# endiqq/Multi-Feature-ViT

Measured on AMD Instinct MI355X. Metric: images/sec (two-stream 224^2 vit_small MF-CA train step), higher is better.
Workload: dtype bf16x3 (split bf16 hi+lo operands, 3 MFMAs per product, f32 accumulate)

## Files before the change

### include/mfvit.h

```cpp
#ifndef MFVIT_H
#define MFVIT_H
#include <stddef.h>
#include <stdint.h>

#ifdef __cplusplus
extern "C" {
#endif

typedef void* mfvit_stream_t;

#define MFVIT_OK 0
#define MFVIT_EINVAL (-22)
#define MFVIT_ENOSYS (-38)
#define MFVIT_ELAUNCH (-5)

#define MFVIT_F32 0
#define MFVIT_BF16 1
#define MFVIT_BF16X3 2
#define MFVIT_F16 3
#define MFVIT_X3F16 4

int mfvit_abi_version(void);
const char* mfvit_build_info(void);

typedef struct mfvit_vit_cfg {
    int dtype;
    int batch;
    int img_h, img_w;
    int dim;
    int depth;
    int heads;
    int mlp_dim;
    int save_for_backward;
    int stop_grad_conv1;
    float ln_eps;
    int token_input;
    int tokens;
    int use_pos;
    int act;
    float p_embd, p_attn, p_resid;
    uint32_t seed_lo, seed_hi;
    int stream_share;
} mfvit_vit_cfg;

size_t mfvit_vit_param_count(const mfvit_vit_cfg* cfg);
int mfvit_vit_param_layout(const mfvit_vit_cfg* cfg, int64_t out[9]);

size_t mfvit_vit_shadow_bytes(const mfvit_vit_cfg* cfg);
int mfvit_vit_prepare_shadow(const mfvit_vit_cfg* cfg, const float* params, void* shadow, mfvit_stream_t stream);

size_t mfvit_vit_workspace_bytes(const mfvit_vit_cfg* cfg);

int mfvit_vit_forward(const mfvit_vit_cfg* cfg, const float* params, const void* shadow, const float* img, void* workspace,
                      float* features, mfvit_stream_t stream);

int mfvit_vit_backward(const mfvit_vit_cfg* cfg, const float* params, const void* shadow, void* workspace, const float* dfeatures,
                       float* dparams, int stage_hi, int stage_lo, mfvit_stream_t stream);

typedef struct mfvit_vit_drop {
    float drop;
    float attn_drop;
    const float* drop_path;
    uint64_t seed;
} mfvit_vit_drop;
size_t mfvit_vit_workspace_bytes_drop(const mfvit_vit_cfg* cfg, const mfvit_vit_drop* drop);
int mfvit_vit_forward_drop(const mfvit_vit_cfg* cfg, const mfvit_vit_drop* drop, const float* params, const void* shadow, const float* img,
                           void* workspace, float* features, mfvit_stream_t stream);
int mfvit_vit_backward_drop(const mfvit_vit_cfg* cfg, const mfvit_vit_drop* drop, const float* params, const void* shadow, void* workspace,
                            const float* dfeatures, float* dparams, int stage_hi, int stage_lo, mfvit_stream_t stream);

size_t mfvit_vit_workspace_bytes_ex(const mfvit_vit_cfg* cfg, const mfvit_vit_drop* drop, int want_dimg);
int mfvit_vit_backward_ex(const mfvit_vit_cfg* cfg, const mfvit_vit_drop* drop, const float* params, const void* shadow, void* workspace,
                          const float* dfeatures, float* dparams, float* dimg, int stage_hi, int stage_lo, mfvit_stream_t stream);

typedef struct mfvit_vit_attn_req {
    uint64_t blocks;
    int fuse;
    int cls_only;
    float* maps;
    float* rollout;
    void* scratch;
} mfvit_vit_attn_req;
size_t mfvit_vit_attn_scratch_bytes(const mfvit_vit_cfg* cfg, const mfvit_vit_attn_req* req);
int mfvit_vit_forward_attn(const mfvit_vit_cfg* cfg, const mfvit_vit_attn_req* req, const float* params, const void* shadow,
                           const float* img, void* workspace, float* features, mfvit_stream_t stream);

typedef struct mfvit_vit_rel_req {
    uint64_t blocks;
    float* maps;
    float* relevance;
    void* scratch;
} mfvit_vit_rel_req;
size_t mfvit_vit_rel_scratch_bytes(const mfvit_vit_cfg* cfg, const mfvit_vit_rel_req* req);
int mfvit_vit_backward_rel(const mfvit_vit_cfg* cfg, const mfvit_vit_rel_req* req, const float* params, const void* shadow, void* workspace,
                           const float* dfeatures, mfvit_stream_t stream);

int mfvit_gpt_forward(const mfvit_vit_cfg* cfg, const float* params, const void* shadow, const float* tokens, void* workspace, float* out,
                      mfvit_stream_t stream);
int mfvit_gpt_backward(const mfvit_vit_cfg* cfg, const float* params, const void* shadow, void* workspace, const float* dout, float* dparams,
                       float* dtokens, mfvit_stream_t stream);

int mfvit_linear_fwd(int dtype, int epilogue, const void* x, int64_t ldx, const void* w, int64_t ldw, const float* bias, void* y,
                     int64_t ldy, void* y2, int64_t ldy2, int M, int N, int K, mfvit_stream_t stream);
int mfvit_linear_dgrad_act(int dtype, const void* dy, int64_t lddy, const void* wt, int64_t ldwt, const void* act_grad, int64_t ldg,
                           void* dx, int64_t lddx, int M, int N, int K, mfvit_stream_t stream);
int mfvit_linear_wgrad(int dtype, const void* dy, int64_t lddy, const void* x, int64_t ldx, float* dw, int64_t lddw, int M, int N, int K,
                       mfvit_stream_t stream);
#define MFVIT_WGRAD_SCRATCH_FLOATS (384 * 128 * 128)
int mfvit_linear_wgrad_ws(int dtype, const void* dy, int64_t lddy, const void* x, int64_t ldx, float* dw, int64_t lddw, int M, int N,
                          int K, float* scratch, mfvit_stream_t stream);
int mfvit_linear_wgrad_pair(int dtype, const void* dy_a, int64_t lddy_a, const void* x_a, int64_t ldx_a, float* dw_a, int64_t lddw_a, float* dbias_a,
                            int Na, const void* dy_b, int64_t lddy_b, const void* x_b, int64_t ldx_b, float* dw_b, int64_t lddw_b, int Nb, int M, int K,
                            mfvit_stream_t stream);
int mfvit_linear_res_ln_fwd(int dtype, const void* a, int64_t lda, const void* w, int64_t ldw, const float* bias, const float* res,
                            int64_t ldres, float* x_out, void* y, int y_f32, const float* gamma, const float* beta, float eps,
                            float* mean, float* rstd, int M, int K, mfvit_stream_t stream);
int mfvit_linear_dgrad_ln_bwd(int dtype, const void* dy, int64_t lddy, const void* wt, int64_t ldwt, const float* x, const float* mean,
                              const float* rstd, const float* gamma, const float* dres, float* dx, void* dx_t, float* dgamma,
                              float* dbeta, float* dcol, int M, int K, mfvit_stream_t stream);
#define MFVIT_ROWP_SCRATCH_FLOATS (264 * 7 * 12 * 512)
int mfvit_linear_res_ln_fwd_ws(int dtype, const void* a, int64_t lda, const void* w, int64_t ldw, const float* bias, const float* res,
                               int64_t ldres, float* x_out, void* y, int y_f32, const float* gamma, const float* beta, float eps,
                               float* mean, float* rstd, int M, int K, float* scratch, mfvit_stream_t stream);
int mfvit_linear_dgrad_ln_bwd_ws(int dtype, const void* dy, int64_t lddy, const void* wt, int64_t ldwt, const float* x, const float* mean,
                                 const float* rstd, const float* gamma, const float* dres, float* dx, void* dx_t, float* dgamma,
                                 float* dbeta, float* dcol, int M, int K, float* scratch, mfvit_stream_t stream);
int mfvit_attention_qkv_dtype(int dtype, int T, int head_dim);
int mfvit_attention_fwd(int dtype, const void* qkv, void* out, float* lse, int B, int T, int H, int head_dim, mfvit_stream_t stream);
int mfvit_attention_bwd(int dtype, const void* qkv, const void* out, const void* dout, const float* lse, void* dqkv, float* dbias_qkv,
                        int B, int T, int H, int head_dim, mfvit_stream_t stream);
int mfvit_attention_drop_fwd(int dtype, const void* qkv, void* out, float* lse, int B, int T, int H, int head_dim, float p, uint64_t seed,
                             uint32_t site, mfvit_stream_t stream);
int mfvit_attention_drop_bwd(int dtype, const void* qkv, const void* out, const void* dout, const float* lse, void* dqkv, int B, int T, int H,
                             int head_dim, float p, uint64_t seed, uint32_t site, mfvit_stream_t stream);
int mfvit_dropout_mask(float p, uint64_t seed, uint32_t site, int64_t n, uint8_t* keep, mfvit_stream_t stream);
int mfvit_layernorm_fwd(int dtype, const float* x, void* y, int y_f32, const float* gamma, const float* beta, float eps, float* mean,
                        float* rstd, int rows, int N, mfvit_stream_t stream);
int mfvit_layernorm_bwd(int dtype, const float* dy, const float* x, const float* mean, const float* rstd, const float* gamma,
                        const float* dres, float* dx, void* dx_t, float* dgamma, float* dbeta, float* dcol, int rows, int N,
                        mfvit_stream_t stream);
int mfvit_cast_transpose(int dtype, const float* src, void* dst, void* dst_t, int R, int C, mfvit_stream_t stream);
int mfvit_head_fwd(const float* x, int64_t ldx, const float* w, const float* b, float* y, int64_t ldy, int M, int N, int K, int accumulate,
                   mfvit_stream_t stream);
int mfvit_head_bwd(const float* dy, int64_t lddy, const float* x, int64_t ldx, const float* w, float* dx, int64_t lddx, int dx_accumulate,
                   float* dw, float* db, int M, int N, int K, mfvit_stream_t stream);
int mfvit_cross_entropy(const float* logits, const int64_t* target, float* loss_mean, float* dlogits, int64_t* preds, int B, int C,
                        mfvit_stream_t stream);
int mfvit_cross_entropy_soft(const float* logits, const int64_t* target, const int32_t* partner, const float* lam, float smoothing,
                             float* loss_mean, float* dlogits, int64_t* preds, int B, int C, mfvit_stream_t stream);

int mfvit_batch_mix(const float* a, const float* b, float* out_a, float* out_b, const int32_t* desc, const float* lam, int n, int C, int H,
                    int W, mfvit_stream_t stream);

int mfvit_input_transform(const uint8_t* src, const int64_t* desc, const int32_t* tables, int n, int S, int crop, const float* mean3,
                          const float* std3, float* out, mfvit_stream_t stream);
int mfvit_input_transform_rect(const uint8_t* src, const int64_t* desc, const int32_t* tables, int n, int S, int out_h, int out_w,
                               const float* mean3, const float* std3, float* out, mfvit_stream_t stream);

size_t mfvit_input_photometric_workspace_bytes(int n, int S);
int mfvit_input_photometric(const uint8_t* src, const int64_t* desc, const int32_t* tables, const int32_t* photo, int n, int S, int max_radius,
                            void* workspace, const float* mean3, const float* std3, float* out, mfvit_stream_t stream);

int mfvit_eval_counts(const float* scores, int64_t ld, const int64_t* labels, int n, int C, uint64_t* confusion, int64_t* preds,
                      uint64_t* u2, uint64_t* npos, mfvit_stream_t stream);

int mfvit_patch_rank(const float* rel, int64_t ld, int32_t* rank, int B, int P, mfvit_stream_t stream);
int mfvit_patch_perturb(const float* img, const int32_t* rank, const int32_t* steps, const float* fill, float* out, int B, int C, int H,
                        int W, int S, mfvit_stream_t stream);
int mfvit_perturb_score(const float* logits, int64_t ld, const int64_t* target, int S, int B, int C, uint64_t* correct, double* sums,
                        uint64_t* nonfinite, mfvit_stream_t stream);

int mfvit_attr_inputs(const float* x, const float* base, int base_full, const float* alpha, const float* sigma, const uint64_t* seed, int s0,
                      float* out, int S, int B, int C, int64_t hw, mfvit_stream_t stream);
int mfvit_attr_accumulate(const float* g, const float* w, float* acc, int k, int B, int64_t n, int power, mfvit_stream_t stream);
int mfvit_attr_finish(const float* acc, const float* x, const float* base, int base_full, int times_input, int absval, float* pixels,
                      float* patches, double* total, int B, int C, int H, int W, mfvit_stream_t stream);

typedef struct mfvit_fusion_cfg {
    int batch;
    int tokens;
    int dim;
    int heads;
    int num_classes;
    float eps_pre;
    float eps_post;
} mfvit_fusion_cfg;

size_t mfvit_fusion_param_count(const mfvit_fusion_cfg* cfg);
size_t mfvit_fusion_workspace_bytes(const mfvit_fusion_cfg* cfg);
int mfvit_fusion_forward(const mfvit_fusion_cfg* cfg, const float* params, const float* f_cxr, const float* f_enh, const float* hw_cxr,
                         const float* hb_cxr, const float* hw_enh, const float* hb_enh, void* workspace, float* fused, float* x_cxr,
                         float* x_enh, mfvit_stream_t stream);
int mfvit_fusion_backward(const mfvit_fusion_cfg* cfg, const float* params, const float* f_cxr, const float* f_enh, const float* hw_cxr,
                          const float* hw_enh, void* workspace, const float* dfused, const float* dx_cxr, const float* dx_enh,
                          float* dparams, float* df_cxr, float* df_enh, float* dhw_cxr, float* dhb_cxr, float* dhw_enh, float* dhb_enh,
                          mfvit_stream_t stream);

size_t mfvit_fusion_ex_param_count(const mfvit_fusion_cfg* cfg, int cross_attn_depth, int pool_mean);
size_t mfvit_fusion_ex_workspace_bytes(const mfvit_fusion_cfg* cfg, int cross_attn_depth, int pool_mean);
int mfvit_fusion_ex_forward(const mfvit_fusion_cfg* cfg, int cross_attn_depth, int pool_mean, const float* params, const float* f_cxr,
                            const float* f_enh, const float* hw_cxr, const float* hb_cxr, const float* hw_enh, const float* hb_enh,
                            void* workspace, float* fused, float* x_cxr, float* x_enh, mfvit_stream_t stream);
int mfvit_fusion_ex_backward(const mfvit_fusion_cfg* cfg, int cross_attn_depth, int pool_mean, const float* params, const float* f_cxr,
                             const float* f_enh, const float* hw_cxr, const float* hw_enh, void* workspace, const float* dfused,
                             const float* dx_cxr, const float* dx_enh, float* dparams, float* df_cxr, float* df_enh, float* dhw_cxr,
                             float* dhb_cxr, float* dhw_enh, float* dhb_enh, mfvit_stream_t stream);

int mfvit_fusion_ex_attention(const mfvit_fusion_cfg* cfg, int cross_attn_depth, int pool_mean, const void* workspace, int layer, int fuse,
                              float* out, mfvit_stream_t stream);
int mfvit_fusion_ex_grad_attention(const mfvit_fusion_cfg* cfg, int cross_attn_depth, int pool_mean, const float* params, const float* f_cxr,
                                   const float* f_enh, const void* workspace, int layer, float* abar, mfvit_stream_t stream);

size_t mfvit_bimodal_relevance_scratch_bytes(int B, int T);
int mfvit_bimodal_relevance(int B, int T, int depth_c, int depth_e, const float* maps_c, const float* maps_e, const float* abar, float* out4,
                            void* scratch, mfvit_stream_t stream);

int mfvit_prenorm_xattn_forward(const mfvit_fusion_cfg* cfg, const float* params, const float* x_own, const float* x_oth,
                                void* workspace, float* out, mfvit_stream_t stream);
int mfvit_prenorm_xattn_backward(const mfvit_fusion_cfg* cfg, const float* params, const float* x_own, const float* x_oth,
                                 void* workspace, const float* dout, float* dparams, float* dx_own, float* dx_oth,
                                 mfvit_stream_t stream);

int mfvit_xattn_forward(const mfvit_fusion_cfg* cfg, const float* params, const float* x, void* workspace, float* out,
                        mfvit_stream_t stream);
int mfvit_xattn_backward(const mfvit_fusion_cfg* cfg, const float* params, const float* x, void* workspace, const float* dout,
                         float* dparams, float* dx, mfvit_stream_t stream);

int mfvit_prof_enable(int class_mask);
int mfvit_set_wgrad_stream(int enabled);
int mfvit_set_stream_share(int n);
int mfvit_prof_collect(double* out, int ncls);
int mfvit_prof_collect_tags(double* out, int ntags);
const char* mfvit_prof_class_name(int cls);

int mfvit_bn_stats(int dtype, const void* x, int n, int C, float* mean, float* m2, mfvit_stream_t stream);
int mfvit_bn_combine(const float* means, const float* m2s, const float* counts, int W, int C, float eps, float momentum, float* mean,
                     float* invstd, float* running_mean, float* running_var, mfvit_stream_t stream);
int mfvit_bn_apply(int dtype, const void* x, const float* mean, const float* invstd, const float* gamma, const float* beta, int relu,
                   void* y, int n, int C, mfvit_stream_t stream);
int mfvit_bn_bwd_sums(int dtype, const void* dy, const void* x, const void* y, const float* mean, const float* invstd, int relu, int n,
                      int C, float* s1, float* s2, mfvit_stream_t stream);
int mfvit_bn_bwd_apply(int dtype, const void* dy, const void* x, const void* y, const float* mean, const float* invstd, const float* gamma,
                       int relu, const float* S1, const float* S2, float inv_count, void* dx, int n, int C, mfvit_stream_t stream);
int mfvit_l2norm_fwd(const float* x, float* y, float* inv_norm, int n, int C, float eps, mfvit_stream_t stream);
int mfvit_l2norm_bwd(const float* dy, const float* y, const float* inv_norm, float* dx, int n, int C, mfvit_stream_t stream);
int mfvit_rowdot(const float* a, const float* b, float* out, int64_t ldo, float scale, int n, int C, mfvit_stream_t stream);
int mfvit_cross_entropy_rows(const float* logits, int64_t ld, const int64_t* target, float* loss_mean, float* lse, float* dlogits,
                             int64_t ldd, int n, int C, mfvit_stream_t stream);
int mfvit_ema_update(float* dst, const float* src, float m, int64_t n, mfvit_stream_t stream);

int mfvit_lars_step(const int64_t* table, int nchunks, int ntensors, float* norms, float lr, float weight_decay, float momentum,
                    float trust_coefficient, mfvit_stream_t stream);
int mfvit_adam_step(const int64_t* table, int nchunks, float lr, float beta1, float beta2, float eps, float weight_decay, int step,
                    mfvit_stream_t stream);
int mfvit_sgd_step(const int64_t* table, int nchunks, float lr, float momentum, float weight_decay, int first_step,
                   mfvit_stream_t stream);
int mfvit_amp_unscale(const int64_t* table, int nchunks, float inv_scale, float* found_inf, mfvit_stream_t stream);

int mfvit_grad_norm_partials(const int64_t* table, int nchunks, int norm_kind, float* partials, mfvit_stream_t stream);
int mfvit_grad_clip_coef(const float* partials, const int32_t* row_tensor, int nrows, int ntensors, int norm_kind, double max_norm,
                         float* per_tensor, float* out2, mfvit_stream_t stream);
int mfvit_grad_scale(const int64_t* table, int nchunks, const float* coef, mfvit_stream_t stream);

#ifdef __cplusplus
}
#endif
#endif
```

### multi-feature-vit_amd/csrc/abi_ops.hip

```cpp
#include "../../include/mfvit.h"
#include "kernels.h"

using namespace mfvit;

extern "C" {

int mfvit_input_transform(const uint8_t* src, const int64_t* desc, const int32_t* tables, int n, int S, int crop, const float* mean3,
                          const float* std3, float* out, mfvit_stream_t stream) {
    if (!src || !desc || !tables || !mean3 || !std3 || !out) return MFVIT_EINVAL;
    if (crop > S) return MFVIT_EINVAL;
    return input_transform(src, (const long long*)desc, tables, n, S, crop, crop, mean3, std3, out, (hipStream_t)stream);
}
int mfvit_input_transform_rect(const uint8_t* src, const int64_t* desc, const int32_t* tables, int n, int S, int out_h, int out_w,
                               const float* mean3, const float* std3, float* out, mfvit_stream_t stream) {
    if (!src || !desc || !tables || !mean3 || !std3 || !out) return MFVIT_EINVAL;
    return input_transform(src, (const long long*)desc, tables, n, S, out_h, out_w, mean3, std3, out, (hipStream_t)stream);
}
size_t mfvit_input_photometric_workspace_bytes(int n, int S) { return input_photometric_workspace_bytes(n, S); }
int mfvit_input_photometric(const uint8_t* src, const int64_t* desc, const int32_t* tables, const int32_t* photo, int n, int S, int max_radius,
                            void* workspace, const float* mean3, const float* std3, float* out, mfvit_stream_t stream) {
    if (!src || !desc || !tables || !photo || !workspace || !mean3 || !std3 || !out) return MFVIT_EINVAL;
    return input_photometric(src, (const long long*)desc, tables, photo, n, S, max_radius, workspace, mean3, std3, out, (hipStream_t)stream);
}
int mfvit_eval_counts(const float* scores, int64_t ld, const int64_t* labels, int n, int C, uint64_t* confusion, int64_t* preds,
                      uint64_t* u2, uint64_t* npos, mfvit_stream_t stream) {
    if (!scores || !labels || (!confusion && !(u2 && npos))) return MFVIT_EINVAL;
    return eval_counts(scores, ld, labels, n, C, (unsigned long long*)confusion, (unsigned long long*)u2, (unsigned long long*)npos, preds,
                       (hipStream_t)stream);
}
int mfvit_linear_fwd(int dtype, int epilogue, const void* x, int64_t ldx, const void* w, int64_t ldw, const float* bias, void* y,
                     int64_t ldy, void* y2, int64_t ldy2, int M, int N, int K, mfvit_stream_t stream) {
    if (!x || !w || (!y && epilogue != EPI_BIAS_GELU)) return MFVIT_EINVAL;
    if (epilogue != EPI_BIAS && epilogue != EPI_BIAS_GELU && epilogue != EPI_NONE && epilogue != EPI_BIAS_X3F16) return MFVIT_EINVAL;
    if (epilogue == EPI_BIAS_GELU && !y2) return MFVIT_EINVAL;
    GemmP p = nt(x, ldx, w, ldw, M, N, K);
    p.bias = bias; p.out0 = y; p.ldo0 = ldy; p.out1 = y2; p.ldo1 = ldy2;
    return gemm_nt_tile(dtype, epilogue, p, (hipStream_t)stream);
}
int mfvit_linear_dgrad_act(int dtype, const void* dy, int64_t lddy, const void* wt, int64_t ldwt, const void* act_grad, int64_t ldg,
                           void* dx, int64_t lddx, int M, int N, int K, mfvit_stream_t stream) {
    if (!dy || !wt || !act_grad || !dx) return MFVIT_EINVAL;
    GemmP p = nt(dy, lddy, wt, ldwt, M, N, K);
    p.aux = act_grad; p.ldaux = ldg; p.out0 = dx; p.ldo0 = lddx;
    return gemm_nt_tile(dtype, EPI_GELU_BWD, p, (hipStream_t)stream);
}
int mfvit_linear_wgrad(int dtype, const void* dy, int64_t lddy, const void* x, int64_t ldx, float* dw, int64_t lddw, int M, int N, int K,
                       mfvit_stream_t stream) {
    if (!dy || !x || !dw) return MFVIT_EINVAL;
    GemmP p = nt(dy, lddy, x, ldx, M, N, K);
    p.out0 = dw; p.ldo0 = lddw;
    return gemm_tn(dtype, p, (hipStream_t)stream);
}
int mfvit_linear_wgrad_ws(int dtype, const void* dy, int64_t lddy, const void* x, int64_t ldx, float* dw, int64_t lddw, int M, int N,
                          int K, float* scratch, mfvit_stream_t stream) {
    if (!dy || !x || !dw) return MFVIT_EINVAL;
    GemmP p = nt(dy, lddy, x, ldx, M, N, K);
    p.out0 = dw; p.ldo0 = lddw;
    p.cpart = scratch;
    return gemm_tn(dtype, p, (hipStream_t)stream);
}
int mfvit_linear_wgrad_pair(int dtype, const void* dy_a, int64_t lddy_a, const void* x_a, int64_t ldx_a, float* dw_a, int64_t lddw_a, float* dbias_a,
                            int Na, const void* dy_b, int64_t lddy_b, const void* x_b, int64_t ldx_b, float* dw_b, int64_t lddw_b, int Nb, int M, int K,
                            mfvit_stream_t stream) {
    if (!dy_a || !x_a || !dw_a || !dy_b || !x_b || !dw_b) return MFVIT_EINVAL;
    GemmP a = nt(dy_a, lddy_a, x_a, ldx_a, M, Na, K), b = nt(dy_b, lddy_b, x_b, ldx_b, M, Nb, K);
    a.out0 = dw_a; a.ldo0 = lddw_a; a.cs0 = dbias_a;
    b.out0 = dw_b; b.ldo0 = lddw_b;
    if (!gemm_tn_pair_supported(dtype, a, b)) return MFVIT_ENOSYS;
    return gemm_tn_glds_pair(dtype, a, b, (hipStream_t)stream);
}
int mfvit_linear_res_ln_fwd(int dtype, const void* a, int64_t lda, const void* w, int64_t ldw, const float* bias, const float* res,
                            int64_t ldres, float* x_out, void* y, int y_f32, const float* gamma, const float* beta, float eps,
                            float* mean, float* rstd, int M, int K, mfvit_stream_t stream) {
    return mfvit_linear_res_ln_fwd_ws(dtype, a, lda, w, ldw, bias, res, ldres, x_out, y, y_f32, gamma, beta, eps, mean, rstd, M, K, nullptr, stream);
}
int mfvit_linear_res_ln_fwd_ws(int dtype, const void* a, int64_t lda, const void* w, int64_t ldw, const float* bias, const float* res,
                               int64_t ldres, float* x_out, void* y, int y_f32, const float* gamma, const float* beta, float eps,
                               float* mean, float* rstd, int M, int K, float* scratch, mfvit_stream_t stream) {
    if (!a || !w || !y || !gamma || !beta || ((size_t)scratch & 15)) return MFVIT_EINVAL;
    GemmP p = nt(a, lda, w, ldw, M, 384, K);
    p.kpart = scratch;
    p.bias = bias; p.res = res; p.ldres = ldres;
    p.out0 = x_out; p.ldo0 = 384; p.out1 = y; p.ldo1 = (dtype == MFVIT_BF16X3 && !y_f32) ? 768 : 384; p.y_f32 = y_f32;
    p.gamma = gamma; p.beta = beta; p.eps = eps; p.mean = mean; p.rstd = rstd;
    return gemm_nt_row(dtype, REPI_RES_LN, p, (hipStream_t)stream);
}
int mfvit_linear_dgrad_ln_bwd(int dtype, const void* dy, int64_t lddy, const void* wt, int64_t ldwt, const float* x, const float* mean,
                              const float* rstd, const float* gamma, const float* dres, float* dx, void* dx_t, float* dgamma,
                              float* dbeta, float* dcol, int M, int K, mfvit_stream_t stream) {
    return mfvit_linear_dgrad_ln_bwd_ws(dtype, dy, lddy, wt, ldwt, x, mean, rstd, gamma, dres, dx, dx_t, dgamma, dbeta, dcol, M, K, nullptr, stream);
}
int mfvit_linear_dgrad_ln_bwd_ws(int dtype, const void* dy, int64_t lddy, const void* wt, int64_t ldwt, const float* x, const float* mean,
                                 const float* rstd, const float* gamma, const float* dres, float* dx, void* dx_t, float* dgamma,
                                 float* dbeta, float* dcol, int M, int K, float* scratch, mfvit_stream_t stream) {
    if (!dy || !wt || !x || !mean || !rstd || !gamma || !dx || ((size_t)scratch & 15)) return MFVIT_EINVAL;
    GemmP p = nt(dy, lddy, wt, ldwt, M, 384, K);
    p.kpart = scratch;
    p.aux = x; p.ldaux = 384; p.mean = (float*)mean; p.rstd = (float*)rstd; p.gamma = gamma;
    p.res = dres; p.ldres = 384;
    p.out0 = dx; p.ldo0 = 384; p.out1 = dx_t; p.ldo1 = dtype == MFVIT_BF16X3 ? 768 : 384;
    p.cs0 = dgamma; p.cs1 = dbeta; p.cs2 = dcol;
    return gemm_nt_row(dtype, REPI_LNBWD_RES, p, (hipStream_t)stream);
}
int mfvit_attention_fwd(int dtype, const void* qkv, void* out, float* lse, int B, int T, int H, int head_dim, mfvit_stream_t stream) {
    if (!qkv || !out || !lse || B <= 0 || T <= 0 || H <= 0) return MFVIT_EINVAL;
    return attn_fwd(dtype, qkv, out, lse, B, T, H, head_dim, (hipStream_t)stream);
}
int mfvit_attention_qkv_dtype(int dtype, int T, int head_dim) { return attn_qkv_dtype(dtype, T, head_dim); }
int mfvit_attention_bwd(int dtype, const void* qkv, const void* out, const void* dout, const float* lse, void* dqkv, float* dbias_qkv,
                        int B, int T, int H, int head_dim, mfvit_stream_t stream) {
    if (!qkv || !out || !dout || !lse || !dqkv || B <= 0 || T <= 0 || H <= 0) return MFVIT_EINVAL;
    return attn_bwd(dtype, qkv, out, dout, lse, dqkv, dbias_qkv, B, T, H, head_dim, (hipStream_t)stream);
}
int mfvit_attention_drop_fwd(int dtype, const void* qkv, void* out, float* lse, int B, int T, int H, int head_dim, float p, uint64_t seed,
                             uint32_t site, mfvit_stream_t stream) {
    if (!qkv || !out || !lse || B <= 0 || T <= 0 || H <= 0 || !(p >= 0.f && p < 1.f)) return MFVIT_EINVAL;
    if (!attn_tiled_supported(dtype, T, head_dim)) return MFVIT_ENOSYS;
    return attn_fwd_tiled_drop(dtype, qkv, out, lse, B, T, H, head_dim, make_drop(p, seed, site), (hipStream_t)stream);
}
int mfvit_attention_drop_bwd(int dtype, const void* qkv, const void* out, const void* dout, const float* lse, void* dqkv, int B, int T, int H,
                             int head_dim, float p, uint64_t seed, uint32_t site, mfvit_stream_t stream) {
    if (!qkv || !out || !dout || !lse || !dqkv || B <= 0 || T <= 0 || H <= 0 || !(p >= 0.f && p < 1.f)) return MFVIT_EINVAL;
    if (!attn_tiled_supported(dtype, T, head_dim)) return MFVIT_ENOSYS;
    return attn_bwd_tiled_drop(dtype, qkv, out, dout, lse, dqkv, B, T, H, head_dim, make_drop(p, seed, site), (hipStream_t)stream);
}
int mfvit_dropout_mask(float p, uint64_t seed, uint32_t site, int64_t n, uint8_t* keep, mfvit_stream_t stream) {
    if (!keep || !(p >= 0.f && p < 1.f)) return MFVIT_EINVAL;
    return dropout_mask(make_drop(p, seed, site), n, keep, (hipStream_t)stream);
}
int mfvit_layernorm_fwd(int dtype, const float* x, void* y, int y_f32, const float* gamma, const float* beta, float eps, float* mean,
                        float* rstd, int rows, int N, mfvit_stream_t stream) {
    if (!x || !y || !gamma || !beta) return MFVIT_EINVAL;
    return ln_rows(dtype, N, x, N, nullptr, 0, 0, nullptr, 0, y, (dtype == MFVIT_BF16X3 && !y_f32) ? 2 * N : N, y_f32, gamma, beta, eps, mean, rstd, rows, 1, 0,
                   0, (hipStream_t)stream);
}
int mfvit_layernorm_bwd(int dtype, const float* dy, const float* x, const float* mean, const float* rstd, const float* gamma,
                        const float* dres, float* dx, void* dx_t, float* dgamma, float* dbeta, float* dcol, int rows, int N,
                        mfvit_stream_t stream) {
    if (!dy || !x || !mean || !rstd || !gamma) return MFVIT_EINVAL;
    return ln_bwd_rows(dtype, N, dy, N, x, N, mean, rstd, gamma, dres, N, dx, N, dx_t, dtype == MFVIT_BF16X3 ? 2 * N : N, dgamma, dbeta, dcol, nullptr, rows, 1, 0,
                       (hipStream_t)stream);
}
int mfvit_cast_transpose(int dtype, const float* src, void* dst, void* dst_t, int R, int C, mfvit_stream_t stream) {
    if (!src || R <= 0 || C <= 0) return MFVIT_EINVAL;
    return cast_transpose(dtype, src, dst, dst_t, R, C, (hipStream_t)stream);
}
int mfvit_head_fwd(const float* x, int64_t ldx, const float* w, const float* b, float* y, int64_t ldy, int M, int N, int K, int accumulate,
                   mfvit_stream_t stream) {
    if (!x || !w || !y) return MFVIT_EINVAL;
    return linear_small_fwd(x, ldx, w, b, y, ldy, M, N, K, accumulate, (hipStream_t)stream);
}
int mfvit_head_bwd(const float* dy, int64_t lddy, const float* x, int64_t ldx, const float* w, float* dx, int64_t lddx, int dx_accumulate,
                   float* dw, float* db, int M, int N, int K, mfvit_stream_t stream) {
    if (!dy || !x || !w) return MFVIT_EINVAL;
    return linear_small_bwd(dy, lddy, x, ldx, w, dx, lddx, dx_accumulate, dw, db, M, N, K, (hipStream_t)stream);
}
int mfvit_cross_entropy(const float* logits, const int64_t* target, float* loss_mean, float* dlogits, int64_t* preds, int B, int C,
                        mfvit_stream_t stream) {
    if (!logits || !target || !loss_mean) return MFVIT_EINVAL;
    return ce_small(logits, (const long*)target, loss_mean, dlogits, (long*)preds, B, C, (hipStream_t)stream);
}

}
```

### multi-feature-vit_amd/csrc/elementwise.hip

```cpp
#include "kernels.h"

namespace mfvit {

template <typename T>
__global__ void im2col16_kernel(const float* __restrict__ img, T* __restrict__ P, int B, int Hh, int Ww) {
    const int gh = Hh / 16, gw = Ww / 16;
    const long total = (long)B * gh * gw * 3 * 16 * 2;
    for (long q = blockIdx.x * (long)blockDim.x + threadIdx.x; q < total; q += (long)gridDim.x * blockDim.x) {
        const int half = q & 1;
        long r = q >> 1;
        const int py = r % 16; r /= 16;
        const int c = r % 3; r /= 3;
        const int pw = r % gw; r /= gw;
        const int ph = r % gh; r /= gh;
        const int b = (int)r;
        const float* s = img + (((long)b * 3 + c) * Hh + ph * 16 + py) * Ww + pw * 16 + half * 8;
        const float4 v0 = *(const float4*)s, v1 = *(const float4*)(s + 4);
        const int k = c * 256 + py * 16 + half * 8;
        T* d = P + ((long)(b * gh + ph) * gw + pw) * 768 * elems_per<T>::value + (is_split<T>::value ? split_col(k) : k);
        if constexpr (sizeof(T) == 2) {
            typedef typename Vec4<T>::elem E;
            const float f[8] = {v0.x, v0.y, v0.z, v0.w, v1.x, v1.y, v1.z, v1.w};
            typename Vec8<T>::type o, l;
#pragma unroll
// ... 99 lines not shown
template <typename T, int NPL>
__global__ __launch_bounds__(256) void add_ln_rows_kernel(const T* __restrict__ tin, long ldt, const float* __restrict__ pos, long ldp, int pmod,
                                                          const float* __restrict__ res, long ldres, int rin, int rout, int roff,
                                                          float* __restrict__ xout, long ldx, void* __restrict__ y, long ldy, int y_f32,
                                                          const float* __restrict__ gamma, const float* __restrict__ beta, float eps,
                                                          float* __restrict__ mean, float* __restrict__ rstd, int rows) {
    constexpr int N = NPL * 64;
    const int lane = threadIdx.x & 63;
    const int g = blockIdx.x * 4 + (threadIdx.x >> 6);
    if (g >= rows) return;
    const long go = rin ? (long)(g / rin) * rout + roff + g % rin : g;
    float v[NPL];
#pragma unroll
    for (int i = 0; i < NPL; ++i) {
        const int n = lane + 64 * i;
        float t = load_elem<T>(tin + (long)g * ldt, n);
        if (pos) t += pos[(pmod ? go % pmod : go) * ldp + n];
        v[i] = res ? res[go * ldres + n] + t : t;
    }
    float s = 0.f;
#pragma unroll
    for (int i = 0; i < NPL; ++i) s += v[i];
    const float mu = wave_sum(s) * (1.0f / N);
    float q = 0.f;
#pragma unroll
    for (int i = 0; i < NPL; ++i) { const float dd = v[i] - mu; q += dd * dd; }
    const float rs = rsqrtf(wave_sum(q) * (1.0f / N) + eps);
    if (lane == 0) {
        if (mean) mean[go] = mu;
        if (rstd) rstd[go] = rs;
    }
#pragma unroll
    for (int i = 0; i < NPL; ++i) {
        const int n = lane + 64 * i;
        if (xout) xout[go * ldx + n] = v[i];
        const float o = (v[i] - mu) * rs * gamma[n] + beta[n];
        if (y_f32) ((float*)y)[go * ldy + n] = o;
        else store_elem<T>((T*)y + go * ldy, n, o);
    }
}
int add_ln_rows(int dtype, int N, const void* tin, long ldt, const float* pos, long ldp, int pmod, const float* res, long ldres, int rin, int rout,
                int roff, float* xout, long ldx, void* y, long ldy, int y_f32, const float* gamma, const float* beta, float eps, float* mean,
                float* rstd, int rows, hipStream_t st) {
    if (rows <= 0) return MFVIT_OK;
    if (!tin || !y || !gamma || !beta || (rin && (rout < rin || roff < 0))) return MFVIT_EINVAL;
    const dim3 grid((rows + 3) / 4), blk(256);
#define MFVIT_ALN(TT, NPL)                                                                                                                 \
    MFVIT_LAUNCH((add_ln_rows_kernel<TT, NPL>), grid, blk, 0, st, (const TT*)tin, ldt, pos, ldp, pmod, res, ldres, rin, rout, roff, xout, ldx, y, \
                 ldy, y_f32, gamma, beta, eps, mean, rstd, rows)
#define MFVIT_ALN_N(NPL)                                  \
    switch (dtype) {                                      \
        case MFVIT_BF16: MFVIT_ALN(bf16, NPL); break;     \
        case MFVIT_BF16X3: MFVIT_ALN(sbf16, NPL); break;  \
        case MFVIT_F16: MFVIT_ALN(f16, NPL); break;       \
        case MFVIT_F32: MFVIT_ALN(float, NPL); break;     \
        default: return MFVIT_EINVAL;                     \
    }
    if (N == 384) { MFVIT_ALN_N(6) }
    else if (N == 768) { MFVIT_ALN_N(12) }
    else return MFVIT_EINVAL;
#undef MFVIT_ALN_N
#undef MFVIT_ALN
    MFVIT_CHECK_LAUNCH();
    return MFVIT_OK;
}

template <typename T, int NPL>
__global__ __launch_bounds__(256) void drop_add_ln_rows_kernel(const T* __restrict__ tin, long ldt, const float* a0, long lda0,
                                                               const float* __restrict__ a1, long lda1, int mod1, const float* __restrict__ res,
                                                               long ldres, DropP drop, DropP dpath, int tpr, float* xout, long ldx, void* __restrict__ y,
                                                               long ldy, int y_f32, const float* __restrict__ gamma,
                                                               const float* __restrict__ beta, float eps, float* __restrict__ mean,
                                                               float* __restrict__ rstd, int rows) {
    constexpr int N = NPL * 64;
    const int lane = threadIdx.x & 63;
    const int g = blockIdx.x * 4 + (threadIdx.x >> 6);
    if (g >= rows) return;
    float v[NPL];
    const float sk = drop_mul(dpath, (unsigned)(g / tpr));
#pragma unroll
    for (int i = 0; i < NPL; ++i) {
        const int n = lane + 64 * i;
        float t = tin ? load_elem<T>(tin + (long)g * ldt, n) : a0[(long)g * lda0 + n];
        if (!tin && a1) t += a1[(long)(mod1 ? g % mod1 : g) * lda1 + n];
        t *= drop_mul(drop, (unsigned)g * (unsigned)N + (unsigned)n) * sk;
        v[i] = res ? res[(long)g * ldres + n] + t : t;
    }
    float s = 0.f;
#pragma unroll
    for (int i = 0; i < NPL; ++i) s += v[i];
    const float mu = wave_sum(s) * (1.0f / N);
    float q = 0.f;
#pragma unroll
    for (int i = 0; i < NPL; ++i) { const float dd = v[i] - mu; q += dd * dd; }
    const float rs = rsqrtf(wave_sum(q) * (1.0f / N) + eps);
    if (lane == 0) {
        if (mean) mean[g] = mu;
        if (rstd) rstd[g] = rs;
    }
#pragma unroll
    for (int i = 0; i < NPL; ++i) {
        const int n = lane + 64 * i;
        if (xout) xout[(long)g * ldx + n] = v[i];
        const float o = (v[i] - mu) * rs * gamma[n] + beta[n];
        if (y_f32) ((float*)y)[(long)g * ldy + n] = o;
        else store_elem<T>((T*)y + (long)g * ldy, n, o);
    }
}
int drop_add_ln_rows(int dtype, int N, const void* tin, long ldt, const float* a0, long lda0, const float* a1, long lda1, int mod1,
                     const float* res, long ldres, DropP drop, DropP dpath, int tpr, float* xout, long ldx, void* y, long ldy, int y_f32,
                     const float* gamma, const float* beta, float eps, float* mean, float* rstd, int rows, hipStream_t st) {
    if (rows <= 0) return MFVIT_OK;
    if ((N != 384 && N != 768) || tpr <= 0 || (!tin && !a0) || !y || (double)rows * N >= 4294967296.0) return MFVIT_EINVAL;
    const dim3 grid((rows + 3) / 4), blk(256);
#define MFVIT_DAL(TT)                                                                                                                      \
    if (N == 384) MFVIT_LAUNCH((drop_add_ln_rows_kernel<TT, 6>), grid, blk, 0, st, (const TT*)tin, ldt, a0, lda0, a1, lda1, mod1, res, ldres, drop, \
                               dpath, tpr, xout, ldx, y, ldy, y_f32, gamma, beta, eps, mean, rstd, rows);                                          \
    else MFVIT_LAUNCH((drop_add_ln_rows_kernel<TT, 12>), grid, blk, 0, st, (const TT*)tin, ldt, a0, lda0, a1, lda1, mod1, res, ldres, drop,       \
                      dpath, tpr, xout, ldx, y, ldy, y_f32, gamma, beta, eps, mean, rstd, rows)
    switch (dtype) {
        case MFVIT_BF16: MFVIT_DAL(bf16); break;
        case MFVIT_BF16X3: MFVIT_DAL(sbf16); break;
        case MFVIT_F16: MFVIT_DAL(f16); break;
        default: return MFVIT_EINVAL;
    }
#undef MFVIT_DAL
    MFVIT_CHECK_LAUNCH();
    return MFVIT_OK;
}
template <typename T, bool F32>
__global__ __launch_bounds__(256) void mask_scale_rows_kernel(const void* src, long lds_, void* dst, long ldd, DropP drop, DropP dpath, int tpr,
                                                              int rows, int N) {
    const long i = (long)blockIdx.x * 256 + threadIdx.x;
    if (i >= (long)rows * N) return;
    const int g = (int)(i / N), n = (int)(i % N);
    const float mk = drop_mul(drop, (unsigned)i) * drop_mul(dpath, (unsigned)(g / tpr));
    if constexpr (F32) ((float*)dst)[(long)g * ldd + n] = ((const float*)src)[(long)g * lds_ + n] * mk;
    else store_elem<T>((T*)dst + (long)g * ldd, n, load_elem<T>((const T*)src + (long)g * lds_, n) * mk);
}
int mask_scale_rows(int dtype, bool f32, const void* src, long lds_, void* dst, long ldd, DropP drop, DropP dpath, int tpr, int rows, int N,
                    hipStream_t st) {
    if (rows <= 0) return MFVIT_OK;
    if (tpr <= 0 || (double)rows * N >= 4294967296.0) return MFVIT_EINVAL;
    const dim3 grid((unsigned)(((long)rows * N + 255) / 256)), blk(256);
    if (f32) MFVIT_LAUNCH((mask_scale_rows_kernel<float, true>), grid, blk, 0, st, src, lds_, dst, ldd, drop, dpath, tpr, rows, N);
    else if (dtype == MFVIT_BF16) MFVIT_LAUNCH((mask_scale_rows_kernel<bf16, false>), grid, blk, 0, st, src, lds_, dst, ldd, drop, dpath, tpr, rows, N);
    else if (dtype == MFVIT_BF16X3) MFVIT_LAUNCH((mask_scale_rows_kernel<sbf16, false>), grid, blk, 0, st, src, lds_, dst, ldd, drop, dpath, tpr, rows, N);
    else if (dtype == MFVIT_F16) MFVIT_LAUNCH((mask_scale_rows_kernel<f16, false>), grid, blk, 0, st, src, lds_, dst, ldd, drop, dpath, tpr, rows, N);
    else return MFVIT_EINVAL;
    MFVIT_CHECK_LAUNCH();
    return MFVIT_OK;
}

template <typename T, int NPL>
__global__ __launch_bounds__(256) void ln_bwd_rows_kernel(const float* __restrict__ dy, long lddy, const float* __restrict__ x, long ldx,
                                                          const float* __restrict__ mean, const float* __restrict__ rstd,
                                                          const float* __restrict__ gamma, const float* __restrict__ dres, long ldres,
                                                          float* __restrict__ dx, long lddx, T* __restrict__ dxT, long lddxT,
                                                          float* __restrict__ dgamma, float* __restrict__ dbeta, float* __restrict__ dcol,
                                                          float* __restrict__ cpart, int rows, int row_stride, int row_off,
                                                          const T* __restrict__ dyT, long lddyT) {
    constexpr int N = NPL * 64;
    __shared__ float red[3][4][N];
    const int lane = threadIdx.x & 63, w = threadIdx.x >> 6;
    float gm[NPL], ag[NPL], ab[NPL], ax[NPL];
#pragma unroll
    for (int i = 0; i < NPL; ++i) { gm[i] = gamma[lane + 64 * i]; ag[i] = ab[i] = ax[i] = 0.f; }
    for (int r = blockIdx.x * 4 + w; r < rows; r += gridDim.x * 4) {
        const long g = (long)r * row_stride + row_off;
        const float mu = mean[g], rs = rstd[g];
        float d[NPL], h[NPL];
        float s1 = 0.f, s2 = 0.f;
#pragma unroll
        for (int i = 0; i < NPL; ++i) {
            const int n = lane + 64 * i;
            d[i] = dyT ? load_elem<T>(dyT + g * lddyT, n) : dy[g * lddy + n];
            h[i] = (x[g * ldx + n] - mu) * rs;
            const float t = d[i] * gm[i];
            s1 += t;
            s2 += t * h[i];
            ag[i] += d[i] * h[i];
            ab[i] += d[i];
        }
        const float c1 = wave_sum(s1) * (1.0f / N), c2 = wave_sum(s2) * (1.0f / N);
#pragma unroll
        for (int i = 0; i < NPL; ++i) {
            const int n = lane + 64 * i;
            float o = rs * (d[i] * gm[i] - c1 - h[i] * c2);
            if (dres) o += dres[g * ldres + n];
            if (dx) dx[g * lddx + n] = o;
            if (dxT) store_elem<T>(dxT + g * lddxT, n, o);
            ax[i] += o;
        }
    }
#pragma unroll
    for (int i = 0; i < NPL; ++i) {
        red[0][w][lane + 64 * i] = ag[i];
        red[1][w][lane + 64 * i] = ab[i];
        red[2][w][lane + 64 * i] = ax[i];
    }
    __syncthreads();
    for (int n = threadIdx.x; n < N; n += 256) {
        const float a = red[0][0][n] + red[0][1][n] + red[0][2][n] + red[0][3][n];
        const float b = red[1][0][n] + red[1][1][n] + red[1][2][n] + red[1][3][n];
        const float c = red[2][0][n] + red[2][1][n] + red[2][2][n] + red[2][3][n];
        if (cpart) {
            cpart[((long)blockIdx.x * 3 + 0) * N + n] = a;
            cpart[((long)blockIdx.x * 3 + 1) * N + n] = b;
            cpart[((long)blockIdx.x * 3 + 2) * N + n] = c;
        } else {
            if (dgamma) atomicAdd(dgamma + n, a);
            if (dbeta) atomicAdd(dbeta + n, b);
            if (dcol) atomicAdd(dcol + n, c);
        }
    }
}
int ln_bwd_rows(int dtype, int N, const float* dy, long lddy, const float* x, long ldx, const float* mean, const float* rstd,
                const float* gamma, const float* dres, long ldres, float* dx, long lddx, void* dxT, long lddxT, float* dgamma, float* dbeta,
                float* dcol, float* cpart, int rows, int row_stride, int row_off, hipStream_t st, const void* dyT, long lddyT) {
    if (rows <= 0) return MFVIT_OK;
    if (!dy && !dyT) return MFVIT_EINVAL;
    int blocks = (rows + 3) / 4;
    const int cap = cpart ? 256 : 1024;
    if (blocks > cap) blocks = cap;
#define MFVIT_LNB(TT, NPL)                                                                                                         \
    MFVIT_LAUNCH((ln_bwd_rows_kernel<TT, NPL>), dim3(blocks), dim3(256), 0, st, dy, lddy, x, ldx, mean, rstd, gamma, dres, ldres, dx, \
                       lddx, (TT*)dxT, lddxT, dgamma, dbeta, dcol, cpart, rows, row_stride, row_off, (const TT*)dyT, lddyT)
#define MFVIT_LNB_N(NPL)                                  \
    switch (dtype) {                                      \
        case MFVIT_BF16: MFVIT_LNB(bf16, NPL); break;     \
        case MFVIT_BF16X3: MFVIT_LNB(sbf16, NPL); break;  \
        case MFVIT_F16: MFVIT_LNB(f16, NPL); break;       \
        case MFVIT_F32: MFVIT_LNB(float, NPL); break;     \
        default: return MFVIT_EINVAL;                     \
    }
    if (N == 384) { MFVIT_LNB_N(6) }
    else if (N == 768) { MFVIT_LNB_N(12) }
    else return MFVIT_EINVAL;
#undef MFVIT_LNB_N
#undef MFVIT_LNB
    MFVIT_CHECK_LAUNCH();
    if (cpart) return colpart_reduce(cpart, blocks, N, 3, dgamma, dbeta, dcol, st);
    return MFVIT_OK;
}

template <typename T>
__global__ __launch_bounds__(256) void cast_transpose_kernel(const float* __restrict__ src, T* __restrict__ dst, T* __restrict__ dstT, int R,
                                                             int C, long s_src, long s_dst, long s_dstT) {
    __shared__ float tile[64][65];
    src += blockIdx.z * s_src;
    if (dst) dst = (T*)((char*)dst + blockIdx.z * s_dst);
    if (dstT) dstT = (T*)((char*)dstT + blockIdx.z * s_dstT);
    const int r0 = blockIdx.y * 64, c0 = blockIdx.x * 64;
    for (int q = threadIdx.x; q < 64 * 64; q += 256) {
        const int r = q >> 6, c = q & 63;
        float v = 0.f;
        if (r0 + r < R && c0 + c < C) {
            v = src[(long)(r0 + r) * C + c0 + c];
            if (dst) store_elem<T>(dst + (long)(r0 + r) * C * elems_per<T>::value, c0 + c, v);
        }
        tile[r][c] = v;
    }
    __syncthreads();
    if (dstT) {
        for (int q = threadIdx.x; q < 64 * 64; q += 256) {
            const int c = q >> 6, r = q & 63;
            if (r0 + r < R && c0 + c < C) store_elem<T>(dstT + (long)(c0 + c) * R * elems_per<T>::value, r0 + r, tile[r][c]);
        }
    }
}
template <typename T> __device__ __forceinline__ void store_elem4(T* row, int n, float v0, float v1, float v2, float v3) {
    if constexpr (std::is_same<T, float>::value) {
        *(float4*)(row + n) = make_float4(v0, v1, v2, v3);
    } else if constexpr (is_split<T>::value) {
        bf16 h[4], l[4];
        cvt_pair<bf16, true>(v0, v1, h[0], h[1], l[0], l[1]);
        cvt_pair<bf16, true>(v2, v3, h[2], h[3], l[2], l[3]);
        bf16* r = (bf16*)row + split_col(n);
        *(bf16x4*)r = bf16x4{h[0], h[1], h[2], h[3]};
        *(bf16x4*)(r + 32) = bf16x4{l[0], l[1], l[2], l[3]};
    } else {
        T h[4], l[4];
        cvt_pair<T, false>(v0, v1, h[0], h[1], l[0], l[1]);
        cvt_pair<T, false>(v2, v3, h[2], h[3], l[2], l[3]);
        typedef typename Vec4<T>::type V;
        *(V*)(row + n) = V{h[0], h[1], h[2], h[3]};
    }
}
template <typename T>
__global__ __launch_bounds__(256) void cast_transpose4_kernel(const float* __restrict__ src, T* __restrict__ dst, T* __restrict__ dstT, int R,
                                                              int C, long s_src, long s_dst, long s_dstT) {
    __shared__ float tile[64][65];
    src += blockIdx.z * s_src;
    if (dst) dst = (T*)((char*)dst + blockIdx.z * s_dst);
    if (dstT) dstT = (T*)((char*)dstT + blockIdx.z * s_dstT);
    const int r0 = blockIdx.y * 64, c0 = blockIdx.x * 64;
#pragma unroll
    for (int k = 0; k < 4; ++k) {
        const int q = threadIdx.x + 256 * k, r = q >> 4, c = (q & 15) * 4;
        float4 v = make_float4(0.f, 0.f, 0.f, 0.f);
        if (r0 + r < R && c0 + c < C) {
            v = *(const float4*)(src + (long)(r0 + r) * C + c0 + c);
            if (dst) store_elem4<T>(dst + (long)(r0 + r) * C * elems_per<T>::value, c0 + c, v.x, v.y, v.z, v.w);
        }
        tile[r][c] = v.x;
        tile[r][c + 1] = v.y;
        tile[r][c + 2] = v.z;
        tile[r][c + 3] = v.w;
    }
    __syncthreads();
    if (dstT) {
#pragma unroll
        for (int k = 0; k < 4; ++k) {
            const int q = threadIdx.x + 256 * k, c = q >> 4, r = (q & 15) * 4;
            if (r0 + r < R && c0 + c < C)
                store_elem4<T>(dstT + (long)(c0 + c) * R * elems_per<T>::value, r0 + r, tile[r][c], tile[r + 1][c], tile[r + 2][c], tile[r + 3][c]);
        }
    }
}
int cast_transpose_batched(int dtype, const float* src, void* dst, void* dstT, int R, int C, int nb, long s_src, long s_dst, long s_dstT,
                           hipStream_t st) {
    const dim3 grid((C + 63) / 64, (R + 63) / 64, nb);
    if (R % 4 == 0 && C % 4 == 0 && s_src % 4 == 0 && s_dst % 16 == 0 && s_dstT % 16 == 0 &&
        (((uintptr_t)src | (uintptr_t)dst | (uintptr_t)dstT) & 15) == 0 && !(dtype == MFVIT_BF16X3 && ((dst && C % 32) || (dstT && R % 32)))) {
        switch (dtype) {
            case MFVIT_BF16: MFVIT_LAUNCH(cast_transpose4_kernel<bf16>, grid, dim3(256), 0, st, src, (bf16*)dst, (bf16*)dstT, R, C, s_src, s_dst, s_dstT); break;
            case MFVIT_BF16X3: MFVIT_LAUNCH(cast_transpose4_kernel<sbf16>, grid, dim3(256), 0, st, src, (sbf16*)dst, (sbf16*)dstT, R, C, s_src, s_dst, s_dstT); break;
            case MFVIT_F16: MFVIT_LAUNCH(cast_transpose4_kernel<f16>, grid, dim3(256), 0, st, src, (f16*)dst, (f16*)dstT, R, C, s_src, s_dst, s_dstT); break;
            case MFVIT_F32: MFVIT_LAUNCH(cast_transpose4_kernel<float>, grid, dim3(256), 0, st, src, (float*)dst, (float*)dstT, R, C, s_src, s_dst, s_dstT); break;
            default: return MFVIT_EINVAL;
        }
        MFVIT_CHECK_LAUNCH();
        return MFVIT_OK;
    }
    if (dtype == MFVIT_BF16)
        MFVIT_LAUNCH(cast_transpose_kernel<bf16>, grid, dim3(256), 0, st, src, (bf16*)dst, (bf16*)dstT, R, C, s_src, s_dst, s_dstT);
    else if (dtype == MFVIT_BF16X3) {
        if ((dst && C % 32) || (dstT && R % 32)) return MFVIT_EINVAL;
        MFVIT_LAUNCH(cast_transpose_kernel<sbf16>, grid, dim3(256), 0, st, src, (sbf16*)dst, (sbf16*)dstT, R, C, s_src, s_dst, s_dstT);
    } else if (dtype == MFVIT_F16)
        MFVIT_LAUNCH(cast_transpose_kernel<f16>, grid, dim3(256), 0, st, src, (f16*)dst, (f16*)dstT, R, C, s_src, s_dst, s_dstT);
    else if (dtype == MFVIT_F32)
        MFVIT_LAUNCH(cast_transpose_kernel<float>, grid, dim3(256), 0, st, src, (float*)dst, (float*)dstT, R, C, s_src, s_dst, s_dstT);
    else
        return MFVIT_EINVAL;
    MFVIT_CHECK_LAUNCH();
    return MFVIT_OK;
}
int cast_transpose(int dtype, const float* src, void* dst, void* dstT, int R, int C, hipStream_t st) {
    return cast_transpose_batched(dtype, src, dst, dstT, R, C, 1, 0, 0, 0, st);
}

__global__ __launch_bounds__(256) void linear_small_fwd_kernel(const float* __restrict__ x, long ldx, const float* __restrict__ W,
                                                               const float* __restrict__ b, float* __restrict__ y, long ldy, int M, int N,
                                                               int K, int accumulate) {
    const int o = blockIdx.x * 4 + (threadIdx.x >> 6), lane = threadIdx.x & 63;
    if (o >= M * N) return;
    const int m = o / N, n = o % N;
    float s = 0.f;
    for (int k = lane; k < K; k += 64) s = fmaf(x[(long)m * ldx + k], W[(long)n * K + k], s);
    s = wave_sum(s);
    if (lane == 0) {
        s += b ? b[n] : 0.f;
        if (accumulate) y[(long)m * ldy + n] += s; else y[(long)m * ldy + n] = s;
    }
}
__global__ __launch_bounds__(256) void linear_small_bwd_kernel(const float* __restrict__ dy, long lddy, const float* __restrict__ x, long ldx,
                                                               const float* __restrict__ W, float* __restrict__ dx, long lddx,
                                                               int dx_accumulate, float* __restrict__ dW, float* __restrict__ db, int M,
                                                               int N, int K) {
    const long id = blockIdx.x * (long)blockDim.x + threadIdx.x;
    if (dx && id < (long)M * K) {
        const int m = id / K, k = id % K;
        float s = 0.f;
        for (int n = 0; n < N; ++n) s = fmaf(dy[(long)m * lddy + n], W[(long)n * K + k], s);
        if (dx_accumulate) dx[(long)m * lddx + k] += s; else dx[(long)m * lddx + k] = s;
    }
    if (dW && id < (long)N * K) {
        const int n = id / K, k = id % K;
        float s = 0.f;
        for (int m = 0; m < M; ++m) s = fmaf(dy[(long)m * lddy + n], x[(long)m * ldx + k], s);
        dW[(long)n * K + k] += s;
    }
    if (db && id < N) {
        float s = 0.f;
        for (int m = 0; m < M; ++m) s += dy[(long)m * lddy + id];
        db[id] += s;
    }
}
int linear_small_fwd(const float* x, long ldx, const float* W, const float* b, float* y, long ldy, int M, int N, int K, int accumulate,
                     hipStream_t st) {
    MFVIT_LAUNCH(linear_small_fwd_kernel, dim3((M * N + 3) / 4), dim3(256), 0, st, x, ldx, W, b, y, ldy, M, N, K, accumulate);
    MFVIT_CHECK_LAUNCH();
    return MFVIT_OK;
}
int linear_small_bwd(const float* dy, long lddy, const float* x, long ldx, const float* W, float* dx, long lddx, int dx_accumulate, float* dW,
                     float* db, int M, int N, int K, hipStream_t st) {
    long work = (long)M * K;
    if ((long)N * K > work) work = (long)N * K;
    MFVIT_LAUNCH(linear_small_bwd_kernel, dim3((unsigned)((work + 255) / 256)), dim3(256), 0, st, dy, lddy, x, ldx, W, dx, lddx,
                       dx_accumulate, dW, db, M, N, K);
    MFVIT_CHECK_LAUNCH();
    return MFVIT_OK;
}

__global__ __launch_bounds__(1024) void ce_small_kernel(const float* __restrict__ logits, const long* __restrict__ target, float* __restrict__ loss_mean,
                                                        float* __restrict__ dlogits, long* __restrict__ preds, int B, int C) {
    __shared__ float red[16];
    float li = 0.f;
    for (int b = threadIdx.x; b < B; b += 1024) {
        const float* z = logits + (long)b * C;
        float m = z[0];
        int am = 0;
        for (int c = 1; c < C; ++c) if (first_max_takes(z[c], m)) { m = z[c]; am = c; }
        float s = 0.f;
        for (int c = 0; c < C; ++c) s += __expf(z[c] - m);
        const float lse = m + __logf(s);
        const int t = (int)target[b];
        li += (lse - z[t]) / (float)B;
        if (dlogits)
            for (int c = 0; c < C; ++c) dlogits[(long)b * C + c] = (__expf(z[c] - lse) - (c == t ? 1.f : 0.f)) / (float)B;
        if (preds) preds[b] = am;
    }
    li = wave_sum(li);
    if ((threadIdx.x & 63) == 0) red[threadIdx.x >> 6] = li;
    __syncthreads();
    if (threadIdx.x == 0) {
        float t = 0.f;
#pragma unroll
        for (int i = 0; i < 16; ++i) t += red[i];
        *loss_mean = t;
    }
}
int ce_small(const float* logits, const long* target, float* loss_mean, float* dlogits, long* preds, int B, int C, hipStream_t st) {
    if (C > 64 || C < 1) return MFVIT_EINVAL;
    MFVIT_LAUNCH(ce_small_kernel, dim3(1), dim3(1024), 0, st, logits, target, loss_mean, dlogits, preds, B, C);
    MFVIT_CHECK_LAUNCH();
    return MFVIT_OK;
}

__global__ void add_rows_kernel(float* __restrict__ dst, long ldd, const float* __restrict__ src, long lds_, int rows, int N) {
    const long id = blockIdx.x * (long)blockDim.x + threadIdx.x;
    if (id < (long)rows * N) dst[(id / N) * ldd + id % N] += src[(id / N) * lds_ + id % N];
}
int add_rows(float* dst, long ldd, const float* src, long lds_, int rows, int N, hipStream_t st) {
    MFVIT_LAUNCH(add_rows_kernel, dim3((unsigned)(((long)rows * N + 255) / 256)), dim3(256), 0, st, dst, ldd, src, lds_, rows, N);
    MFVIT_CHECK_LAUNCH();
    return MFVIT_OK;
}
__global__ void axpy_kernel(float* __restrict__ y, const float* __restrict__ x, float a, long n) {
    const long i = blockIdx.x * (long)blockDim.x + threadIdx.x;
    if (i < n) y[i] = fmaf(a, x[i], y[i]);
}
int axpy(float* y, const float* x, float a, long n, hipStream_t st) {
    MFVIT_LAUNCH(axpy_kernel, dim3((unsigned)((n + 255) / 256)), dim3(256), 0, st, y, x, a, n);
    MFVIT_CHECK_LAUNCH();
    return MFVIT_OK;
}
__global__ __launch_bounds__(1024) void colsum_rows_kernel(const float* __restrict__ x, long ld, float* __restrict__ out, int rows,
                                                           int row_stride, int row_off, int N) {
    const int n = blockIdx.x * 64 + (threadIdx.x & 63), sub = threadIdx.x >> 6;
    __shared__ float sm[16][64];
    float s = 0.f;
    if (n < N) {
#pragma unroll 4
        for (int r = sub; r < rows; r += 16) s += x[((long)r * row_stride + row_off) * ld + n];
    }
    sm[sub][threadIdx.x & 63] = s;
    __syncthreads();
    if (sub == 0 && n < N) {
        s = 0.f;
#pragma unroll
        for (int i = 0; i < 16; ++i) s += sm[i][threadIdx.x];
        out[n] += s;
    }
}
int colsum_rows(const float* x, long ld, float* out, int rows, int row_stride, int row_off, int N, hipStream_t st) {
    MFVIT_LAUNCH(colsum_rows_kernel, dim3((N + 63) / 64), dim3(1024), 0, st, x, ld, out, rows, row_stride, row_off, N);
    MFVIT_CHECK_LAUNCH();
    return MFVIT_OK;
}

__global__ __launch_bounds__(256) void batch_sum_kernel(const float* __restrict__ x, float* __restrict__ out, int B, long n) {
    const long i = blockIdx.x * 256L + threadIdx.x;
    if (i >= n) return;
    float s = 0.f;
    for (int b = 0; b < B; ++b) s += x[(long)b * n + i];
    out[i] += s;
}
int batch_sum(const float* x, float* out, int B, long n, hipStream_t st) {
    MFVIT_LAUNCH(batch_sum_kernel, dim3((unsigned)((n + 255) / 256)), dim3(256), 0, st, x, out, B, n);
    MFVIT_CHECK_LAUNCH();
    return MFVIT_OK;
}

__global__ __launch_bounds__(256) void dropout_mask_kernel(DropP drop, long n, unsigned char* __restrict__ out) {
    const long i = (long)blockIdx.x * 256 + threadIdx.x;
    if (i < n) out[i] = drop_mul(drop, (unsigned)i) != 0.f;
}
int dropout_mask(DropP drop, long n, unsigned char* out, hipStream_t st) {
    if (n <= 0 || n >= (1L << 32)) return MFVIT_EINVAL;
    MFVIT_LAUNCH(dropout_mask_kernel, dim3((unsigned)((n + 255) / 256)), dim3(256), 0, st, drop, n, out);
    MFVIT_CHECK_LAUNCH();
    return MFVIT_OK;
}

}
```

### multi-feature-vit_amd/csrc/fusion.hip

```cpp
#include "kernels.h"
#include "prof.h"

#include <string.h>

using namespace mfvit;

namespace {

constexpr int NH = 3;

struct FusLayout {
    long ca[2], post[2], head[2];
    long n_w, n_b, wq, wk, wv, wp, bp;
    long ca_stride;
    long total;
    int no_norm;
};
FusLayout fus_layout(int D, int C) {
    FusLayout L;
    const long blk = 4L * D * D + 3L * D;
    L.n_w = 0; L.n_b = D; L.wq = 2L * D; L.wk = L.wq + (long)D * D; L.wv = L.wk + (long)D * D; L.wp = L.wv + (long)D * D;
    L.bp = L.wp + (long)D * D;
    const long o0 = 0, o1 = blk, o2 = o1 + 2 * D, o3 = o2 + blk, oh = o3 + 2 * D;
    L.ca[0] = o0; L.ca[1] = o2;
// ... 720 lines not shown
        if (dx) {
            const float c1 = wave_sum(s1) * (1.f / D), c2 = wave_sum(s2) * (1.f / D);
#pragma unroll
            for (int i = 0; i < NPL; ++i) {
                float* o = dx + ((long)b * T + t) * D + lane + 64 * i;
                *o = *o + rs * (dy[i] * g[i] - c1 - xh[i] * c2) + (add_ev ? e[i] : 0.f);
            }
        }
    }
#pragma unroll
    for (int i = 0; i < NPL; ++i) { red[(w * 2) * D + lane + 64 * i] = ag[i]; red[(w * 2 + 1) * D + lane + 64 * i] = ab[i]; }
    __syncthreads();
    for (int q = threadIdx.x; q < 2 * D; q += XW * 64) {
        float v = 0.f;
        for (int w2 = 0; w2 < XW; ++w2) v += red[w2 * 2 * D + q];
        pr_r[q] = v;
    }
}

__global__ __launch_bounds__(256) void x_attn_map_kernel(const float* __restrict__ a, int nh, int T, long n, int fuse, float* __restrict__ out) {
    const long i = blockIdx.x * 256L + threadIdx.x;
    if (i >= n) return;
    if (fuse == 0) { out[i] = a[i]; return; }
    const long sb = i / T;
    const int t = (int)(i - sb * T);
    const float* p = a + sb * nh * T + t;
    float f = p[0];
    for (int h = 1; h < nh; ++h) {
        const float v = p[(long)h * T];
        f = fuse == 1 ? f + v : fuse == 2 ? fmaxf(f, v) : fminf(f, v);
    }
    out[i] = fuse == 1 ? f / (float)nh : f;
}

template <int XW, int D>
__global__ __launch_bounds__(XW * 64) void x_grad_map_kernel(const float* __restrict__ fc, const float* __restrict__ fe,
                                                         const float* __restrict__ params, FusLayout L, int B, int T, int nh,
                                                         const float* __restrict__ a_in, const float* __restrict__ st_in,
                                                         const float* __restrict__ du, float* __restrict__ abar) {
    constexpr int NPL = D / 64;
    extern __shared__ __attribute__((aligned(16))) float xs[];
    float* st = xs;
    float* acc = st + 2 * T;
    const int b = blockIdx.x, dir = blockIdx.y, lane = threadIdx.x & 63, w = threadIdx.x >> 6;
    const long sb = (long)dir * B + b;
    const float* own = (dir == 0 ? fc : fe) + (long)b * T * D;
    const float* oth = (dir == 0 ? fe : fc) + (long)b * T * D;
    float g[NPL], be[NPL];
#pragma unroll
    for (int i = 0; i < NPL; ++i) {
        g[i] = L.no_norm ? 1.f : params[L.ca[dir] + L.n_w + lane + 64 * i];
        be[i] = L.no_norm ? 0.f : params[L.ca[dir] + L.n_b + lane + 64 * i];
    }
    for (int q = threadIdx.x; q < 2 * T; q += XW * 64) st[q] = st_in[sb * 2 * T + q];
    __syncthreads();
    for (int h0 = 0; h0 < nh; h0 += NH) {
        float duv[NH][NPL];
#pragma unroll
        for (int h = 0; h < NH; ++h)
#pragma unroll
            for (int i = 0; i < NPL; ++i) duv[h][i] = du[(sb * nh + h0 + h) * D + lane + 64 * i];
        for (int t = w; t < T; t += XW) {
            const float* row = t == 0 ? own : oth + (long)t * D;
            const float mu = st[t], rs = st[T + t];
            float d0 = 0.f, d1 = 0.f, d2 = 0.f;
#pragma unroll
            for (int i = 0; i < NPL; ++i) {
                const float z = (row[lane + 64 * i] - mu) * rs * g[i] + be[i];
                d0 = fmaf(z, duv[0][i], d0); d1 = fmaf(z, duv[1][i], d1); d2 = fmaf(z, duv[2][i], d2);
            }
            d0 = wave_sum(d0); d1 = wave_sum(d1); d2 = wave_sum(d2);
            if (lane == 0) {
                const float* ap = a_in + (sb * nh + h0) * T + t;
                float s = h0 == 0 ? 0.f : acc[t];
                s += fmaxf(0.f, ap[0] * d0);
                s += fmaxf(0.f, ap[T] * d1);
                s += fmaxf(0.f, ap[2 * T] * d2);
                acc[t] = s;
            }
        }
    }
    __syncthreads();
    for (int t = threadIdx.x; t < T; t += XW * 64) abar[sb * T + t] = acc[t] / (float)nh;
}

GemmP zg() { GemmP p; memset(&p, 0, sizeof(p)); return p; }

template <int D> constexpr int xw_fwd() { return D == 384 ? 16 : 8; }
constexpr int XW_BWD = 8, XW_DZ = 8, XW_ROWS = 8;
constexpr int MAX_XDEPTH = 16;
#define FUS_TRY(expr) do { int rc__ = (expr); if (rc__ != MFVIT_OK) return rc__; } while (0)
#define FUS_BY_DIM(dim, CALL) ((dim) == 384 ? CALL<384> : CALL<768>)

constexpr size_t FUS_MAX_LDS = 160 * 1024;
size_t lds_stream_fwd(int D, int T) { return (size_t)(5L * T + (long)(D == 384 ? xw_fwd<384>() : xw_fwd<768>()) * NH * D) * 4; }
size_t lds_stream_bwd(int D, int T) { return (size_t)(8L * T + (long)XW_BWD * 5 * D) * 4; }
size_t lds_stream_dz(int D, int T, int nh) {
    const long big = 2L * nh * D + 2L * nh * T, redn = (long)XW_DZ * 2 * D;
    return (size_t)((big > redn ? big : redn) + 2L * T) * 4;
}
bool fus_lds_ok(int D, int T, int nh) {
    return lds_stream_fwd(D, T) <= FUS_MAX_LDS && lds_stream_bwd(D, T) <= FUS_MAX_LDS && (nh == NH || lds_stream_dz(D, T, nh) <= FUS_MAX_LDS);
}

bool fus_ok(const mfvit_fusion_cfg* c) {
    return c && c->batch > 0 && c->tokens > 1 && (c->dim == 384 || c->dim == 768) && (c->heads == 3 || c->heads == 6 || c->heads == 12) &&
           c->num_classes > 0 && c->num_classes <= 64 && fus_lds_ok(c->dim, c->tokens, c->heads);
}
bool fus_ex_ok(const mfvit_fusion_cfg* c, int depth, int pool_mean) {
    return fus_ok(c) && depth >= 1 && depth <= MAX_XDEPTH && (pool_mean == 0 || pool_mean == 1);
}
bool fus_full(int depth, int pool_mean) { return depth > 1 || pool_mean; }

FusLayout fus_layer_layout(int D, int C, int depth, int l) {
    FusLayout L = fus_layout(D, C);
    const long lay = 8L * D * D + 10L * D;
    for (int dir = 0; dir < 2; ++dir) { L.ca[dir] += l * lay; L.post[dir] += l * lay; }
    L.head[0] = depth * lay;
    L.head[1] = L.head[0] + (long)C * D + C;
    L.total = depth * lay + 2 * ((long)C * D + C);
    return L;
}

struct FusExWs {
    long Y, yst, pr, pbp, slab;
    long dx, ev, bb, fusv;
    long total;
};
FusExWs fus_ex_ws(int B, int T, int C, int D, int NH, int depth) {
    FusExWs E;
    long o = 0;
    auto take = [&](long n) { long r = o; o += (n + 63) & ~63L; return r; };
    take(fus_ws(B, T, C, D, NH).total);
    E.Y = take(2L * B * T * D); E.yst = take(2L * B * T * 2); E.pr = take(2L * 2 * B * 2 * D); E.pbp = take(2L * B * D);
    E.slab = o;
    o = depth * E.slab;
    E.dx = take(depth > 1 ? 2 * 2L * B * T * D : 0);
    E.ev = take(2L * B * D); E.bb = take(2L * B * D); E.fusv = take(2L * B * D);
    E.total = o;
    return E;
}

template <typename K> void max_lds(K* kern, PerDeviceOnce& once) {
    if (once.first()) (void)hipFuncSetAttribute((const void*)kern, hipFuncAttributeMaxDynamicSharedMemorySize, (int)FUS_MAX_LDS);
}

}

template <int D>
static int xattn_core_forward(int ndir, int nh, const FusLayout& L, const FusWs& W, const float* params, const float* f_cxr,
                              const float* f_enh, float* ws, int B, int T, float eps_pre, hipStream_t st) {
    const int DH = D / nh;
    const float scale = 1.0f / sqrtf((float)DH);
    for (int dir = 0; dir < ndir; ++dir) {
        const long offs[4] = {L.wq, L.wk, L.wv, L.wp};
        for (int k = 0; k < 4; ++k)
            FUS_TRY(cast_transpose(MFVIT_F32, params + L.ca[dir] + offs[k], nullptr, ws + W.wT + ((long)dir * 4 + k) * D * D, D, D, st));
    }
    MFVIT_LAUNCH(x_cls_ln_kernel<D>, dim3(B, ndir), dim3(64), 0, st, f_cxr, f_enh, params, L, eps_pre, B, T, ws + W.z0, ws + W.st0);
    MFVIT_CHECK_LAUNCH();
    {
        GemmP p = zg();
        p.A = ws + W.z0; p.lda = D; p.W = params + L.ca[0] + L.wq; p.ldw = D; p.M = B; p.N = D; p.K = D;
        p.out0 = ws + W.qv; p.ldo0 = D;
        p.nb = ndir; p.nbi = 1; p.sAo = (long)B * D; p.sWo = L.ca_stride; p.sOo = (long)B * D;
        FUS_TRY(gemm_nt_tile(MFVIT_F32, EPI_NONE, p, st));
    }
    {
        GemmP p = zg();
        p.A = ws + W.qv; p.lda = D; p.W = ws + W.wT + 1L * D * D; p.ldw = D; p.M = B; p.N = D; p.K = DH;
        p.out0 = ws + W.kq; p.ldo0 = nh * D;
        p.nb = ndir * nh; p.nbi = nh; p.sAo = (long)B * D; p.sAi = DH; p.sWo = 4L * D * D; p.sWi = DH; p.sOo = (long)B * nh * D; p.sOi = D;
        FUS_TRY(gemm_nt_tile(MFVIT_F32, EPI_NONE, p, st));
    }
    {
        constexpr int XW = xw_fwd<D>();
        const size_t lds = lds_stream_fwd(D, T);
        static PerDeviceOnce attr1, attrc;
        ProfScope ps(PROF_XATTN_FWD, 0, 2.0 * B * T * D * 4 * 2 * (nh / NH), st);
        if (nh == NH) {
            max_lds((x_stream_fwd_kernel<XW, D, false>), attr1);
            MFVIT_LAUNCH((x_stream_fwd_kernel<XW, D, false>), dim3(B, ndir), dim3(XW * 64), lds, st, f_cxr, f_enh, params, L, eps_pre, scale, B, T,
                               ws + W.kq, ws + W.u, ws + W.a, ws + W.st);
        } else {
            max_lds((x_stream_fwd_kernel<XW, D, true>), attrc);
            MFVIT_LAUNCH((x_stream_fwd_kernel<XW, D, true>), dim3(B, ndir, nh / NH), dim3(XW * 64), lds, st, f_cxr, f_enh, params, L, eps_pre, scale,
                               B, T, ws + W.kq, ws + W.u, ws + W.a, ws + W.st);
        }
        MFVIT_CHECK_LAUNCH();
    }
    {
        GemmP p = zg();
        p.A = ws + W.u; p.lda = nh * D; p.W = params + L.ca[0] + L.wv; p.ldw = D; p.M = B; p.N = DH; p.K = D;
        p.out0 = ws + W.o; p.ldo0 = D;
        p.nb = ndir * nh; p.nbi = nh; p.sAo = (long)B * nh * D; p.sAi = D; p.sWo = L.ca_stride; p.sWi = (long)DH * D; p.sOo = (long)B * D; p.sOi = DH;
        FUS_TRY(gemm_nt_tile(MFVIT_F32, EPI_NONE, p, st));
    }
    {
        GemmP p = zg();
        p.A = ws + W.o; p.lda = D; p.W = params + L.ca[0] + L.wp; p.ldw = D; p.M = B; p.N = D; p.K = D;
        p.bias = params + L.ca[0] + L.bp;
        p.out0 = ws + W.outp; p.ldo0 = D;
        p.nb = ndir; p.nbi = 1; p.sAo = (long)B * D; p.sWo = L.ca_stride; p.sOo = (long)B * D; p.sBo = L.ca_stride;
        FUS_TRY(gemm_nt_tile(MFVIT_F32, EPI_BIAS, p, st));
    }
    return MFVIT_OK;
}

static int fus_prenorm_job(int D, int dir, const FusLayout& L, const FusWs& W, float* ws, int B, float* dparams, hipStream_t st) {
    if (L.no_norm) return MFVIT_OK;
    return colpart_reduce(ws + W.pd + (long)dir * 2 * B * 2 * D, 2 * B, D, 2, dparams + L.ca[dir] + L.n_w, dparams + L.ca[dir] + L.n_b, nullptr, st);
}

static int fus_wgrad(const GemmP& p, hipStream_t st) { return gemm_tn_small(p, st); }

template <int D>
static int xattn_core_backward(int ndir, int nh, const FusLayout& L, const FusWs& W, const float* params, const float* f_cxr,
                               const float* f_enh, float* ws, int B, int T, float* dparams, float* df_cxr, float* df_enh, hipStream_t st) {
    const int DH = D / nh;
    const float scale = 1.0f / sqrtf((float)DH);
    const float* wT = ws + W.wT;
    {
        GemmP p = zg();
        p.A = ws + W.dout; p.lda = D; p.W = ws + W.o; p.ldw = D; p.M = B; p.N = D; p.K = D;
        p.out0 = dparams + L.ca[0] + L.wp; p.ldo0 = D;
        p.nb = ndir; p.nbi = 1; p.sAo = (long)B * D; p.sWo = (long)B * D; p.sOo = L.ca_stride;
        FUS_TRY(fus_wgrad(p, st));
    }
    {
        GemmP p = zg();
        p.A = ws + W.dout; p.lda = D; p.W = wT + 3L * D * D; p.ldw = D; p.M = B; p.N = D; p.K = D;
        p.out0 = ws + W.dob; p.ldo0 = D;
        p.nb = ndir; p.nbi = 1; p.sAo = (long)B * D; p.sWo = 4L * D * D; p.sOo = (long)B * D;
        FUS_TRY(gemm_nt_tile(MFVIT_F32, EPI_NONE, p, st));
    }
    {
        GemmP p = zg();
        p.A = ws + W.dob; p.lda = D; p.W = ws + W.u; p.ldw = nh * D; p.M = B; p.N = DH; p.K = D;
        p.out0 = dparams + L.ca[0] + L.wv; p.ldo0 = D;
        p.nb = ndir * nh; p.nbi = nh; p.sAo = (long)B * D; p.sAi = DH; p.sWo = (long)B * nh * D; p.sWi = D; p.sOo = L.ca_stride; p.sOi = (long)DH * D;
        FUS_TRY(fus_wgrad(p, st));
    }
    {
        GemmP p = zg();
        p.A = ws + W.dob; p.lda = D; p.W = wT + 2L * D * D; p.ldw = D; p.M = B; p.N = D; p.K = DH;
        p.out0 = ws + W.du; p.ldo0 = nh * D;
        p.nb = ndir * nh; p.nbi = nh; p.sAo = (long)B * D; p.sAi = DH; p.sWo = 4L * D * D; p.sWi = DH; p.sOo = (long)B * nh * D; p.sOi = D;
        FUS_TRY(gemm_nt_tile(MFVIT_F32, EPI_NONE, p, st));
    }
    {
        const size_t lds = lds_stream_bwd(D, T);
        static PerDeviceOnce attr1, attrc, attrz;
        ProfScope ps(PROF_XATTN_BWD, 0, 2.0 * B * T * D * 4 * 3 * (nh == NH ? 1 : nh / NH + 1), st);
        if (nh == NH) {
            max_lds((x_stream_bwd_kernel<XW_BWD, D, false>), attr1);
            MFVIT_LAUNCH((x_stream_bwd_kernel<XW_BWD, D, false>), dim3(B, ndir), dim3(XW_BWD * 64), lds, st, f_cxr, f_enh, params, L, scale, B, T,
                               ws + W.kq, ws + W.a, ws + W.st, ws + W.du, ws + W.dkq, ws + W.dz0p, ws + W.pd, df_cxr, df_enh, nullptr);
            MFVIT_CHECK_LAUNCH();
        } else {
            max_lds((x_stream_bwd_kernel<XW_BWD, D, true>), attrc);
            MFVIT_LAUNCH((x_stream_bwd_kernel<XW_BWD, D, true>), dim3(B, ndir, nh / NH), dim3(XW_BWD * 64), lds, st, f_cxr, f_enh, params, L, scale,
                               B, T, ws + W.kq, ws + W.a, ws + W.st, ws + W.du, ws + W.dkq, ws + W.dz0p, ws + W.pd, df_cxr, df_enh, ws + W.ds);
            MFVIT_CHECK_LAUNCH();
            const size_t ldz = lds_stream_dz(D, T, nh);
            max_lds((x_stream_dz_kernel<XW_DZ, D>), attrz);
            MFVIT_LAUNCH((x_stream_dz_kernel<XW_DZ, D>), dim3(B, ndir), dim3(XW_DZ * 64), ldz, st, f_cxr, f_enh, params, L, scale, B, T, nh,
                               ws + W.kq, ws + W.a, ws + W.st, ws + W.du, ws + W.ds, ws + W.dz0p, ws + W.pd, df_cxr, df_enh);
            MFVIT_CHECK_LAUNCH();
        }
    }
    {
        GemmP p = zg();
        p.A = ws + W.qv; p.lda = D; p.W = ws + W.dkq; p.ldw = nh * D; p.M = B; p.N = DH; p.K = D;
        p.out0 = dparams + L.ca[0] + L.wk; p.ldo0 = D;
        p.nb = ndir * nh; p.nbi = nh; p.sAo = (long)B * D; p.sAi = DH; p.sWo = (long)B * nh * D; p.sWi = D; p.sOo = L.ca_stride; p.sOi = (long)DH * D;
        FUS_TRY(fus_wgrad(p, st));
    }
    {
        GemmP p = zg();
        p.A = ws + W.dkq; p.lda = nh * D; p.W = params + L.ca[0] + L.wk; p.ldw = D; p.M = B; p.N = DH; p.K = D;
        p.out0 = ws + W.dqv; p.ldo0 = D;
        p.nb = ndir * nh; p.nbi = nh; p.sAo = (long)B * nh * D; p.sAi = D; p.sWo = L.ca_stride; p.sWi = (long)DH * D; p.sOo = (long)B * D; p.sOi = DH;
        FUS_TRY(gemm_nt_tile(MFVIT_F32, EPI_NONE, p, st));
    }
    {
        GemmP p = zg();
        p.A = ws + W.dqv; p.lda = D; p.W = ws + W.z0; p.ldw = D; p.M = B; p.N = D; p.K = D;
        p.out0 = dparams + L.ca[0] + L.wq; p.ldo0 = D;
        p.nb = ndir; p.nbi = 1; p.sAo = (long)B * D; p.sWo = (long)B * D; p.sOo = L.ca_stride;
        FUS_TRY(fus_wgrad(p, st));
    }
    {
        GemmP p = zg();
        p.A = ws + W.dqv; p.lda = D; p.W = wT; p.ldw = D; p.M = B; p.N = D; p.K = D;
        p.out0 = ws + W.dz0q; p.ldo0 = D;
        p.nb = ndir; p.nbi = 1; p.sAo = (long)B * D; p.sWo = 4L * D * D; p.sOo = (long)B * D;
        FUS_TRY(gemm_nt_tile(MFVIT_F32, EPI_NONE, p, st));
    }
    MFVIT_LAUNCH(x_row0_bwd_kernel<D>, dim3(B), dim3(64 * ndir), 0, st, f_cxr, f_enh, params, L, B, T, ws + W.st0, ws + W.dz0p, ws + W.dz0q,
                       ws + W.dqp, ws + W.pd, df_cxr, df_enh);
    MFVIT_CHECK_LAUNCH();
    return MFVIT_OK;
}

template <int D>
static int fusion_forward(const mfvit_fusion_cfg* cfg, const float* params, const float* f_cxr, const float* f_enh, const float* hw_cxr,
                          const float* hb_cxr, const float* hw_enh, const float* hb_enh, float* ws, float* fused, float* x_cxr, float* x_enh,
                          hipStream_t st) {
    const int B = cfg->batch, T = cfg->tokens, C = cfg->num_classes;
    const FusLayout L = fus_layout(D, C);
// ... 298 lines not shown
```

### multi-feature-vit_amd/csrc/kernels.h

```cpp
#pragma once
#include "gemm.cuh"

#include <string.h>

namespace mfvit {

enum { EPI_BIAS = 0, EPI_BIAS_GELU = 1, EPI_GELU_BWD = 2, EPI_NONE = 3, EPI_BIAS_RELU = 4,
       EPI_BIAS_X3F16 = 5,
       EPI_BIAS_GELU_DROP = 6,
       EPI_COL2IM16 = 7 };
enum { REPI_RES_LN = 0, REPI_LNBWD_RES = 1,
       REPI_RES_LN_DP = 2 };

int gemm_nt_tile(int dtype, int epi, const GemmP& p, hipStream_t st);
bool gemm_nt_pp_supported(int dtype, int epi, const GemmP& p);
int gemm_nt_pp(int dtype, int epi, const GemmP& p, hipStream_t st);
int gemm_nt_row(int dtype, int repi, const GemmP& p, hipStream_t st);
bool gemm_nt_rowp_supported(int dtype, int repi, const GemmP& p);
int gemm_nt_rowp(int dtype, int repi, const GemmP& p, hipStream_t st);
int input_transform(const unsigned char* src, const long long* desc, const int* tables, int n, int S, int out_h, int out_w,
                    const float* mean, const float* stdv, float* out, hipStream_t st);
int input_transform_u8(const unsigned char* src, const long long* desc, const int* tables, int n, int S, unsigned* frames,
                       hipStream_t st);
size_t input_photometric_workspace_bytes(int n, int S);
int input_photometric(const unsigned char* src, const long long* desc, const int* tables, const int* photo, int n, int S, int max_radius,
                      void* workspace, const float* mean, const float* stdv, float* out, hipStream_t st);
int eval_counts(const float* scores, long ld, const int64_t* labels, int n, int C, unsigned long long* conf, unsigned long long* u2,
                unsigned long long* npos, int64_t* preds, hipStream_t st);
int gemm_tn(int dtype, const GemmP& p, hipStream_t st);
bool gemm_nt_small_supported(int dtype, int epi, const GemmP& p);
int gemm_nt_small(int epi, GemmP p, hipStream_t st);
bool gemm_tn_small_supported(int dtype, const GemmP& p);
int gemm_tn_small(GemmP p, hipStream_t st);
bool gemm_tn_glds_supported(int dtype, const GemmP& p);
int gemm_tn_glds(int dtype, GemmP p, hipStream_t st);
int colpart_reduce(const float* part, int G, int ncols, int nq, float* d0, float* d1, float* d2, hipStream_t st);
struct ColpartJob { const float* part; float* d[3]; int G, ncols, nq; };
struct ColpartBatch { static constexpr int MAXJ = 48; int n; ColpartJob job[MAXJ]; };
ColpartBatch* colpart_batch_begin(ColpartBatch* b);
int colpart_batch_flush(hipStream_t st);
bool gemm_tn_pair_supported(int dtype, const GemmP& a, const GemmP& b);
int gemm_tn_glds_pair(int dtype, GemmP a, const GemmP& b, hipStream_t st);
int tn_partial_reduce(const float* part, int splits, long stride, int N, int K, float* out, long ldo, hipStream_t st);
struct TnPartJob { const float* part; float* out; long stride, ldo; int splits, N, K; long first4; };
struct TnPartBatch { static constexpr int MAXJ = 56; int n; long total4; TnPartJob job[MAXJ]; };
TnPartBatch* tnpart_batch_begin(TnPartBatch* b);
int tnpart_batch_flush(hipStream_t st);

int attn_fwd_exact(int dtype, const void* qkv, void* out, float* lse, int B, int Tn, int H, int HD, hipStream_t st);
int attn_bwd_exact(int dtype, const void* qkv, const void* out, const void* dout, const float* lse, void* dqkv, float* dbias, int B, int Tn,
                   int H, int HD, hipStream_t st);

int attn_qkv_dtype(int dtype, int Tn, int HD);
int attn_fwd(int dtype, const void* qkv, void* out, float* lse, int B, int Tn, int H, int HD, hipStream_t st);
int attn_bwd(int dtype, const void* qkv, const void* out, const void* dout, const float* lse, void* dqkv, float* dbias, int B, int Tn,
             int H, int HD, hipStream_t st, const unsigned* domax = nullptr);

int im2col16(int dtype, const float* img, void* P, int B, int H, int W, hipStream_t st);
int ln_rows(int dtype, int N, const float* in0, long ld0, const float* in1, long ld1, int mod1, float* xout, long ldx, void* y, long ldy,
            int y_f32, const float* gamma, const float* beta, float eps, float* mean, float* rstd, int rows, int row_stride, int row_off,
            int in0_bcast, hipStream_t st);
int ln_bwd_rows(int dtype, int N, const float* dy, long lddy, const float* x, long ldx, const float* mean, const float* rstd,
                const float* gamma, const float* dres, long ldres, float* dx, long lddx, void* dxT, long lddxT, float* dgamma, float* dbeta,
                float* dcol, float* cpart, int rows, int row_stride, int row_off, hipStream_t st, const void* dyT = nullptr, long lddyT = 0);
int add_ln_rows(int dtype, int N, const void* tin, long ldt, const float* pos, long ldp, int pmod, const float* res, long ldres, int rin, int rout,
                int roff, float* xout, long ldx, void* y, long ldy, int y_f32, const float* gamma, const float* beta, float eps, float* mean,
                float* rstd, int rows, hipStream_t st);
int cast_transpose(int dtype, const float* src, void* dst, void* dstT, int R, int C, hipStream_t st);
int cast_transpose_batched(int dtype, const float* src, void* dst, void* dstT, int R, int C, int nb, long s_src, long s_dst, long s_dstT,
                           hipStream_t st);
int linear_small_fwd(const float* x, long ldx, const float* W, const float* b, float* y, long ldy, int M, int N, int K, int accumulate,
                     hipStream_t st);
int linear_small_bwd(const float* dy, long lddy, const float* x, long ldx, const float* W, float* dx, long lddx, int dx_accumulate, float* dW,
                     float* db, int M, int N, int K, hipStream_t st);
int ce_small(const float* logits, const long* target, float* loss_mean, float* dlogits, long* preds, int B, int C, hipStream_t st);
int add_rows(float* dst, long ldd, const float* src, long lds_, int rows, int N, hipStream_t st);
int axpy(float* y, const float* x, float a, long n, hipStream_t st);
int colsum_rows(const float* x, long ld, float* out, int rows, int row_stride, int row_off, int N, hipStream_t st);
int batch_sum(const float* x, float* out, int B, long n, hipStream_t st);

int attn_fwd_tiled_drop(int dtype, const void* qkv, void* out, float* lse, int B, int Tn, int H, int HDim, DropP drop, hipStream_t st);
int attn_bwd_tiled_drop(int dtype, const void* qkv, const void* out, const void* dout, const float* lse, void* dqkv, int B, int Tn, int H, int HDim,
                        DropP drop, hipStream_t st);
bool attn_tiled_supported(int dtype, int Tn, int HDim);
int dropout_mask(DropP drop, long n, unsigned char* out, hipStream_t st);
int drop_add_ln_rows(int dtype, int N, const void* tin, long ldt, const float* a0, long lda0, const float* a1, long lda1, int mod1,
                     const float* res, long ldres, DropP drop, DropP dpath, int tpr, float* xout, long ldx, void* y, long ldy, int y_f32,
                     const float* gamma, const float* beta, float eps, float* mean, float* rstd, int rows, hipStream_t st);
int mask_scale_rows(int dtype, bool f32, const void* src, long lds_, void* dst, long ldd, DropP drop, DropP dpath, int tpr, int rows, int N,
                    hipStream_t st);
int attn_probs(int qdt, const void* qkv, const float* lse, int B, int Tn, int H, int HD, int fuse, int cls_only, float* out, float* sums,
               hipStream_t st);
int attn_rollout(const float* maps, const float* sums, int depth, int B, int Tn, float* out, hipStream_t st);
int attn_rel_map(int qdt, int ddt, const void* qkv, const float* lse, const void* dout, int B, int Tn, int H, int HD, float* map, const float* v,
                 float* part, int first, hipStream_t st);
int attn_rel_update(float* v, const float* part, int B, int Tn, int first, float* out, hipStream_t st);

inline GemmP nt(const void* A, long lda, const void* W, long ldw, int M, int N, int K) {
    GemmP p;
    memset(&p, 0, sizeof(p));
    p.A = A; p.lda = lda; p.W = W; p.ldw = ldw;
    p.M = M; p.N = N; p.K = K;
    return p;
}
}

#define MFVIT_TRY(expr)            \
    do {                           \
        int rc__ = (expr);         \
        if (rc__ != MFVIT_OK) return rc__; \
    } while (0)
```

### multi-feature-vit_amd/csrc/vit.hip

```cpp
#include "../../include/mfvit.h"
#include "kernels.h"
#include "prof.h"

#include <atomic>
#include <stdlib.h>

using namespace mfvit;

namespace mfvit {
static std::atomic<int> g_stream_share{1};
static thread_local int t_stream_share = 0;
int stream_share() { return t_stream_share > 0 ? t_stream_share : g_stream_share.load(std::memory_order_relaxed); }
namespace {
struct ShareScope {
    int prev;
    explicit ShareScope(const mfvit_vit_cfg* cfg) : prev(t_stream_share) { if (cfg && cfg->stream_share > 0) t_stream_share = cfg->stream_share > 8 ? 8 : cfg->stream_share; }
    ~ShareScope() { t_stream_share = prev; }
};
}
}

namespace {

inline size_t align256(size_t x) { return (x + 255) & ~(size_t)255; }
// ... 236 lines not shown
    float* xbuf(int l) const { return (float*)(ws + W.x0 + slot(l) * W.x_stride); }
    float* stat(int l) const { return (float*)(ws + W.st0 + slot(l) * W.st_stride); }
    char* blk(int l) const { return ws + W.blk0 + slot(l) * W.blk_stride; }
    const float* pblk(int l) const { return params + L.blk0 + (long)l * L.blk_stride; }
    const char* sblk(int l) const { return sh + S.blk0 + (size_t)l * S.blk_stride; }
    float* kpart() const { return (float*)(ws + W.kpart); }
    const void* weight(const char* shadow_w, const float* arena_w) const { return hw ? (const void*)shadow_w : (const void*)arena_w; }
    static unsigned site(int l, int which) { return 16u * (unsigned)l + (unsigned)which; }
    DropP dpath(int l, int which) const { return make_drop(d.dpr ? d.dpr[l] : 0.f, d.seed, site(l, which)); }
};

struct BranchDrop { DropP drop, dpath; };

GemmP operands_of(const GemmP& p) {
    GemmP q = nt(p.A, p.lda, p.W, p.ldw, p.M, p.N, p.K);
    q.bias = p.bias;
    return q;
}

int linear_res_ln(const EncCtx& c, const GemmP& p, const BranchDrop* mask, int tag) {
    const Dims& d = c.d;
    const long De = c.D * c.e;
    const bool masked = mask && d.rdrop;
    if (masked && !(d.p_resid > 0.f) && !d.unfused) {
        GemmP r = p;
        r.aux = p.res; r.ldaux = p.ldres; r.res = nullptr; r.ldres = 0;
        r.drop = mask->dpath; r.drop_tpr = d.T;
        ProfTag scope(tag);
        if (gemm_nt_rowp_supported(d.dtype, REPI_RES_LN_DP, r)) return gemm_nt_rowp(d.dtype, REPI_RES_LN_DP, r, c.st);
    }
    if (masked || d.unfused) {
        GemmP q = operands_of(p);
        q.out0 = c.ws + (masked ? c.W.dtmp : c.W.utmp); q.ldo0 = De;
        MFVIT_TRY(gemm_nt_tile(d.dtype, EPI_BIAS, q, c.st));
        if (masked)
            return drop_add_ln_rows(d.dtype, d.D, q.out0, De, nullptr, 0, nullptr, 0, 0, p.res, p.ldres, mask->drop, mask->dpath, d.T, (float*)p.out0,
                                    p.ldo0, p.out1, p.ldo1, p.y_f32, p.gamma, p.beta, p.eps, p.mean, p.rstd, p.M, c.st);
        const bool table = p.res_mod != 0;
        return add_ln_rows(d.dtype, d.D, q.out0, De, table ? p.res : nullptr, table ? p.ldres : 0, table ? p.orow_out : 0, table ? nullptr : p.res,
                           table ? 0 : p.ldres, p.orow_in, p.orow_out, p.orow_off, (float*)p.out0, p.ldo0, p.out1, p.ldo1, p.y_f32, p.gamma, p.beta,
                           p.eps, p.mean, p.rstd, p.M, c.st);
    }
    ProfTag scope(tag);
    return gemm_nt_row(d.dtype, REPI_RES_LN, p, c.st);
}

int dgrad_ln_bwd(const EncCtx& c, GemmP p, const float* res, const void* res_t, float* dx, void* dx_t) {
    const Dims& d = c.d;
    const long D = c.D, De = c.D * c.e;
    if (d.unfused) {
        GemmP q = operands_of(p);
        q.out0 = c.ws + c.W.utmp; q.ldo0 = De;
        MFVIT_TRY(gemm_nt_tile(d.dtype, EPI_NONE, q, c.st));
        return ln_bwd_rows(d.dtype, d.D, nullptr, 0, (const float*)p.aux, p.ldaux, p.mean, p.rstd, p.gamma, res, D, dx, D, dx_t, De, p.cs0, p.cs1,
                           p.cs2, p.cpart, p.M, 1, 0, c.st, q.out0, De);
    }
    if (c.lean_grad) { p.res_t = res_t; p.ldres_t = De; }
    else { p.res = res; p.ldres = D; }
    p.out0 = dx; p.ldo0 = D; p.out1 = dx_t; p.ldo1 = De;
    return gemm_nt_row(d.dtype, REPI_LNBWD_RES, p, c.st);
}

struct SideStream {
    hipStream_t owner = nullptr;
    hipStream_t s = nullptr;
    hipEvent_t in = nullptr, end = nullptr;
    hipEvent_t done[64] = {};
    bool ok = false;
};
std::atomic<int> g_wgrad_stream{1};
SideStream& side_stream(hipStream_t caller) {
    static thread_local SideStream ss[8];
    static thread_local int used = 0;
    SideStream* px = nullptr;
    for (int i = 0; i < used; ++i)
        if (ss[i].owner == caller) px = &ss[i];
    if (!px) {
        px = &ss[used < 8 ? used++ : 7];
        if (px->owner != caller && px->s) return *px;
        px->owner = caller;
    }
    SideStream& x = *px;
    if (!x.s) {
        if (hipStreamCreateWithFlags(&x.s, hipStreamNonBlocking) == hipSuccess &&
            hipEventCreateWithFlags(&x.in, hipEventDisableTiming) == hipSuccess &&
            hipEventCreateWithFlags(&x.end, hipEventDisableTiming) == hipSuccess) {
            x.ok = true;
            for (auto& e : x.done) x.ok = x.ok && hipEventCreateWithFlags(&e, hipEventDisableTiming) == hipSuccess;
        }
        if (!x.ok && !x.s) x.s = (hipStream_t)-1;
    }
    return x;
}

}

extern "C" {

int mfvit_abi_version(void) { return 5; }
int mfvit_set_stream_share(int n) {
    mfvit::g_stream_share.store(n < 1 ? 1 : (n > 8 ? 8 : n), std::memory_order_relaxed);
    return MFVIT_OK;
}
int mfvit_set_wgrad_stream(int enabled) {
    g_wgrad_stream.store(enabled ? 1 : 0, std::memory_order_relaxed);
    return MFVIT_OK;
}
const char* mfvit_build_info(void) { return "libmfvit_hip gfx950 (MFMA bf16 | split-bf16 x3 | f16 32x32x16, f32 32x32x2), wave64, abi 5"; }

size_t mfvit_vit_param_count(const mfvit_vit_cfg* cfg) {
    Dims d;
    if (!get_dims(cfg, d)) return 0;
    return (size_t)param_layout(d).total;
}
int mfvit_vit_param_layout(const mfvit_vit_cfg* cfg, int64_t out[9]) {
    Dims d;
    if (!get_dims(cfg, d) || !out) return MFVIT_EINVAL;
    const ParamLayout L = param_layout(d);
    out[0] = L.cls; out[1] = L.pos; out[2] = L.pe_w; out[3] = L.pe_b; out[4] = L.blk0; out[5] = L.blk_stride;
    out[6] = L.norm_w; out[7] = L.norm_b; out[8] = L.total;
    return MFVIT_OK;
}
size_t mfvit_vit_shadow_bytes(const mfvit_vit_cfg* cfg) {
    Dims d;
    if (!get_dims(cfg, d)) return 0;
    return shadow_layout(d).total;
}
size_t mfvit_vit_workspace_bytes(const mfvit_vit_cfg* cfg) {
    Dims d;
    if (!get_dims(cfg, d)) return 0;
    return ws_layout(d).total;
}
size_t mfvit_vit_workspace_bytes_drop(const mfvit_vit_cfg* cfg, const mfvit_vit_drop* drop) {
    Dims d;
    if (!get_dims(cfg, drop, d)) return 0;
    return ws_layout(d).total;
}
size_t mfvit_vit_workspace_bytes_ex(const mfvit_vit_cfg* cfg, const mfvit_vit_drop* drop, int want_dimg) {
    Dims d;
    if (!get_dims(cfg, drop, d)) return 0;
    if (!want_dimg) return ws_layout(d).total;
    if (d.tok || !d.save) return 0;
    return ws_layout(d).total_dimg;
}

int mfvit_vit_prepare_shadow(const mfvit_vit_cfg* cfg, const float* params, void* shadow, mfvit_stream_t stream) {
    Dims d;
    if (!get_dims(cfg, d) || !params || !shadow) return MFVIT_EINVAL;
    hipStream_t st = (hipStream_t)stream;
    const ParamLayout L = param_layout(d);
    const ShadowLayout S = shadow_layout(d);
    char* sh = (char*)shadow;
    const bool hw = d.dtype != MFVIT_F32;
    if (hw && !d.tok) MFVIT_TRY(cast_transpose(d.dtype, params + L.pe_w, sh + S.pe_w, nullptr, d.D, 768, st));
    const float* pb = params + L.blk0;
    char* sb = sh + S.blk0;
    const long ss = L.blk_stride, sd = (long)S.blk_stride;
    MFVIT_TRY(cast_transpose_batched(d.dtype, pb + L.qkv_w, hw ? sb + S.qkv_w : nullptr, sb + S.qkv_t, 3 * d.D, d.D, d.depth, ss, sd, sd, st));
    MFVIT_TRY(cast_transpose_batched(d.dtype, pb + L.proj_w, hw ? sb + S.proj_w : nullptr, sb + S.proj_t, d.D, d.D, d.depth, ss, sd, sd, st));
    MFVIT_TRY(cast_transpose_batched(d.dtype, pb + L.fc1_w, hw ? sb + S.fc1_w : nullptr, sb + S.fc1_t, d.F, d.D, d.depth, ss, sd, sd, st));
    MFVIT_TRY(cast_transpose_batched(d.dtype, pb + L.fc2_w, hw ? sb + S.fc2_w : nullptr, sb + S.fc2_t, d.D, d.F, d.depth, ss, sd, sd, st));
    return MFVIT_OK;
}

}

static bool attn_req_ok(const mfvit_vit_cfg* cfg, const mfvit_vit_attn_req* r, Dims& d) {
    if (!r || !get_dims(cfg, d) || d.tok) return false;
    if (d.depth < 64 && (r->blocks >> d.depth) != 0) return false;
    if (r->fuse < 0 || r->fuse > 3 || (r->cls_only != 0 && r->cls_only != 1)) return false;
    if (r->rollout && (r->fuse == 0 || 2 * (size_t)d.T * 4 > 64 * 1024)) return false;
    if ((r->blocks != 0) != (r->maps != nullptr)) return false;
    return r->blocks != 0 || r->rollout != nullptr;
}
static float* attn_scratch_sums(const Dims& d, const mfvit_vit_attn_req* r) { return (float*)r->scratch + (size_t)d.depth * d.B * d.T * d.T; }
static int attn_block_step(const Dims& d, const mfvit_vit_attn_req* r, int l, int qdt, const void* qkv, const float* lse, hipStream_t st) {
    if ((r->blocks >> l) & 1) {
        const size_t slot = __builtin_popcountll(r->blocks & ((1ull << l) - 1));
        const size_t per = (size_t)d.B * (r->fuse ? 1 : d.H) * (r->cls_only ? 1 : d.T) * d.T;
        MFVIT_TRY(attn_probs(qdt, qkv, lse, d.B, d.T, d.H, d.HD, r->fuse, r->cls_only, r->maps + slot * per, nullptr, st));
    }
    if (r->rollout)
        MFVIT_TRY(attn_probs(qdt, qkv, lse, d.B, d.T, d.H, d.HD, r->fuse, 0, (float*)r->scratch + (size_t)l * d.B * d.T * d.T,
                             attn_scratch_sums(d, r) + (size_t)l * d.B * d.T, st));
    return MFVIT_OK;
}

static bool rel_req_ok(const mfvit_vit_cfg* cfg, const mfvit_vit_rel_req* r, Dims& d) {
    if (!r || !get_dims(cfg, d) || d.tok || !d.save || d.T > 8192) return false;
    if (d.depth < 64 && (r->blocks >> d.depth) != 0) return false;
    if ((r->blocks != 0) != (r->maps != nullptr)) return false;
    return r->blocks != 0 || r->relevance != nullptr;
}
static int rel_block_step(const Dims& d, const mfvit_vit_rel_req* r, int l, int qdt, const void* qkv, const float* lse, const void* dout,
                          hipStream_t st) {
    const bool sel = (r->blocks >> l) & 1;
    if (!sel && !r->relevance) return MFVIT_OK;
    float* map = nullptr;
    if (sel) map = r->maps + (size_t)__builtin_popcountll(r->blocks & ((1ull << l) - 1)) * d.B * d.T * d.T;
    float* v = r->relevance ? (float*)r->scratch : nullptr;
    float* part = r->relevance ? v + (size_t)d.B * d.T : nullptr;
    const int first = l == d.depth - 1;
    MFVIT_TRY(attn_rel_map(qdt, d.dtype, qkv, lse, dout, d.B, d.T, d.H, d.HD, map, v, part, first, st));
    if (r->relevance) MFVIT_TRY(attn_rel_update(v, part, d.B, d.T, first, l == 0 ? r->relevance : nullptr, st));
    return MFVIT_OK;
}

static int encoder_forward(const mfvit_vit_cfg* cfg, const mfvit_vit_drop* dropcfg, const float* params, const void* shadow, const float* img,
                           void* workspace, float* features, mfvit_stream_t stream, bool want_tokens,
                           const mfvit_vit_attn_req* attn = nullptr) {
    Dims d;
    if (!get_dims(cfg, dropcfg, d) || !params || !shadow || !img || !workspace || !features) return MFVIT_EINVAL;
    if (d.tok != want_tokens) return MFVIT_EINVAL;
    const EncCtx c(cfg, d, params, shadow, workspace, stream);
    const ParamLayout& L = c.L;
    const ShadowLayout& S = c.S;
    const WsLayout& W = c.W;
    char* const ws = c.ws;
    const hipStream_t st = c.st;
    const long D = c.D, F = c.F, e = c.e;
    const float eps = c.eps;
    float* const x0 = c.xbuf(0);
    char* const y1_0 = c.blk(0) + W.y1;
    const float* const g0 = c.pblk(0) + L.ln1_w;
    const float* const b0 = c.pblk(0) + L.ln1_b;
    float* const mean0 = c.stat(0);
    float* const rstd0 = c.stat(0) + d.M;
    if (d.tok && d.p_embd > 0.f) {
        MFVIT_TRY(drop_add_ln_rows(d.dtype, d.D, nullptr, 0, img, D, d.use_pos ? params + L.pos : nullptr, D, d.T, nullptr, 0,
                                   make_drop(d.p_embd, d.seed, 1), c.off, 1, x0, D, y1_0, D * e, 0, g0, b0, eps, mean0, rstd0, d.M, st));
    } else if (d.tok) {
        MFVIT_TRY(ln_rows(d.dtype, d.D, img, D, d.use_pos ? params + L.pos : nullptr, D, d.T, x0, D, y1_0, D * e, 0, g0, b0, eps, mean0, rstd0, d.M,
                          1, 0, 0, st));
    } else {
        MFVIT_TRY(im2col16(d.dtype, img, ws + W.patches, d.B, cfg->img_h, cfg->img_w, st));
        GemmP p = nt(ws + W.patches, 768 * e, c.weight(c.sh + S.pe_w, params + L.pe_w), 768 * e, d.Mp, d.D, 768);
        p.bias = params + L.pe_b;
        p.res = params + L.pos; p.ldres = D; p.res_mod = d.np; p.res_off = 1;
        p.orow_in = d.np; p.orow_out = d.T; p.orow_off = 1;
        p.out0 = x0; p.ldo0 = D;
        p.out1 = y1_0; p.ldo1 = D * e;
        p.gamma = g0; p.beta = b0; p.eps = eps;
        p.mean = mean0; p.rstd = rstd0;
        MFVIT_TRY(linear_res_ln(c, p, nullptr, PROF_TAG_NONE));
        MFVIT_TRY(ln_rows(d.dtype, d.D, params + L.cls, 0, params + L.pos, D, 1, x0, D, y1_0, D * e, 0, g0, b0, eps, mean0, rstd0, d.B, d.T, 0, 1, st));
        if (d.p_embd > 0.f)
            MFVIT_TRY(drop_add_ln_rows(d.dtype, d.D, nullptr, 0, x0, D, nullptr, 0, 0, nullptr, 0, make_drop(d.p_embd, d.seed, 1), c.off, 1, x0, D,
                                       y1_0, D * e, 0, g0, b0, eps, mean0, rstd0, d.M, st));
    }

    for (int l = 0; l < d.depth; ++l) {
        char* b = c.blk(l);
        const float* pb = c.pblk(l);
        const char* sb = c.sblk(l);
        const int qdt = d.p_attn > 0.f ? d.dtype : attn_qkv_dtype(d.dtype, d.T, d.HD);
        {
            GemmP p = nt(b + W.y1, D * e, c.weight(sb + S.qkv_w, pb + L.qkv_w), D * e, d.M, 3 * d.D, d.D);
            p.bias = pb + L.qkv_b;
            p.out0 = b + W.qkv; p.ldo0 = 3 * D * e;
            ProfTag tag(PROF_TAG_MHSA_QKV);
            MFVIT_TRY(gemm_nt_tile(d.dtype, qdt == MFVIT_X3F16 ? EPI_BIAS_X3F16 : EPI_BIAS, p, st));
        }
        if (d.p_attn > 0.f) {
            if (!attn_tiled_supported(d.dtype, d.T, d.HD)) return MFVIT_ENOSYS;
            MFVIT_TRY(attn_fwd_tiled_drop(d.dtype, b + W.qkv, b + W.attn, (float*)(b + W.lse), d.B, d.T, d.H, d.HD,
                                          make_drop(d.p_attn, d.seed, c.site(l, 2)), st));
        } else {
            MFVIT_TRY(attn_fwd(qdt, b + W.qkv, b + W.attn, (float*)(b + W.lse), d.B, d.T, d.H, d.HD, st));
        }
        if (attn) MFVIT_TRY(attn_block_step(d, attn, l, qdt, b + W.qkv, (const float*)(b + W.lse), st));
        {
            GemmP p = nt(b + W.attn, D * e, c.weight(sb + S.proj_w, pb + L.proj_w), D * e, d.M, d.D, d.D);
            p.bias = pb + L.proj_b;
            p.res = c.xbuf(l); p.ldres = D;
            p.out0 = b + W.xmid; p.ldo0 = D;
            p.out1 = b + W.y2; p.ldo1 = D * e;
            p.gamma = pb + L.ln2_w; p.beta = pb + L.ln2_b; p.eps = eps;
            p.mean = (float*)(b + W.st2); p.rstd = (float*)(b + W.st2) + d.M;
            p.kpart = c.kpart();
            const BranchDrop mask = {make_drop(d.p_resid, d.seed, c.site(l, 3)), c.dpath(l, 6)};
            MFVIT_TRY(linear_res_ln(c, p, &mask, PROF_TAG_MHSA_PROJ));
        }
        {
            GemmP p = nt(b + W.y2, D * e, c.weight(sb + S.fc1_w, pb + L.fc1_w), D * e, d.M, d.F, d.D);
            p.bias = pb + L.fc1_b;
            p.out0 = d.save ? b + W.hpre : nullptr; p.ldo0 = F;
            p.out1 = b + W.hact; p.ldo1 = F * e;
            p.drop = make_drop(d.p_gelu, d.seed, c.site(l, 5));
            MFVIT_TRY(gemm_nt_tile(d.dtype, d.act == 1 ? EPI_BIAS_RELU : (d.p_gelu > 0.f ? EPI_BIAS_GELU_DROP : EPI_BIAS_GELU), p, st));
        }
        {
            const bool last = l + 1 == d.depth;
            GemmP p = nt(b + W.hact, F * e, c.weight(sb + S.fc2_w, pb + L.fc2_w), F * e, d.M, d.D, d.F);
            p.bias = pb + L.fc2_b;
            p.res = (const float*)(b + W.xmid); p.ldres = D;
            p.out0 = c.xbuf(l + 1); p.ldo0 = D;
            if (last) {
                p.out1 = features; p.ldo1 = D; p.y_f32 = 1;
                p.gamma = params + L.norm_w; p.beta = params + L.norm_b;
            } else {
                p.out1 = c.blk(l + 1) + W.y1; p.ldo1 = D * e;
                p.gamma = c.pblk(l + 1) + L.ln1_w; p.beta = c.pblk(l + 1) + L.ln1_b;
            }
            p.eps = eps;
            p.mean = c.stat(l + 1); p.rstd = c.stat(l + 1) + d.M;
            p.kpart = c.kpart();
            const BranchDrop mask = {make_drop(d.p_resid, d.seed, c.site(l, 4)), c.dpath(l, 7)};
            MFVIT_TRY(linear_res_ln(c, p, &mask, PROF_TAG_NONE));
        }
    }
    return MFVIT_OK;
}

static int encoder_backward(const mfvit_vit_cfg* cfg, const mfvit_vit_drop* dropcfg, const float* params, const void* shadow, void* workspace,
// ... 65 lines not shown
    }
    for (int s = stage_hi; s >= stage_lo; --s) {
        if (s == d.depth) {
            if (!dfeatures) return MFVIT_EINVAL;
            float* const dcol = !wg ? nullptr : rdrop ? colscr + D : gblk(d.depth - 1) + L.fc2_b;
            MFVIT_TRY(ln_bwd_rows(d.dtype, d.D, dfeatures, D, c.xbuf(d.depth), D, c.stat(d.depth), c.stat(d.depth) + d.M, params + L.norm_w,
                                  nullptr, 0, gx, D, pp(W.gxT, d.depth - 1), D * e, wg ? dparams + L.norm_w : nullptr,
                                  wg ? dparams + L.norm_b : nullptr, dcol, wg ? next_colpart() : nullptr, d.M, 1, 0, st));
        } else if (s >= 0) {
            const int l = s;
            char* b = c.blk(l);
            const float* pb = c.pblk(l);
            float* gb = gblk(l);
            const char* sb = c.sblk(l);
            void* gxT = pp(W.gxT, l);
            void* gmidT = pp(W.gmidT, l);
            void* dhpre = pp(W.dhpre, l);
            void* dqkv = pp(W.dqkv, l);
            MFVIT_TRY(wait_layer(l + 2));
            GemmP def_tn[2];
            int ndef = 0;
            auto tn_now_or_later = [&](const GemmP& g) -> int {
                if (use_side) { def_tn[ndef++] = g; return MFVIT_OK; }
                return gemm_tn(d.dtype, g, wst);
            };
            const void* gy2 = gxT;
            if (rdrop) {
                MFVIT_TRY(mask_scale_rows(d.dtype, false, gxT, D * e, ws + W.dtmp, D * e, make_drop(d.p_resid, d.seed, c.site(l, 4)), c.dpath(l, 7), d.T,
                                          d.M, d.D, st));
                gy2 = ws + W.dtmp;
            }
            if (wg) {
                GemmP p = nt(gy2, D * e, b + W.hact, F * e, d.M, d.D, d.F);
                if (rdrop) p.cs0 = gb + L.fc2_b;
                p.out0 = gb + L.fc2_w; p.ldo0 = F;
                p.cpart = next_tnpart();
                MFVIT_TRY(tn_now_or_later(p));
            }
            {
                GemmP p = nt(gy2, D * e, sb + S.fc2_t, D * e, d.M, d.F, d.D);
                p.aux = b + W.hpre; p.ldaux = F;
                p.out0 = dhpre; p.ldo0 = F * e;
                if (wg) { p.cs0 = gb + L.fc1_b; p.cpart = next_colpart(); }
                MFVIT_TRY(gemm_nt_tile(d.dtype, EPI_GELU_BWD, p, st));
            }
            if (wg) {
                GemmP p = nt(dhpre, F * e, b + W.y2, D * e, d.M, d.F, d.D);
                p.out0 = gb + L.fc1_w; p.ldo0 = D;
                p.cpart = next_tnpart();
                MFVIT_TRY(tn_now_or_later(p));
            }
            {
                GemmP p = nt(dhpre, F * e, sb + S.fc1_t, F * e, d.M, d.D, d.F);
                p.aux = b + W.xmid; p.ldaux = D;
                p.mean = (float*)(b + W.st2); p.rstd = (float*)(b + W.st2) + d.M;
                p.gamma = pb + L.ln2_w;
                p.kpart = c.kpart();
                if (wg) { p.cs0 = gb + L.ln2_w; p.cs1 = gb + L.ln2_b; p.cs2 = rdrop ? colscr + D : gb + L.proj_b; p.cpart = next_colpart(); }
                MFVIT_TRY(dgrad_ln_bwd(c, p, gx, gxT, lean_grad ? nullptr : gmid, gmidT));
            }
            const void* gyp = gmidT;
            if (rdrop) {
                MFVIT_TRY(mask_scale_rows(d.dtype, false, gmidT, D * e, ws + W.dtmp, D * e, make_drop(d.p_resid, d.seed, c.site(l, 3)), c.dpath(l, 6), d.T,
                                          d.M, d.D, st));
                gyp = ws + W.dtmp;
            }
            GemmP pend_proj = {};
            bool have_pend = false;
            if (wg) {
                GemmP p = nt(gyp, D * e, b + W.attn, D * e, d.M, d.D, d.D);
                if (rdrop) p.cs0 = gb + L.proj_b;
                p.out0 = gb + L.proj_w; p.ldo0 = D;
                p.cpart = next_tnpart();
                if (!rdrop) {
                    pend_proj = p;
                    have_pend = true;
                } else {
                    MFVIT_TRY(gemm_tn(d.dtype, p, wst));
                }
            }
            {
                GemmP p = nt(gyp, D * e, sb + S.proj_t, D * e, d.M, d.D, d.D);
                p.out0 = ws + W.dattn; p.ldo0 = D * e;
                if (do_max) { p.omax = domax(l); p.omax_rows = d.T; p.omax_hd = d.HD; }
                MFVIT_TRY(gemm_nt_tile(d.dtype, EPI_NONE, p, st));
            }
            if (rel && l == 0) {
                MFVIT_TRY(rel_block_step(d, rel, l, qdt_bwd, b + W.qkv, (const float*)(b + W.lse), ws + W.dattn, st));
                continue;
            }
            if (d.p_attn > 0.f)
                MFVIT_TRY(attn_bwd_tiled_drop(d.dtype, b + W.qkv, b + W.attn, ws + W.dattn, (const float*)(b + W.lse), dqkv, d.B, d.T, d.H, d.HD,
                                              make_drop(d.p_attn, d.seed, c.site(l, 2)), st));
            else
            MFVIT_TRY(attn_bwd(qdt_bwd, b + W.qkv, b + W.attn, ws + W.dattn, (const float*)(b + W.lse), dqkv, nullptr,
                               d.B, d.T, d.H, d.HD, st, do_max ? domax(l) : nullptr));
            if (rel) MFVIT_TRY(rel_block_step(d, rel, l, qdt_bwd, b + W.qkv, (const float*)(b + W.lse), ws + W.dattn, st));
            MFVIT_TRY(fork());
            for (int i = 0; i < ndef; ++i) MFVIT_TRY(gemm_tn(d.dtype, def_tn[i], wst));
            if (wg) {
                GemmP p = nt(dqkv, 3 * D * e, b + W.y1, D * e, d.M, 3 * d.D, d.D);
                p.cs0 = gb + L.qkv_b;
                p.out0 = gb + L.qkv_w; p.ldo0 = D;
                p.cpart = next_tnpart();
                GemmP pend_nc = pend_proj;
                pend_nc.cpart = nullptr;
                if (have_pend && gemm_tn_pair_supported(d.dtype, p, pend_nc)) {
                    MFVIT_TRY(gemm_tn_glds_pair(d.dtype, p, pend_nc, wst));
                } else {
                    if (have_pend) MFVIT_TRY(gemm_tn(d.dtype, pend_proj, wst));
                    MFVIT_TRY(gemm_tn(d.dtype, p, wst));
                }
            }
            MFVIT_TRY(tnpart_batch_flush(wst));
            tn_used = 0;
            if (use_side && hipEventRecord(ss.done[l & 63], ss.s) != hipSuccess) return MFVIT_ELAUNCH;
            MFVIT_TRY(wait_layer(l + 1));
            {
                if (wg && l == 0 && hipMemsetAsync(colscr, 0, 2 * D * sizeof(float), st) != hipSuccess) return MFVIT_ELAUNCH;
                GemmP p = nt(dqkv, 3 * D * e, sb + S.qkv_t, 3 * D * e, d.M, d.D, 3 * d.D);
                p.aux = c.xbuf(l); p.ldaux = D;
                p.mean = c.stat(l); p.rstd = c.stat(l) + d.M;
                p.gamma = pb + L.ln1_w;
                p.kpart = c.kpart();
                if (wg) { p.cs0 = gb + L.ln1_w; p.cs1 = gb + L.ln1_b; p.cs2 = (l > 0 && !rdrop) ? gblk(l - 1) + L.fc2_b : colscr; p.cpart = next_colpart(); }
                MFVIT_TRY(dgrad_ln_bwd(c, p, gmid, gmidT, lean_grad && l > 0 ? nullptr : gx, pp(W.gxT, l - 1)));
            }
        } else if (d.tok) {
            MFVIT_TRY(colpart_batch_flush(st));
            if (d.p_embd > 0.f)
                MFVIT_TRY(mask_scale_rows(d.dtype, true, gx, D, gx, D, make_drop(d.p_embd, d.seed, 1), c.off, 1, d.M, d.D, st));
            if (dinput && hipMemcpyAsync(dinput, gx, (size_t)d.M * D * sizeof(float), hipMemcpyDeviceToDevice, st) != hipSuccess)
                return MFVIT_ELAUNCH;
            if (d.use_pos) MFVIT_TRY(batch_sum(gx, dparams + L.pos, d.B, (long)d.T * D, st));
        } else {
            MFVIT_TRY(colpart_batch_flush(st));
            if (d.p_embd > 0.f) {
                MFVIT_TRY(mask_scale_rows(d.dtype, true, gx, D, gx, D, make_drop(d.p_embd, d.seed, 1), c.off, 1, d.M, d.D, st));
                MFVIT_TRY(cast_transpose(d.dtype, gx, pp(W.gxT, -1), nullptr, d.M, d.D, st));
                if (wg) {
                    if (hipMemsetAsync(colscr, 0, D * sizeof(float), st) != hipSuccess) return MFVIT_ELAUNCH;
                    MFVIT_TRY(colsum_rows(gx, D, colscr, d.M, 1, 0, d.D, st));
                }
            }
            if (dimg) {
                char* wpeT = ws + W.wpeT;
                MFVIT_TRY(cast_transpose(d.dtype, params + L.pe_w, nullptr, wpeT, d.D, 768, st));
                GemmP p = nt((const char*)pp(W.gxT, -1) + (size_t)D * d.es, D * e, wpeT, D * e, d.M - 1, 768, d.D);
                p.orow_in = d.np; p.orow_out = d.T;
                p.out0 = dimg; p.ldo0 = cfg->img_w;
                MFVIT_TRY(gemm_nt_tile(d.dtype, EPI_COL2IM16, p, st));
            }
            if (!wg) continue;
            MFVIT_TRY(colsum_rows(gx, D, dparams + L.cls, d.B, d.T, 0, d.D, st));
            if (!cfg->stop_grad_conv1) {
                MFVIT_TRY(colsum_rows(gx, D, colscr + D, d.B, d.T, 0, d.D, st));
                MFVIT_TRY(axpy(dparams + L.pe_b, colscr, 1.0f, d.D, st));
                MFVIT_TRY(axpy(dparams + L.pe_b, colscr + D, -1.0f, d.D, st));
                GemmP p = nt(pp(W.gxT, -1), D * e, ws + W.patches, 768 * e, d.Mp, d.D, 768);
                p.orow_in = d.np; p.orow_out = d.T; p.orow_off = 1;
                p.out0 = dparams + L.pe_w; p.ldo0 = 768;
                p.cpart = next_tnpart();
                MFVIT_TRY(fork());
                MFVIT_TRY(gemm_tn(d.dtype, p, wst));
            }
        }
    }
    MFVIT_TRY(colpart_batch_flush(st));
    MFVIT_TRY(tnpart_batch_flush(wst));
    if (use_side) {
        if (hipEventRecord(ss.end, ss.s) != hipSuccess || hipStreamWaitEvent(st, ss.end, 0) != hipSuccess) return MFVIT_ELAUNCH;
    }
    return MFVIT_OK;
}

extern "C" {

int mfvit_vit_forward(const mfvit_vit_cfg* cfg, const float* params, const void* shadow, const float* img, void* workspace,
                      float* features, mfvit_stream_t stream) {
    ShareScope share(cfg);
    return encoder_forward(cfg, nullptr, params, shadow, img, workspace, features, stream, false);
}
int mfvit_vit_forward_drop(const mfvit_vit_cfg* cfg, const mfvit_vit_drop* drop, const float* params, const void* shadow, const float* img,
                           void* workspace, float* features, mfvit_stream_t stream) {
    if (!drop) return MFVIT_EINVAL;
    ShareScope share(cfg);
    return encoder_forward(cfg, drop, params, shadow, img, workspace, features, stream, false);
}
size_t mfvit_vit_attn_scratch_bytes(const mfvit_vit_cfg* cfg, const mfvit_vit_attn_req* req) {
    Dims d;
    if (!attn_req_ok(cfg, req, d)) return 0;
    return req->rollout ? align256((size_t)d.depth * d.B * d.T * (d.T + 1) * 4) : 256;
}
int mfvit_vit_forward_attn(const mfvit_vit_cfg* cfg, const mfvit_vit_attn_req* req, const float* params, const void* shadow, const float* img,
                           void* workspace, float* features, mfvit_stream_t stream) {
    Dims d;
    if (!attn_req_ok(cfg, req, d) || !req->scratch) return MFVIT_EINVAL;
    ShareScope share(cfg);
    MFVIT_TRY(encoder_forward(cfg, nullptr, params, shadow, img, workspace, features, stream, false, req));
    if (req->rollout) MFVIT_TRY(attn_rollout((const float*)req->scratch, attn_scratch_sums(d, req), d.depth, d.B, d.T, req->rollout, (hipStream_t)stream));
    return MFVIT_OK;
}
size_t mfvit_vit_rel_scratch_bytes(const mfvit_vit_cfg* cfg, const mfvit_vit_rel_req* req) {
    Dims d;
    if (!rel_req_ok(cfg, req, d)) return 0;
    return req->relevance ? align256((size_t)d.B * d.T * ((d.T + 31) / 32 + 1) * 4) : 256;
}
int mfvit_vit_backward_rel(const mfvit_vit_cfg* cfg, const mfvit_vit_rel_req* req, const float* params, const void* shadow, void* workspace,
                           const float* dfeatures, mfvit_stream_t stream) {
    Dims d;
    if (!rel_req_ok(cfg, req, d) || !req->scratch || !dfeatures || !params || !shadow || !workspace) return MFVIT_EINVAL;
    ShareScope share(cfg);
    return encoder_backward(cfg, nullptr, params, shadow, workspace, dfeatures, nullptr, nullptr, nullptr, d.depth, 0, stream, false, req);
}
int mfvit_vit_backward(const mfvit_vit_cfg* cfg, const float* params, const void* shadow, void* workspace, const float* dfeatures,
                       float* dparams, int stage_hi, int stage_lo, mfvit_stream_t stream) {
    if (!dparams) return MFVIT_EINVAL;
    ShareScope share(cfg);
    return encoder_backward(cfg, nullptr, params, shadow, workspace, dfeatures, dparams, nullptr, nullptr, stage_hi, stage_lo, stream, false);
}
int mfvit_vit_backward_ex(const mfvit_vit_cfg* cfg, const mfvit_vit_drop* drop, const float* params, const void* shadow, void* workspace,
                          const float* dfeatures, float* dparams, float* dimg, int stage_hi, int stage_lo, mfvit_stream_t stream) {
    ShareScope share(cfg);
    return encoder_backward(cfg, drop, params, shadow, workspace, dfeatures, dparams, nullptr, dimg, stage_hi, stage_lo, stream, false);
}
int mfvit_vit_backward_drop(const mfvit_vit_cfg* cfg, const mfvit_vit_drop* drop, const float* params, const void* shadow, void* workspace,
                            const float* dfeatures, float* dparams, int stage_hi, int stage_lo, mfvit_stream_t stream) {
    if (!drop || !dparams) return MFVIT_EINVAL;
    ShareScope share(cfg);
    return encoder_backward(cfg, drop, params, shadow, workspace, dfeatures, dparams, nullptr, nullptr, stage_hi, stage_lo, stream, false);
}
int mfvit_gpt_forward(const mfvit_vit_cfg* cfg, const float* params, const void* shadow, const float* tokens, void* workspace, float* out,
                      mfvit_stream_t stream) {
    ShareScope share(cfg);
    return encoder_forward(cfg, nullptr, params, shadow, tokens, workspace, out, stream, true);
}
int mfvit_gpt_backward(const mfvit_vit_cfg* cfg, const float* params, const void* shadow, void* workspace, const float* dout, float* dparams,
                       float* dtokens, mfvit_stream_t stream) {
    if (!cfg || !dtokens || !dout) return MFVIT_EINVAL;
    ShareScope share(cfg);
    if (!dparams) return MFVIT_EINVAL;
    return encoder_backward(cfg, nullptr, params, shadow, workspace, dout, dparams, dtokens, nullptr, cfg->depth, -1, stream, true);
}

}
```

### multi-feature-vit_amd/mfvit/_lib.py

```python
import ctypes
import os

import torch
from ctypes import POINTER, Structure, c_char_p, c_double, c_float, c_int, c_int64, c_size_t, c_uint32, c_uint64, c_void_p

_HERE = os.path.dirname(os.path.abspath(__file__))
LIB_PATH = os.environ.get("MFVIT_LIB") or os.path.join(_HERE, "libmfvit_hip.so")
ABI_VERSION = 5

F32, BF16, BF16X3, F16, X3F16 = 0, 1, 2, 3, 4
EPI_BIAS, EPI_BIAS_GELU, EPI_NONE, EPI_BIAS_X3F16 = 0, 1, 3, 5


class VitCfg(Structure):
    _fields_ = [("dtype", c_int), ("batch", c_int), ("img_h", c_int), ("img_w", c_int), ("dim", c_int), ("depth", c_int),
                ("heads", c_int), ("mlp_dim", c_int), ("save_for_backward", c_int), ("stop_grad_conv1", c_int),
                ("ln_eps", c_float), ("token_input", c_int), ("tokens", c_int), ("use_pos", c_int), ("act", c_int),
                ("p_embd", c_float), ("p_attn", c_float), ("p_resid", c_float), ("seed_lo", c_uint32), ("seed_hi", c_uint32),
                ("stream_share", c_int)]


class VitDrop(Structure):
    _fields_ = [("drop", c_float), ("attn_drop", c_float), ("drop_path", POINTER(c_float)), ("seed", c_uint64)]


class VitAttnReq(Structure):
    _fields_ = [("blocks", c_uint64), ("fuse", c_int), ("cls_only", c_int), ("maps", c_void_p), ("rollout", c_void_p), ("scratch", c_void_p)]


HEAD_FUSION = {None: 0, "mean": 1, "max": 2, "min": 3}


class VitRelReq(Structure):
    _fields_ = [("blocks", c_uint64), ("maps", c_void_p), ("relevance", c_void_p), ("scratch", c_void_p)]


class FusionCfg(Structure):
    _fields_ = [("batch", c_int), ("tokens", c_int), ("dim", c_int), ("heads", c_int), ("num_classes", c_int),
                ("eps_pre", c_float), ("eps_post", c_float)]


P = c_void_p
I = c_int
L = c_int64
F = c_float
D = c_double

SIGNATURES = {
    "mfvit_abi_version": (I, []),
    "mfvit_build_info": (c_char_p, []),
    "mfvit_vit_param_count": (c_size_t, [POINTER(VitCfg)]),
    "mfvit_vit_param_layout": (I, [POINTER(VitCfg), POINTER(c_int64)]),
    "mfvit_vit_shadow_bytes": (c_size_t, [POINTER(VitCfg)]),
    "mfvit_vit_prepare_shadow": (I, [POINTER(VitCfg), P, P, P]),
    "mfvit_vit_workspace_bytes": (c_size_t, [POINTER(VitCfg)]),
    "mfvit_vit_forward": (I, [POINTER(VitCfg), P, P, P, P, P, P]),
    "mfvit_vit_backward": (I, [POINTER(VitCfg), P, P, P, P, P, I, I, P]),
    "mfvit_vit_workspace_bytes_drop": (c_size_t, [POINTER(VitCfg), POINTER(VitDrop)]),
    "mfvit_vit_forward_drop": (I, [POINTER(VitCfg), POINTER(VitDrop), P, P, P, P, P, P]),
    "mfvit_vit_backward_drop": (I, [POINTER(VitCfg), POINTER(VitDrop), P, P, P, P, P, I, I, P]),
    "mfvit_vit_workspace_bytes_ex": (c_size_t, [POINTER(VitCfg), POINTER(VitDrop), I]),
    "mfvit_vit_backward_ex": (I, [POINTER(VitCfg), POINTER(VitDrop), P, P, P, P, P, P, I, I, P]),
    "mfvit_vit_attn_scratch_bytes": (c_size_t, [POINTER(VitCfg), POINTER(VitAttnReq)]),
    "mfvit_vit_forward_attn": (I, [POINTER(VitCfg), POINTER(VitAttnReq), P, P, P, P, P, P]),
    "mfvit_vit_rel_scratch_bytes": (c_size_t, [POINTER(VitCfg), POINTER(VitRelReq)]),
    "mfvit_vit_backward_rel": (I, [POINTER(VitCfg), POINTER(VitRelReq), P, P, P, P, P]),
    "mfvit_gpt_forward": (I, [POINTER(VitCfg), P, P, P, P, P, P]),
    "mfvit_gpt_backward": (I, [POINTER(VitCfg), P, P, P, P, P, P, P]),
    "mfvit_linear_fwd": (I, [I, I, P, L, P, L, P, P, L, P, L, I, I, I, P]),
    "mfvit_linear_dgrad_act": (I, [I, P, L, P, L, P, L, P, L, I, I, I, P]),
    "mfvit_linear_wgrad": (I, [I, P, L, P, L, P, L, I, I, I, P]),
    "mfvit_linear_wgrad_ws": (I, [I, P, L, P, L, P, L, I, I, I, P, P]),
    "mfvit_linear_wgrad_pair": (I, [I, P, L, P, L, P, L, P, I, P, L, P, L, P, L, I, I, I, P]),
    "mfvit_linear_res_ln_fwd": (I, [I, P, L, P, L, P, P, L, P, P, I, P, P, F, P, P, I, I, P]),
    "mfvit_linear_dgrad_ln_bwd": (I, [I, P, L, P, L, P, P, P, P, P, P, P, P, P, P, I, I, P]),
    "mfvit_linear_res_ln_fwd_ws": (I, [I, P, L, P, L, P, P, L, P, P, I, P, P, F, P, P, I, I, P, P]),
    "mfvit_linear_dgrad_ln_bwd_ws": (I, [I, P, L, P, L, P, P, P, P, P, P, P, P, P, P, I, I, P, P]),
    "mfvit_attention_fwd": (I, [I, P, P, P, I, I, I, I, P]),
    "mfvit_attention_bwd": (I, [I, P, P, P, P, P, P, I, I, I, I, P]),
    "mfvit_attention_qkv_dtype": (I, [I, I, I]),
    "mfvit_attention_drop_fwd": (I, [I, P, P, P, I, I, I, I, F, c_uint64, c_uint32, P]),
    "mfvit_attention_drop_bwd": (I, [I, P, P, P, P, P, I, I, I, I, F, c_uint64, c_uint32, P]),
    "mfvit_dropout_mask": (I, [F, c_uint64, c_uint32, L, P, P]),
    "mfvit_layernorm_fwd": (I, [I, P, P, I, P, P, F, P, P, I, I, P]),
    "mfvit_layernorm_bwd": (I, [I, P, P, P, P, P, P, P, P, P, P, P, I, I, P]),
    "mfvit_cast_transpose": (I, [I, P, P, P, I, I, P]),
    "mfvit_head_fwd": (I, [P, L, P, P, P, L, I, I, I, I, P]),
    "mfvit_head_bwd": (I, [P, L, P, L, P, P, L, I, P, P, I, I, I, P]),
    "mfvit_cross_entropy": (I, [P, P, P, P, P, I, I, P]),
    "mfvit_cross_entropy_soft": (I, [P, P, P, P, F, P, P, P, I, I, P]),
    "mfvit_batch_mix": (I, [P, P, P, P, P, P, I, I, I, I, P]),
    "mfvit_fusion_param_count": (c_size_t, [POINTER(FusionCfg)]),
    "mfvit_fusion_workspace_bytes": (c_size_t, [POINTER(FusionCfg)]),
    "mfvit_fusion_forward": (I, [POINTER(FusionCfg), P, P, P, P, P, P, P, P, P, P, P, P]),
    "mfvit_fusion_ex_param_count": (c_size_t, [POINTER(FusionCfg), I, I]),
    "mfvit_fusion_ex_workspace_bytes": (c_size_t, [POINTER(FusionCfg), I, I]),
    "mfvit_fusion_ex_forward": (I, [POINTER(FusionCfg), I, I, P, P, P, P, P, P, P, P, P, P, P, P]),
    "mfvit_fusion_ex_backward": (I, [POINTER(FusionCfg), I, I, P, P, P, P, P, P, P, P, P, P, P, P, P, P, P, P, P]),
    "mfvit_fusion_ex_attention": (I, [POINTER(FusionCfg), I, I, P, I, I, P, P]),
    "mfvit_fusion_ex_grad_attention": (I, [POINTER(FusionCfg), I, I, P, P, P, P, I, P, P]),
    "mfvit_bimodal_relevance_scratch_bytes": (c_size_t, [I, I]),
    "mfvit_bimodal_relevance": (I, [I, I, I, I, P, P, P, P, P, P]),
    "mfvit_bn_stats": (I, [I, P, I, I, P, P, P]),
    "mfvit_bn_combine": (I, [P, P, P, I, I, F, F, P, P, P, P, P]),
    "mfvit_bn_apply": (I, [I, P, P, P, P, P, I, P, I, I, P]),
    "mfvit_bn_bwd_sums": (I, [I, P, P, P, P, P, I, I, I, P, P, P]),
    "mfvit_bn_bwd_apply": (I, [I, P, P, P, P, P, P, I, P, P, F, P, I, I, P]),
    "mfvit_l2norm_fwd": (I, [P, P, P, I, I, F, P]),
    "mfvit_l2norm_bwd": (I, [P, P, P, P, I, I, P]),
    "mfvit_rowdot": (I, [P, P, P, L, F, I, I, P]),
    "mfvit_cross_entropy_rows": (I, [P, L, P, P, P, P, L, I, I, P]),
    "mfvit_ema_update": (I, [P, P, F, L, P]),
    "mfvit_lars_step": (I, [P, I, I, P, F, F, F, F, P]),
    "mfvit_adam_step": (I, [P, I, F, F, F, F, F, I, P]),
    "mfvit_sgd_step": (I, [P, I, F, F, F, I, P]),
    "mfvit_amp_unscale": (I, [P, I, F, P, P]),
    "mfvit_grad_norm_partials": (I, [P, I, I, P, P]),
    "mfvit_grad_clip_coef": (I, [P, P, I, I, I, D, P, P, P]),
    "mfvit_grad_scale": (I, [P, I, P, P]),
    "mfvit_prenorm_xattn_forward": (I, [POINTER(FusionCfg), P, P, P, P, P, P]),
    "mfvit_prenorm_xattn_backward": (I, [POINTER(FusionCfg), P, P, P, P, P, P, P, P, P]),
    "mfvit_xattn_forward": (I, [POINTER(FusionCfg), P, P, P, P, P]),
    "mfvit_xattn_backward": (I, [POINTER(FusionCfg), P, P, P, P, P, P, P]),
    "mfvit_input_transform": (I, [P, P, P, I, I, I, P, P, P, P]),
    "mfvit_input_transform_rect": (I, [P, P, P, I, I, I, I, P, P, P, P]),
    "mfvit_input_photometric_workspace_bytes": (c_size_t, [I, I]),
    "mfvit_input_photometric": (I, [P, P, P, P, I, I, I, P, P, P, P, P]),
    "mfvit_eval_counts": (I, [P, L, P, I, I, P, P, P, P, P]),
    "mfvit_patch_rank": (I, [P, L, P, I, I, P]),
    "mfvit_patch_perturb": (I, [P, P, P, P, P, I, I, I, I, I, P]),
    "mfvit_perturb_score": (I, [P, L, P, I, I, I, P, P, P, P]),
    "mfvit_attr_inputs": (I, [P, P, I, P, P, P, I, P, I, I, I, L, P]),
    "mfvit_attr_accumulate": (I, [P, P, P, I, I, L, I, P]),
    "mfvit_attr_finish": (I, [P, P, P, I, I, I, P, P, P, I, I, I, I, P]),
    "mfvit_prof_enable": (I, [I]),
    "mfvit_set_wgrad_stream": (I, [I]),
    "mfvit_set_stream_share": (I, [I]),
    "mfvit_prof_collect": (I, [POINTER(ctypes.c_double), I]),
    "mfvit_prof_collect_tags": (I, [POINTER(ctypes.c_double), I]),
    "mfvit_prof_class_name": (c_char_p, [I]),
    "mfvit_fusion_backward": (I, [POINTER(FusionCfg), P, P, P, P, P, P, P, P, P, P, P, P, P, P, P, P, P]),
}

_lib = None


class MfvitError(RuntimeError):
    pass


def lib():
    global _lib
    if _lib is not None:
        return _lib
    if not os.path.exists(LIB_PATH):
        raise MfvitError(
            f"libmfvit_hip.so not found at {LIB_PATH}. Build it with `python -c 'import __graft_entry__ as g; g.build()'` "
            "(hipcc --offload-arch=gfx950). There is no CPU/eager fallback for the MF-ViT hot path.")
    try:
        h = ctypes.CDLL(LIB_PATH)
    except OSError as e:
        raise MfvitError(f"cannot load {LIB_PATH}: {e}") from e
    abi = h.mfvit_abi_version()
    if abi != ABI_VERSION:
        raise MfvitError(f"{LIB_PATH} has C ABI {abi}, this package expects ABI {ABI_VERSION}: rebuild the library")
    for name, (res, args) in SIGNATURES.items():
        fn = getattr(h, name)
        fn.restype = res
        fn.argtypes = args
    _lib = h
    return h


def source_hash():
    import hashlib
    h = hashlib.sha1()
    csrc = os.path.join(os.path.dirname(_HERE), "csrc")
    files = sorted(os.path.join(csrc, f) for f in os.listdir(csrc) if f.endswith((".hip", ".cuh", ".h")))
    files.append(os.path.join(os.path.dirname(os.path.dirname(_HERE)), "include", "mfvit.h"))
    for f in files:
        h.update(os.path.basename(f).encode())
        with open(f, "rb") as fh:
            h.update(fh.read())
    return h.hexdigest()


def check(rc, what):
    if rc != 0:
        raise MfvitError(f"{what} failed with code {rc} (-22 = invalid argument, -5 = launch error, -38 = not built for this dtype / size)")


def ptr(t):
    return None if t is None else t.data_ptr()


def stream():
    import torch
    return torch.cuda.current_stream().cuda_stream


def require_cuda(*tensors):
    for t in tensors:
        if t is not None and not t.is_cuda:
            raise MfvitError("MF-ViT HIP ops need tensors on a ROCm GPU ('cuda' device); there is no CPU fallback")


PRECISIONS = ("bf16x3", "bf16", "fp16", "fp32")


def dtype_code(precision):
    if precision in ("bf16x3", "split", "split-bf16"):
        return BF16X3
    if precision in ("bf16", "bfloat16"):
        return BF16
    if precision in ("fp16", "f16", "float16", "half"):
        return F16
    if precision in ("fp32", "f32", "float32"):
        return F32
    raise ValueError(f"precision must be one of {PRECISIONS}, got {precision!r}")
```

### multi-feature-vit_amd/mfvit/ops.py

```python
import torch

from . import _lib
from ._lib import BF16, BF16X3, EPI_BIAS, EPI_BIAS_GELU, EPI_BIAS_X3F16, EPI_NONE, F16, F32, X3F16, check, lib, ptr, require_cuda, stream

_TORCH_OF = {BF16: torch.bfloat16, BF16X3: torch.bfloat16, F16: torch.float16, F32: torch.float32}


def _tdtype(code):
    return _TORCH_OF[code]


def _code_of(t, split=False):
    if t.dtype == torch.bfloat16:
        return BF16X3 if split else BF16
    if t.dtype == torch.float16 and not split:
        return F16
    if t.dtype == torch.float32 and not split:
        return F32
    raise _lib.MfvitError(f"unsupported dtype {t.dtype}{' for a split tensor' if split else ''}")


def split_pack(x):
    x = x.float()
    hi = x.to(torch.bfloat16)
# ... 82 lines not shown
        if scratch.dtype != torch.float32 or scratch.numel() < WGRAD_SCRATCH_FLOATS:
            raise _lib.MfvitError("wgrad scratch must be float32 with at least WGRAD_SCRATCH_FLOATS elements")
        check(lib().mfvit_linear_wgrad_ws(code, ptr(dy), dy.stride(0), ptr(x), x.stride(0), ptr(out), out.stride(0), M, N, K,
                                          ptr(scratch), stream()), "mfvit_linear_wgrad_ws")
    else:
        check(lib().mfvit_linear_wgrad(code, ptr(dy), dy.stride(0), ptr(x), x.stride(0), ptr(out), out.stride(0), M, N, K, stream()),
              "mfvit_linear_wgrad")
    return out


def linear_wgrad_pair(dy_a, x_a, dy_b, x_b, want_dbias=True, split=False):
    require_cuda(dy_a, x_a, dy_b, x_b)
    code = _code_of(dy_a, split)
    e = 2 if split else 1
    M, Na, Nb = dy_a.shape[0], dy_a.shape[1] // e, dy_b.shape[1] // e
    K = x_a.shape[1] // e
    if dy_b.shape[0] != M or x_a.shape[0] != M or x_b.shape[0] != M or x_b.shape[1] // e != K:
        raise _lib.MfvitError("linear_wgrad_pair: the two GEMMs must share M and K")
    dw_a = torch.zeros(Na, K, device=dy_a.device, dtype=torch.float32)
    dw_b = torch.zeros(Nb, K, device=dy_a.device, dtype=torch.float32)
    db_a = torch.zeros(Na, device=dy_a.device, dtype=torch.float32) if want_dbias else None
    check(lib().mfvit_linear_wgrad_pair(code, ptr(dy_a), dy_a.stride(0), ptr(x_a), x_a.stride(0), ptr(dw_a), dw_a.stride(0), ptr(db_a), Na,
                                        ptr(dy_b), dy_b.stride(0), ptr(x_b), x_b.stride(0), ptr(dw_b), dw_b.stride(0), Nb, M, K, stream()),
          "mfvit_linear_wgrad_pair")
    return dw_a, db_a, dw_b


ROWP_SCRATCH_FLOATS = 264 * 7 * 12 * 512


def linear_res_ln_fwd(a, w, bias, res, gamma, beta, eps, y_f32=False, split=False, scratch=None):
    require_cuda(a, w, res)
    code = _code_of(a, split)
    e = 2 if split else 1
    M, K = a.shape[0], a.shape[1] // e
    x_out = torch.empty(M, 384, device=a.device, dtype=torch.float32)
    y = torch.empty(M, 384 if y_f32 else 384 * e, device=a.device, dtype=torch.float32 if y_f32 else a.dtype)
    mean = torch.empty(M, device=a.device, dtype=torch.float32)
    rstd = torch.empty_like(mean)
    check(lib().mfvit_linear_res_ln_fwd_ws(code, ptr(a), a.stride(0), ptr(w), w.stride(0), ptr(bias), ptr(res),
                                           res.stride(0) if res is not None else 0, ptr(x_out), ptr(y), int(y_f32), ptr(gamma),
                                           ptr(beta), eps, ptr(mean), ptr(rstd), M, K, ptr(scratch), stream()), "mfvit_linear_res_ln_fwd_ws")
    return x_out, y, mean, rstd


def linear_dgrad_ln_bwd(dy, wt, x, mean, rstd, gamma, dres, want_copy=True, split=False, scratch=None):
    require_cuda(dy, wt, x)
    code = _code_of(dy, split)
    e = 2 if split else 1
    M, K = dy.shape[0], dy.shape[1] // e
    dx = torch.empty(M, 384, device=dy.device, dtype=torch.float32)
    dx_t = torch.empty(M, 384 * e, device=dy.device, dtype=dy.dtype) if want_copy else None
    dgamma = torch.zeros(384, device=dy.device, dtype=torch.float32)
    dbeta = torch.zeros_like(dgamma)
    dcol = torch.zeros_like(dgamma)
    check(lib().mfvit_linear_dgrad_ln_bwd_ws(code, ptr(dy), dy.stride(0), ptr(wt), wt.stride(0), ptr(x), ptr(mean), ptr(rstd),
                                             ptr(gamma), ptr(dres), ptr(dx), ptr(dx_t), ptr(dgamma), ptr(dbeta), ptr(dcol), M, K,
                                             ptr(scratch), stream()), "mfvit_linear_dgrad_ln_bwd_ws")
    return dx, dx_t, dgamma, dbeta, dcol


def _attn_code(qkv, split):
    if split and qkv.dtype == torch.float16:
        return X3F16, torch.bfloat16
    return _code_of(qkv, split), qkv.dtype


def attention_fwd(qkv, heads, split=False):
    require_cuda(qkv)
    code, odt = _attn_code(qkv, split)
    e = 2 if split else 1
    B, T, D3 = qkv.shape
    D = D3 // (3 * e)
    out = torch.empty(B, T, D * e, device=qkv.device, dtype=odt)
    lse = torch.empty(B, heads, T, device=qkv.device, dtype=torch.float32)
    check(lib().mfvit_attention_fwd(code, ptr(qkv), ptr(out), ptr(lse), B, T, heads, D // heads, stream()), "mfvit_attention_fwd")
    return out, lse


def attention_bwd(qkv, out, dout, lse, heads, want_dbias=True, split=False):
    require_cuda(qkv, out, dout, lse)
    code, odt = _attn_code(qkv, split)
    e = 2 if split else 1
    B, T, D3 = qkv.shape
    D = D3 // (3 * e)
    dqkv = torch.empty(qkv.shape, device=qkv.device, dtype=odt)
    dbias = torch.zeros(3 * D, device=qkv.device, dtype=torch.float32) if want_dbias else None
    check(lib().mfvit_attention_bwd(code, ptr(qkv), ptr(out), ptr(dout), ptr(lse), ptr(dqkv), ptr(dbias), B, T, heads, D // heads,
                                    stream()), "mfvit_attention_bwd")
    return dqkv, dbias


def attention_drop_fwd(qkv, heads, p, seed, site, split=False):
    require_cuda(qkv)
    code = _code_of(qkv, split)
    e = 2 if split else 1
    B, T, D3 = qkv.shape
    D = D3 // (3 * e)
    out = torch.empty(B, T, D * e, device=qkv.device, dtype=qkv.dtype)
    lse = torch.empty(B, heads, T, device=qkv.device, dtype=torch.float32)
    check(lib().mfvit_attention_drop_fwd(code, ptr(qkv), ptr(out), ptr(lse), B, T, heads, D // heads, float(p), int(seed), int(site), stream()),
          "mfvit_attention_drop_fwd")
    return out, lse


def attention_drop_bwd(qkv, out, dout, lse, heads, p, seed, site, split=False):
    require_cuda(qkv, out, dout, lse)
    code, odt = _attn_code(qkv, split)
    e = 2 if split else 1
    B, T, D3 = qkv.shape
    D = D3 // (3 * e)
    dqkv = torch.empty(qkv.shape, device=qkv.device, dtype=odt)
    check(lib().mfvit_attention_drop_bwd(code, ptr(qkv), ptr(out), ptr(dout), ptr(lse), ptr(dqkv), B, T, heads, D // heads, float(p), int(seed),
                                         int(site), stream()), "mfvit_attention_drop_bwd")
    return dqkv


def dropout_mask(p, seed, site, n, device="cuda:0"):
    keep = torch.empty(n, device=device, dtype=torch.uint8)
    check(lib().mfvit_dropout_mask(float(p), int(seed), int(site), n, ptr(keep), stream()), "mfvit_dropout_mask")
    return keep.bool()


def _code_of_dtype(dt, split=False):
    if dt == torch.bfloat16:
        return BF16X3 if split else BF16
    return F16 if dt == torch.float16 else F32


def layernorm_fwd(x, gamma, beta, eps, out_dtype=torch.float32, split=False):
    require_cuda(x, gamma, beta)
    rows, N = x.shape
    y = torch.empty(rows, N * (2 if split else 1), device=x.device, dtype=out_dtype)
    mean = torch.empty(rows, device=x.device, dtype=torch.float32)
    rstd = torch.empty_like(mean)
    code = _code_of_dtype(out_dtype, split)
    check(lib().mfvit_layernorm_fwd(code, ptr(x), ptr(y), int(out_dtype == torch.float32), ptr(gamma), ptr(beta), eps, ptr(mean),
                                    ptr(rstd), rows, N, stream()), "mfvit_layernorm_fwd")
    return y, mean, rstd


def layernorm_bwd(dy, x, mean, rstd, gamma, dres=None, copy_dtype=None, split=False):
    require_cuda(dy, x)
    rows, N = x.shape
    dx = torch.empty_like(x)
    dx_t = torch.empty(rows, N * (2 if split else 1), device=x.device, dtype=copy_dtype) if copy_dtype is not None else None
    dgamma = torch.zeros(N, device=x.device, dtype=torch.float32)
    dbeta = torch.zeros_like(dgamma)
    dcol = torch.zeros_like(dgamma)
    code = _code_of_dtype(copy_dtype, split)
    check(lib().mfvit_layernorm_bwd(code, ptr(dy), ptr(x), ptr(mean), ptr(rstd), ptr(gamma), ptr(dres), ptr(dx), ptr(dx_t), ptr(dgamma),
                                    ptr(dbeta), ptr(dcol), rows, N, stream()), "mfvit_layernorm_bwd")
    return dx, dx_t, dgamma, dbeta, dcol


def cast_transpose(src, dtype, want_straight=True, want_transposed=True, split=False):
    require_cuda(src)
    R, C = src.shape
    code = _code_of_dtype(dtype, split)
    e = 2 if split else 1
    dst = torch.empty(R, C * e, device=src.device, dtype=dtype) if want_straight else None
    dst_t = torch.empty(C, R * e, device=src.device, dtype=dtype) if want_transposed else None
    check(lib().mfvit_cast_transpose(code, ptr(src), ptr(dst), ptr(dst_t), R, C, stream()), "mfvit_cast_transpose")
    return dst, dst_t


def head_fwd(x, w, b, ldx=None, out=None, accumulate=False):
    require_cuda(x, w, b)
    N, K = w.shape
    if ldx is None:
        ldx = x.stride(0)
    M = x.shape[0]
    if out is None:
        out = torch.empty(M, N, device=x.device, dtype=torch.float32)
    check(lib().mfvit_head_fwd(ptr(x), ldx, ptr(w), ptr(b), ptr(out), out.stride(0), M, N, K, int(accumulate), stream()),
          "mfvit_head_fwd")
    return out


def head_bwd(dy, x, w, ldx=None, dx=None, lddx=None, dx_accumulate=False, dw=None, db=None):
    require_cuda(dy, x, w)
    N, K = w.shape
    M = dy.shape[0]
    if ldx is None:
        ldx = x.stride(0)
    if dx is not None and lddx is None:
        lddx = dx.stride(0)
    check(lib().mfvit_head_bwd(ptr(dy), dy.stride(0), ptr(x), ldx, ptr(w), ptr(dx), lddx or 0, int(dx_accumulate), ptr(dw), ptr(db),
                               M, N, K, stream()), "mfvit_head_bwd")
    return dx, dw, db


def cross_entropy(logits, target, want_grad=True):
    require_cuda(logits, target)
    B, C = logits.shape
    loss = torch.empty(1, device=logits.device, dtype=torch.float32)
    dlogits = torch.empty_like(logits) if want_grad else None
    preds = torch.empty(B, device=logits.device, dtype=torch.int64)
    check(lib().mfvit_cross_entropy(ptr(logits), ptr(target), ptr(loss), ptr(dlogits), ptr(preds), B, C, stream()),
          "mfvit_cross_entropy")
    return loss, dlogits, preds


def cross_entropy_soft(logits, target, partner=None, lam=None, smoothing=0.0, want_grad=True):
    require_cuda(logits, target, partner, lam)
    if logits.dim() != 2 or logits.dtype != torch.float32 or not logits.is_contiguous():
        raise _lib.MfvitError("cross_entropy_soft: logits must be a contiguous f32 [B][C] tensor")
    B, C = logits.shape
    if target.shape != (B,) or target.dtype != torch.int64 or not target.is_contiguous():
        raise _lib.MfvitError(f"cross_entropy_soft: target must be a contiguous int64 [{B}] tensor")
    if (partner is None) != (lam is None):
        raise _lib.MfvitError("cross_entropy_soft: partner and lam come together")
    if partner is not None:
        if partner.shape != (B,) or partner.dtype != torch.int32 or not partner.is_contiguous():
            raise _lib.MfvitError(f"cross_entropy_soft: partner must be a contiguous int32 [{B}] tensor")
        if lam.shape != (B,) or lam.dtype != torch.float32 or not lam.is_contiguous():
            raise _lib.MfvitError(f"cross_entropy_soft: lam must be a contiguous f32 [{B}] tensor")
    if not 0.0 <= float(smoothing) < 1.0:
        raise ValueError(f"smoothing must lie in [0, 1), got {smoothing}")
    loss = torch.empty(1, device=logits.device, dtype=torch.float32)
    dlogits = torch.empty_like(logits) if want_grad else None
    preds = torch.empty(B, device=logits.device, dtype=torch.int64)
    check(lib().mfvit_cross_entropy_soft(ptr(logits), ptr(target), ptr(partner), ptr(lam), float(smoothing), ptr(loss), ptr(dlogits), ptr(preds),
                                         B, C, stream()), "mfvit_cross_entropy_soft")
    return loss, dlogits, preds


def batch_mix(a, desc, lam, b=None):
    require_cuda(a, desc, lam, b)
    if a.dim() != 4 or a.dtype != torch.float32 or not a.is_contiguous():
        raise _lib.MfvitError("batch_mix: the batch must be a contiguous f32 [n][C][H][W] tensor")
    if b is not None and (b.shape != a.shape or b.dtype != torch.float32 or not b.is_contiguous()):
        raise _lib.MfvitError(f"batch_mix: the second stream must be a contiguous f32 tensor of the first one's shape {tuple(a.shape)}, got {tuple(b.shape)}")
    n, C, H, W = a.shape
    if desc.shape != (n, 12) or desc.dtype != torch.int32 or not desc.is_contiguous():
        raise _lib.MfvitError(f"batch_mix: desc must be a contiguous int32 [{n}][12] tensor")
    if lam.shape != (n,) or lam.dtype != torch.float32 or not lam.is_contiguous():
        raise _lib.MfvitError(f"batch_mix: lam must be a contiguous f32 [{n}] tensor")
    out_a = torch.empty_like(a)
    out_b = torch.empty_like(b) if b is not None else None
    check(lib().mfvit_batch_mix(ptr(a), ptr(b), ptr(out_a), ptr(out_b), ptr(desc), ptr(lam), n, C, H, W, stream()), "mfvit_batch_mix")
    return out_a if b is None else (out_a, out_b)
```

Measured before the change: 4949.

## Batch weight cast-transposes into one table launch, add streaming LN backward, fuse embed grads

Replaces the separate cast_transpose launches for the shadow weights and the cross-attention weight transposes with a single table-driven kernel that walks several tensor families in one grid. It also adds a software-pipelined streaming layernorm-backward kernel that stages output rows through shared memory for vectorized stores. A fused embed_param_grads kernel replaces two colsum passes plus two axpy calls for the cls and patch-embed bias gradients. The aim is fewer small kernel launches and better memory throughput in LN backward, at the cost of more kernel code and an env switch that selects the table path.

```diff
diff --git a/include/mfvit.h b/include/mfvit.h
--- a/include/mfvit.h
+++ b/include/mfvit.h
@@ -139,7 +139,12 @@
 int mfvit_layernorm_bwd(int dtype, const float* dy, const float* x, const float* mean, const float* rstd, const float* gamma,
                         const float* dres, float* dx, void* dx_t, float* dgamma, float* dbeta, float* dcol, int rows, int N,
                         mfvit_stream_t stream);
+int mfvit_layernorm_bwd_ws(int dtype, const float* dy, const float* x, const float* mean, const float* rstd, const float* gamma,
+                           const float* dres, float* dx, void* dx_t, float* dgamma, float* dbeta, float* dcol, float* colpart, int rows, int N,
+                           mfvit_stream_t stream);
 int mfvit_cast_transpose(int dtype, const float* src, void* dst, void* dst_t, int R, int C, mfvit_stream_t stream);
+int mfvit_embed_param_grads(const float* gx, int64_t ld, const float* colsum_all, float* dcls, float* dpe_b, int B, int T, int N, mfvit_stream_t stream);
+int mfvit_cast_table_plan(int dtype, int nfam, const int64_t* fams, int64_t* plan, int64_t* where, int nwhere);
 int mfvit_head_fwd(const float* x, int64_t ldx, const float* w, const float* b, float* y, int64_t ldy, int M, int N, int K, int accumulate,
                    mfvit_stream_t stream);
 int mfvit_head_bwd(const float* dy, int64_t lddy, const float* x, int64_t ldx, const float* w, float* dx, int64_t lddx, int dx_accumulate,
diff --git a/multi-feature-vit_amd/csrc/abi_ops.hip b/multi-feature-vit_amd/csrc/abi_ops.hip
--- a/multi-feature-vit_amd/csrc/abi_ops.hip
+++ b/multi-feature-vit_amd/csrc/abi_ops.hip
@@ -141,9 +141,44 @@
     return ln_bwd_rows(dtype, N, dy, N, x, N, mean, rstd, gamma, dres, N, dx, N, dx_t, dtype == MFVIT_BF16X3 ? 2 * N : N, dgamma, dbeta, dcol, nullptr, rows, 1, 0,
                        (hipStream_t)stream);
 }
+int mfvit_layernorm_bwd_ws(int dtype, const float* dy, const float* x, const float* mean, const float* rstd, const float* gamma,
+                           const float* dres, float* dx, void* dx_t, float* dgamma, float* dbeta, float* dcol, float* colpart, int rows, int N,
+                           mfvit_stream_t stream) {
+    if (!dy || !x || !mean || !rstd || !gamma || !colpart) return MFVIT_EINVAL;
+    return ln_bwd_rows(dtype, N, dy, N, x, N, mean, rstd, gamma, dres, N, dx, N, dx_t, dtype == MFVIT_BF16X3 ? 2 * N : N, dgamma, dbeta, dcol, colpart, rows, 1,
+                       0, (hipStream_t)stream);
+}
 int mfvit_cast_transpose(int dtype, const float* src, void* dst, void* dst_t, int R, int C, mfvit_stream_t stream) {
     if (!src || R <= 0 || C <= 0) return MFVIT_EINVAL;
     return cast_transpose(dtype, src, dst, dst_t, R, C, (hipStream_t)stream);
+}
+int mfvit_embed_param_grads(const float* gx, int64_t ld, const float* colsum_all, float* dcls, float* dpe_b, int B, int T, int N, mfvit_stream_t stream) {
+    return embed_param_grads(gx, ld, colsum_all, dcls, dpe_b, B, T, N, (hipStream_t)stream);
+}
+int mfvit_cast_table_plan(int dtype, int nfam, const int64_t* fams, int64_t* plan, int64_t* where, int nwhere) {
+    if (!fams || !plan || nfam <= 0 || nfam > CAST_TABLE_MAX || (nwhere > 0 && !where)) return MFVIT_EINVAL;
+    CastFam in[CAST_TABLE_MAX];
+    for (int i = 0; i < nfam; ++i) {
+        const int64_t* f = fams + 9 * i;
+        in[i] = CastFam{(const float*)(uintptr_t)f[0], (void*)(uintptr_t)f[1], (void*)(uintptr_t)f[2], (int)f[3], (int)f[4], (int)f[5], (long)f[6], (long)f[7],
+                        (long)f[8]};
+    }
+    CastTable tb;
+    const unsigned own = cast_table_build(dtype, in, nfam, tb);
+    for (int i = 0, k = 0; i < nfam; ++i) {
+        const bool in_table = !(own >> i & 1);
+        plan[3 * i + 0] = in_table ? tb.tile0[k] : -1;
+        plan[3 * i + 1] = in_table ? tb.tile0[k + 1] - tb.tile0[k] : 0;
+        plan[3 * i + 2] = in_table ? k : -1;
+        k += in_table;
+    }
+    const int tiles = tb.tile0[tb.nfam];
+    for (int t = 0; t < tiles && t < nwhere; ++t) {
+        int f, z, r0, c0;
+        cast_table_locate(tb, t, f, z, r0, c0);
+        where[4 * t + 0] = f; where[4 * t + 1] = z; where[4 * t + 2] = r0; where[4 * t + 3] = c0;
+    }
+    return tiles;
 }
 int mfvit_head_fwd(const float* x, int64_t ldx, const float* w, const float* b, float* y, int64_t ldy, int M, int N, int K, int accumulate,
                    mfvit_stream_t stream) {
diff --git a/multi-feature-vit_amd/csrc/elementwise.hip b/multi-feature-vit_amd/csrc/elementwise.hip
--- a/multi-feature-vit_amd/csrc/elementwise.hip
+++ b/multi-feature-vit_amd/csrc/elementwise.hip
@@ -275,123 +275,6 @@
     return MFVIT_OK;
 }
 
-template <typename T, int NPL>
-__global__ __launch_bounds__(256) void ln_bwd_rows_kernel(const float* __restrict__ dy, long lddy, const float* __restrict__ x, long ldx,
-                                                          const float* __restrict__ mean, const float* __restrict__ rstd,
-                                                          const float* __restrict__ gamma, const float* __restrict__ dres, long ldres,
-                                                          float* __restrict__ dx, long lddx, T* __restrict__ dxT, long lddxT,
-                                                          float* __restrict__ dgamma, float* __restrict__ dbeta, float* __restrict__ dcol,
-                                                          float* __restrict__ cpart, int rows, int row_stride, int row_off,
-                                                          const T* __restrict__ dyT, long lddyT) {
-    constexpr int N = NPL * 64;
-    __shared__ float red[3][4][N];
-    const int lane = threadIdx.x & 63, w = threadIdx.x >> 6;
-    float gm[NPL], ag[NPL], ab[NPL], ax[NPL];
-#pragma unroll
-    for (int i = 0; i < NPL; ++i) { gm[i] = gamma[lane + 64 * i]; ag[i] = ab[i] = ax[i] = 0.f; }
-    for (int r = blockIdx.x * 4 + w; r < rows; r += gridDim.x * 4) {
-        const long g = (long)r * row_stride + row_off;
-        const float mu = mean[g], rs = rstd[g];
-        float d[NPL], h[NPL];
-        float s1 = 0.f, s2 = 0.f;
-#pragma unroll
-        for (int i = 0; i < NPL; ++i) {
-            const int n = lane + 64 * i;
-            d[i] = dyT ? load_elem<T>(dyT + g * lddyT, n) : dy[g * lddy + n];
-            h[i] = (x[g * ldx + n] - mu) * rs;
-            const float t = d[i] * gm[i];
-            s1 += t;
-            s2 += t * h[i];
-            ag[i] += d[i] * h[i];
-            ab[i] += d[i];
-        }
-        const float c1 = wave_sum(s1) * (1.0f / N), c2 = wave_sum(s2) * (1.0f / N);
-#pragma unroll
-        for (int i = 0; i < NPL; ++i) {
-            const int n = lane + 64 * i;
-            float o = rs * (d[i] * gm[i] - c1 - h[i] * c2);
-            if (dres) o += dres[g * ldres + n];
-            if (dx) dx[g * lddx + n] = o;
-            if (dxT) store_elem<T>(dxT + g * lddxT, n, o);
-            ax[i] += o;
-        }
-    }
-#pragma unroll
-    for (int i = 0; i < NPL; ++i) {
-        red[0][w][lane + 64 * i] = ag[i];
-        red[1][w][lane + 64 * i] = ab[i];
-        red[2][w][lane + 64 * i] = ax[i];
-    }
-    __syncthreads();
-    for (int n = threadIdx.x; n < N; n += 256) {
-        const float a = red[0][0][n] + red[0][1][n] + red[0][2][n] + red[0][3][n];
-        const float b = red[1][0][n] + red[1][1][n] + red[1][2][n] + red[1][3][n];
-        const float c = red[2][0][n] + red[2][1][n] + red[2][2][n] + red[2][3][n];
-        if (cpart) {
-            cpart[((long)blockIdx.x * 3 + 0) * N + n] = a;
-            cpart[((long)blockIdx.x * 3 + 1) * N + n] = b;
-            cpart[((long)blockIdx.x * 3 + 2) * N + n] = c;
-        } else {
-            if (dgamma) atomicAdd(dgamma + n, a);
-            if (dbeta) atomicAdd(dbeta + n, b);
-            if (dcol) atomicAdd(dcol + n, c);
-        }
-    }
-}
-int ln_bwd_rows(int dtype, int N, const float* dy, long lddy, const float* x, long ldx, const float* mean, const float* rstd,
-                const float* gamma, const float* dres, long ldres, float* dx, long lddx, void* dxT, long lddxT, float* dgamma, float* dbeta,
-                float* dcol, float* cpart, int rows, int row_stride, int row_off, hipStream_t st, const void* dyT, long lddyT) {
-    if (rows <= 0) return MFVIT_OK;
-    if (!dy && !dyT) return MFVIT_EINVAL;
-    int blocks = (rows + 3) / 4;
-    const int cap = cpart ? 256 : 1024;
-    if (blocks > cap) blocks = cap;
-#define MFVIT_LNB(TT, NPL)                                                                                                         \
-    MFVIT_LAUNCH((ln_bwd_rows_kernel<TT, NPL>), dim3(blocks), dim3(256), 0, st, dy, lddy, x, ldx, mean, rstd, gamma, dres, ldres, dx, \
-                       lddx, (TT*)dxT, lddxT, dgamma, dbeta, dcol, cpart, rows, row_stride, row_off, (const TT*)dyT, lddyT)
-#define MFVIT_LNB_N(NPL)                                  \
-    switch (dtype) {                                      \
-        case MFVIT_BF16: MFVIT_LNB(bf16, NPL); break;     \
-        case MFVIT_BF16X3: MFVIT_LNB(sbf16, NPL); break;  \
-        case MFVIT_F16: MFVIT_LNB(f16, NPL); break;       \
-        case MFVIT_F32: MFVIT_LNB(float, NPL); break;     \
-        default: return MFVIT_EINVAL;                     \
-    }
-    if (N == 384) { MFVIT_LNB_N(6) }
-    else if (N == 768) { MFVIT_LNB_N(12) }
-    else return MFVIT_EINVAL;
-#undef MFVIT_LNB_N
-#undef MFVIT_LNB
-    MFVIT_CHECK_LAUNCH();
-    if (cpart) return colpart_reduce(cpart, blocks, N, 3, dgamma, dbeta, dcol, st);
-    return MFVIT_OK;
-}
-
-template <typename T>
-__global__ __launch_bounds__(256) void cast_transpose_kernel(const float* __restrict__ src, T* __restrict__ dst, T* __restrict__ dstT, int R,
-                                                             int C, long s_src, long s_dst, long s_dstT) {
-    __shared__ float tile[64][65];
-    src += blockIdx.z * s_src;
-    if (dst) dst = (T*)((char*)dst + blockIdx.z * s_dst);
-    if (dstT) dstT = (T*)((char*)dstT + blockIdx.z * s_dstT);
-    const int r0 = blockIdx.y * 64, c0 = blockIdx.x * 64;
-    for (int q = threadIdx.x; q < 64 * 64; q += 256) {
-        const int r = q >> 6, c = q & 63;
-        float v = 0.f;
-        if (r0 + r < R && c0 + c < C) {
-            v = src[(long)(r0 + r) * C + c0 + c];
-            if (dst) store_elem<T>(dst + (long)(r0 + r) * C * elems_per<T>::value, c0 + c, v);
-        }
-        tile[r][c] = v;
-    }
-    __syncthreads();
-    if (dstT) {
-        for (int q = threadIdx.x; q < 64 * 64; q += 256) {
-            const int c = q >> 6, r = q & 63;
-            if (r0 + r < R && c0 + c < C) store_elem<T>(dstT + (long)(c0 + c) * R * elems_per<T>::value, r0 + r, tile[r][c]);
-        }
-    }
-}
 template <typename T> __device__ __forceinline__ void store_elem4(T* row, int n, float v0, float v1, float v2, float v3) {
     if constexpr (std::is_same<T, float>::value) {
         *(float4*)(row + n) = make_float4(v0, v1, v2, v3);
@@ -410,6 +293,265 @@
         *(V*)(row + n) = V{h[0], h[1], h[2], h[3]};
     }
 }
+
+template <typename T, int NPL>
+__global__ __launch_bounds__(256) void ln_bwd_rows_kernel(const float* __restrict__ dy, long lddy, const float* __restrict__ x, long ldx,
+                                                          const float* __restrict__ mean, const float* __restrict__ rstd,
+                                                          const float* __restrict__ gamma, const float* __restrict__ dres, long ldres,
+                                                          float* __restrict__ dx, long lddx, T* __restrict__ dxT, long lddxT,
+                                                          float* __restrict__ dgamma, float* __restrict__ dbeta, float* __restrict__ dcol,
+                                                          float* __restrict__ cpart, int rows, int row_stride, int row_off,
+                                                          const T* __restrict__ dyT, long lddyT) {
+    constexpr int N = NPL * 64;
+    __shared__ float red[3][4][N];
+    const int lane = threadIdx.x & 63, w = threadIdx.x >> 6;
+    float gm[NPL], ag[NPL], ab[NPL], ax[NPL];
+#pragma unroll
+    for (int i = 0; i < NPL; ++i) { gm[i] = gamma[lane + 64 * i]; ag[i] = ab[i] = ax[i] = 0.f; }
+    for (int r = blockIdx.x * 4 + w; r < rows; r += gridDim.x * 4) {
+        const long g = (long)r * row_stride + row_off;
+        const float mu = mean[g], rs = rstd[g];
+        float d[NPL], h[NPL];
+        float s1 = 0.f, s2 = 0.f;
+#pragma unroll
+        for (int i = 0; i < NPL; ++i) {
+            const int n = lane + 64 * i;
+            d[i] = dyT ? load_elem<T>(dyT + g * lddyT, n) : dy[g * lddy + n];
+            h[i] = (x[g * ldx + n] - mu) * rs;
+            const float t = d[i] * gm[i];
+            s1 += t;
+            s2 += t * h[i];
+            ag[i] += d[i] * h[i];
+            ab[i] += d[i];
+        }
+        const float c1 = wave_sum(s1) * (1.0f / N), c2 = wave_sum(s2) * (1.0f / N);
+#pragma unroll
+        for (int i = 0; i < NPL; ++i) {
+            const int n = lane + 64 * i;
+            float o = rs * (d[i] * gm[i] - c1 - h[i] * c2);
+            if (dres) o += dres[g * ldres + n];
+            if (dx) dx[g * lddx + n] = o;
+            if (dxT) store_elem<T>(dxT + g * lddxT, n, o);
+            ax[i] += o;
+        }
+    }
+#pragma unroll
+    for (int i = 0; i < NPL; ++i) {
+        red[0][w][lane + 64 * i] = ag[i];
+        red[1][w][lane + 64 * i] = ab[i];
+        red[2][w][lane + 64 * i] = ax[i];
+    }
+    __syncthreads();
+    for (int n = threadIdx.x; n < N; n += 256) {
+        const float a = red[0][0][n] + red[0][1][n] + red[0][2][n] + red[0][3][n];
+        const float b = red[1][0][n] + red[1][1][n] + red[1][2][n] + red[1][3][n];
+        const float c = red[2][0][n] + red[2][1][n] + red[2][2][n] + red[2][3][n];
+        if (cpart) {
+            cpart[((long)blockIdx.x * 3 + 0) * N + n] = a;
+            cpart[((long)blockIdx.x * 3 + 1) * N + n] = b;
+            cpart[((long)blockIdx.x * 3 + 2) * N + n] = c;
+        } else {
+            if (dgamma) atomicAdd(dgamma + n, a);
+            if (dbeta) atomicAdd(dbeta + n, b);
+            if (dcol) atomicAdd(dcol + n, c);
+        }
+    }
+}
+template <typename T, int NPL, bool RES>
+__global__ __launch_bounds__(256) void ln_bwd_rows_stream_kernel(const float* __restrict__ dy, long lddy, const float* __restrict__ x, long ldx,
+                                                                 const float* __restrict__ mean, const float* __restrict__ rstd,
+                                                                 const float* __restrict__ gamma, const float* __restrict__ dres, long ldres,
+                                                                 float* __restrict__ dx, long lddx, T* __restrict__ dxT, long lddxT,
+                                                                 float* __restrict__ dgamma, float* __restrict__ dbeta, float* __restrict__ dcol,
+                                                                 float* __restrict__ cpart, int rows, int row_stride, int row_off) {
+#pragma clang fp contract(off)
+    constexpr int N = NPL * 64;
+    __shared__ __attribute__((aligned(16))) float red[3][4][N];
+    const int lane = threadIdx.x & 63, w = threadIdx.x >> 6;
+    float* const stage = red[0][w];
+    float gm[NPL], ag[NPL], ab[NPL], ax[NPL];
+#pragma unroll
+    for (int i = 0; i < NPL; ++i) { gm[i] = gamma[lane + 64 * i]; ag[i] = ab[i] = ax[i] = 0.f; }
+    struct Row { float d[NPL], xv[NPL], mu, rs; };
+    auto issue = [&](Row& q, int r) __attribute__((always_inline)) {
+        const long g = (long)(r < rows ? r : rows - 1) * row_stride + row_off;
+        q.mu = mean[g];
+        q.rs = rstd[g];
+#pragma unroll
+        for (int i = 0; i < NPL; ++i) {
+            q.d[i] = dy[g * lddy + lane + 64 * i];
+            q.xv[i] = x[g * ldx + lane + 64 * i];
+        }
+    };
+    auto process = [&](const Row& q, int r) __attribute__((always_inline)) {
+        const long g = (long)r * row_stride + row_off;
+        float mu = q.mu, rs = q.rs;
+        float d[NPL], xv[NPL], h[NPL], o[NPL];
+        asm volatile("" : "+v"(mu), "+v"(rs));
+#pragma unroll
+        for (int i = 0; i < NPL; ++i) {
+            d[i] = q.d[i];
+            xv[i] = q.xv[i];
+            asm volatile("" : "+v"(d[i]), "+v"(xv[i]));
+        }
+        float s1 = 0.f, s2 = 0.f, t[NPL];
+#pragma unroll
+        for (int i = 0; i < NPL; ++i) {
+            h[i] = (xv[i] - mu) * rs;
+            t[i] = d[i] * gm[i];
+            s1 += t[i];
+            s2 += t[i] * h[i];
+            ag[i] = fmaf(d[i], h[i], ag[i]);
+            ab[i] += d[i];
+        }
+        const float c1 = wave_sum(s1) * (1.0f / N), c2 = wave_sum(s2) * (1.0f / N);
+#pragma unroll
+        for (int i = 0; i < NPL; ++i) o[i] = rs * fmaf(-c2, h[i], t[i] - c1);
+        if constexpr (RES) {
+#pragma unroll
+            for (int i = 0; i < NPL; ++i) o[i] += dres[g * ldres + lane + 64 * i];
+        }
+#pragma unroll
+        for (int i = 0; i < NPL; ++i) {
+            stage[lane + 64 * i] = o[i];
+            ax[i] += o[i];
+        }
+#pragma unroll
+        for (int k = 0; k < (N / 4 + 63) / 64; ++k) {
+            constexpr int Q = N / 4;
+            const int j = Q - 64 * k >= 64 ? lane + 64 * k : 64 * k + lane % (Q - 64 * k < 64 ? Q - 64 * k : 64);
+            const float4 v = *(const float4*)(stage + 4 * j);
+            *(float4*)(dx + g * lddx + 4 * j) = v;
+            store_elem4<T>(dxT + g * lddxT, 4 * j, v.x, v.y, v.z, v.w);
+        }
+    };
+    const int step = gridDim.x * 4;
+    int r = blockIdx.x * 4 + w;
+    Row qa, qb, qc;
+    issue(qa, r);
+    issue(qb, r + step);
+    int left = r < rows ? (rows - 1 - r) / step + 1 : 0;
+#define MFVIT_LNB_ISSUE(q, row) __builtin_amdgcn_sched_barrier(0); issue(q, row); __builtin_amdgcn_sched_barrier(0)
+    for (; left >= 3; left -= 3, r += 3 * step) {
+        MFVIT_LNB_ISSUE(qc, r + 2 * step);
+        process(qa, r);
+        MFVIT_LNB_ISSUE(qa, r + 3 * step);
+        process(qb, r + step);
+        MFVIT_LNB_ISSUE(qb, r + 4 * step);
+        process(qc, r + 2 * step);
+    }
+#undef MFVIT_LNB_ISSUE
+    if (left >= 1) process(qa, r);
+    if (left == 2) process(qb, r + step);
+#pragma unroll
+    for (int i = 0; i < NPL; ++i) {
+        red[0][w][lane + 64 * i] = ag[i];
+        red[1][w][lane + 64 * i] = ab[i];
+        red[2][w][lane + 64 * i] = ax[i];
+    }
+    __syncthreads();
+    for (int n = threadIdx.x; n < N; n += 256) {
+        const float a = red[0][0][n] + red[0][1][n] + red[0][2][n] + red[0][3][n];
+        const float b = red[1][0][n] + red[1][1][n] + red[1][2][n] + red[1][3][n];
+        const float c = red[2][0][n] + red[2][1][n] + red[2][2][n] + red[2][3][n];
+        if (cpart) {
+            cpart[((long)blockIdx.x * 3 + 0) * N + n] = a;
+            cpart[((long)blockIdx.x * 3 + 1) * N + n] = b;
+            cpart[((long)blockIdx.x * 3 + 2) * N + n] = c;
+        } else {
+            if (dgamma) atomicAdd(dgamma + n, a);
+            if (dbeta) atomicAdd(dbeta + n, b);
+            if (dcol) atomicAdd(dcol + n, c);
+        }
+    }
+}
+int ln_bwd_rows(int dtype, int N, const float* dy, long lddy, const float* x, long ldx, const float* mean, const float* rstd,
+                const float* gamma, const float* dres, long ldres, float* dx, long lddx, void* dxT, long lddxT, float* dgamma, float* dbeta,
+                float* dcol, float* cpart, int rows, int row_stride, int row_off, hipStream_t st, const void* dyT, long lddyT) {
+    if (rows <= 0) return MFVIT_OK;
+    if (!dy && !dyT) return MFVIT_EINVAL;
+    int blocks = (rows + 3) / 4;
+    const int cap = cpart ? 256 : 1024;
+    if (blocks > cap) blocks = cap;
+    static int s_stream = INT_MIN;
+    const bool wide = dy && !dyT && dx && dxT && dtype != MFVIT_F32 && ((uintptr_t)dx & 15) == 0 && lddx % 4 == 0 && lddxT % 4 == 0 &&
+                      ((uintptr_t)dxT & 7) == 0 && env_switch("MFVIT_LNB_STREAM", 1, s_stream) != 0;
+#define MFVIT_LNB(TT, NPL)                                                                                                         \
+    if (wide && dres) MFVIT_LAUNCH((ln_bwd_rows_stream_kernel<TT, NPL, true>), dim3(blocks), dim3(256), 0, st, dy, lddy, x, ldx, mean, rstd, gamma, dres, \
+                       ldres, dx, lddx, (TT*)dxT, lddxT, dgamma, dbeta, dcol, cpart, rows, row_stride, row_off);                        \
+    else if (wide) MFVIT_LAUNCH((ln_bwd_rows_stream_kernel<TT, NPL, false>), dim3(blocks), dim3(256), 0, st, dy, lddy, x, ldx, mean, rstd, gamma, dres, \
+                       ldres, dx, lddx, (TT*)dxT, lddxT, dgamma, dbeta, dcol, cpart, rows, row_stride, row_off);                        \
+    else MFVIT_LAUNCH((ln_bwd_rows_kernel<TT, NPL>), dim3(blocks), dim3(256), 0, st, dy, lddy, x, ldx, mean, rstd, gamma, dres, ldres, dx, \
+                       lddx, (TT*)dxT, lddxT, dgamma, dbeta, dcol, cpart, rows, row_stride, row_off, (const TT*)dyT, lddyT)
+#define MFVIT_LNB_N(NPL)                                  \
+    switch (dtype) {                                      \
+        case MFVIT_BF16: MFVIT_LNB(bf16, NPL); break;     \
+        case MFVIT_BF16X3: MFVIT_LNB(sbf16, NPL); break;  \
+        case MFVIT_F16: MFVIT_LNB(f16, NPL); break;       \
+        case MFVIT_F32: MFVIT_LNB(float, NPL); break;     \
+        default: return MFVIT_EINVAL;                     \
+    }
+    if (N == 384) { MFVIT_LNB_N(6) }
+    else if (N == 768) { MFVIT_LNB_N(12) }
+    else return MFVIT_EINVAL;
+#undef MFVIT_LNB_N
+#undef MFVIT_LNB
+    MFVIT_CHECK_LAUNCH();
+    if (cpart) return colpart_reduce(cpart, blocks, N, 3, dgamma, dbeta, dcol, st);
+    return MFVIT_OK;
+}
+
+template <typename T>
+__global__ __launch_bounds__(256) void cast_transpose_kernel(const float* __restrict__ src, T* __restrict__ dst, T* __restrict__ dstT, int R,
+                                                             int C, long s_src, long s_dst, long s_dstT) {
+    __shared__ float tile[64][65];
+    src += blockIdx.z * s_src;
+    if (dst) dst = (T*)((char*)dst + blockIdx.z * s_dst);
+    if (dstT) dstT = (T*)((char*)dstT + blockIdx.z * s_dstT);
+    const int r0 = blockIdx.y * 64, c0 = blockIdx.x * 64;
+    for (int q = threadIdx.x; q < 64 * 64; q += 256) {
+        const int r = q >> 6, c = q & 63;
+        float v = 0.f;
+        if (r0 + r < R && c0 + c < C) {
+            v = src[(long)(r0 + r) * C + c0 + c];
+            if (dst) store_elem<T>(dst + (long)(r0 + r) * C * elems_per<T>::value, c0 + c, v);
+        }
+        tile[r][c] = v;
+    }
+    __syncthreads();
+    if (dstT) {
+        for (int q = threadIdx.x; q < 64 * 64; q += 256) {
+            const int c = q >> 6, r = q & 63;
+            if (r0 + r < R && c0 + c < C) store_elem<T>(dstT + (long)(c0 + c) * R * elems_per<T>::value, r0 + r, tile[r][c]);
+        }
+    }
+}
+template <typename T>
+__device__ __forceinline__ void cast_transpose4_tile(const float* __restrict__ src, T* __restrict__ dst, T* __restrict__ dstT, int R, int C, int r0,
+                                                     int c0, float (*tile)[65]) {
+#pragma unroll
+    for (int k = 0; k < 4; ++k) {
+        const int q = threadIdx.x + 256 * k, r = q >> 4, c = (q & 15) * 4;
+        float4 v = make_float4(0.f, 0.f, 0.f, 0.f);
+        if (r0 + r < R && c0 + c < C) {
+            v = *(const float4*)(src + (long)(r0 + r) * C + c0 + c);
+            if (dst) store_elem4<T>(dst + (long)(r0 + r) * C * elems_per<T>::value, c0 + c, v.x, v.y, v.z, v.w);
+        }
+        tile[r][c] = v.x;
+        tile[r][c + 1] = v.y;
+        tile[r][c + 2] = v.z;
+        tile[r][c + 3] = v.w;
+    }
+    __syncthreads();
+    if (dstT) {
+#pragma unroll
+        for (int k = 0; k < 4; ++k) {
+            const int q = threadIdx.x + 256 * k, c = q >> 4, r = (q & 15) * 4;
+            if (r0 + r < R && c0 + c < C)
+                store_elem4<T>(dstT + (long)(c0 + c) * R * elems_per<T>::value, r0 + r, tile[r][c], tile[r + 1][c], tile[r + 2][c], tile[r + 3][c]);
+        }
+    }
+}
 template <typename T>
 __global__ __launch_bounds__(256) void cast_transpose4_kernel(const float* __restrict__ src, T* __restrict__ dst, T* __restrict__ dstT, int R,
                                                               int C, long s_src, long s_dst, long s_dstT) {
@@ -417,35 +559,57 @@
     src += blockIdx.z * s_src;
     if (dst) dst = (T*)((char*)dst + blockIdx.z * s_dst);
     if (dstT) dstT = (T*)((char*)dstT + blockIdx.z * s_dstT);
-    const int r0 = blockIdx.y * 64, c0 = blockIdx.x * 64;
-#pragma unroll
-    for (int k = 0; k < 4; ++k) {
-        const int q = threadIdx.x + 256 * k, r = q >> 4, c = (q & 15) * 4;
-        float4 v = make_float4(0.f, 0.f, 0.f, 0.f);
-        if (r0 + r < R && c0 + c < C) {
-            v = *(const float4*)(src + (long)(r0 + r) * C + c0 + c);
-            if (dst) store_elem4<T>(dst + (long)(r0 + r) * C * elems_per<T>::value, c0 + c, v.x, v.y, v.z, v.w);
-        }
-        tile[r][c] = v.x;
-        tile[r][c + 1] = v.y;
-        tile[r][c + 2] = v.z;
-        tile[r][c + 3] = v.w;
-    }
-    __syncthreads();
-    if (dstT) {
-#pragma unroll
-        for (int k = 0; k < 4; ++k) {
-            const int q = threadIdx.x + 256 * k, c = q >> 4, r = (q & 15) * 4;
-            if (r0 + r < R && c0 + c < C)
-                store_elem4<T>(dstT + (long)(c0 + c) * R * elems_per<T>::value, r0 + r, tile[r][c], tile[r + 1][c], tile[r + 2][c], tile[r + 3][c]);
-        }
-    }
+    cast_transpose4_tile<T>(src, dst, dstT, R, C, blockIdx.y * 64, blockIdx.x * 64, tile);
+}
+template <typename T>
+__global__ __launch_bounds__(256) void cast_transpose4_table_kernel(const CastTable tb) {
+    __shared__ float tile[64][65];
+    int f, z, r0, c0;
+    cast_table_locate(tb, blockIdx.x, f, z, r0, c0);
+    const CastFam& m = tb.fam[f];
+    cast_transpose4_tile<T>(m.src + z * m.s_src, m.dst ? (T*)((char*)m.dst + z * m.s_dst) : nullptr,
+                            m.dstT ? (T*)((char*)m.dstT + z * m.s_dstT) : nullptr, m.R, m.C, r0, c0, tile);
+}
+static bool cast_transpose4_ok(int dtype, const float* src, const void* dst, const void* dstT, int R, int C, long s_src, long s_dst, long s_dstT) {
+    return R % 4 == 0 && C % 4 == 0 && s_src % 4 == 0 && s_dst % 16 == 0 && s_dstT % 16 == 0 &&
+           (((uintptr_t)src | (uintptr_t)dst | (uintptr_t)dstT) & 15) == 0 && !(dtype == MFVIT_BF16X3 && ((dst && C % 32) || (dstT && R % 32)));
+}
+unsigned cast_table_build(int dtype, const CastFam* fams, int n, CastTable& tb) {
+    unsigned out = 0;
+    tb.nfam = 0;
+    tb.tile0[0] = 0;
+    for (int i = 0; i < n; ++i) {
+        const CastFam& m = fams[i];
+        const long tiles = (long)((m.R + 63) / 64) * ((m.C + 63) / 64) * m.nb;
+        if (m.R <= 0 || m.C <= 0 || m.nb <= 0 || tb.nfam == CAST_TABLE_MAX || tb.tile0[tb.nfam] + tiles > INT_MAX ||
+            !cast_transpose4_ok(dtype, m.src, m.dst, m.dstT, m.R, m.C, m.s_src, m.s_dst, m.s_dstT)) {
+            out |= 1u << i;
+            continue;
+        }
+        tb.fam[tb.nfam] = m;
+        tb.tile0[tb.nfam + 1] = tb.tile0[tb.nfam] + (int)tiles;
+        ++tb.nfam;
+    }
+    for (int i = tb.nfam; i < CAST_TABLE_MAX; ++i) { tb.fam[i] = CastFam{}; tb.tile0[i + 1] = tb.tile0[tb.nfam]; }
+    return out;
+}
+int cast_transpose_table(int dtype, const CastTable& tb, hipStream_t st) {
+    const int tiles = tb.tile0[tb.nfam];
+    if (tiles <= 0) return MFVIT_OK;
+    switch (dtype) {
+        case MFVIT_BF16: MFVIT_LAUNCH(cast_transpose4_table_kernel<bf16>, dim3(tiles), dim3(256), 0, st, tb); break;
+        case MFVIT_BF16X3: MFVIT_LAUNCH(cast_transpose4_table_kernel<sbf16>, dim3(tiles), dim3(256), 0, st, tb); break;
+        case MFVIT_F16: MFVIT_LAUNCH(cast_transpose4_table_kernel<f16>, dim3(tiles), dim3(256), 0, st, tb); break;
+        case MFVIT_F32: MFVIT_LAUNCH(cast_transpose4_table_kernel<float>, dim3(tiles), dim3(256), 0, st, tb); break;
+        default: return MFVIT_EINVAL;
+    }
+    MFVIT_CHECK_LAUNCH();
+    return MFVIT_OK;
 }
 int cast_transpose_batched(int dtype, const float* src, void* dst, void* dstT, int R, int C, int nb, long s_src, long s_dst, long s_dstT,
                            hipStream_t st) {
     const dim3 grid((C + 63) / 64, (R + 63) / 64, nb);
-    if (R % 4 == 0 && C % 4 == 0 && s_src % 4 == 0 && s_dst % 16 == 0 && s_dstT % 16 == 0 &&
-        (((uintptr_t)src | (uintptr_t)dst | (uintptr_t)dstT) & 15) == 0 && !(dtype == MFVIT_BF16X3 && ((dst && C % 32) || (dstT && R % 32)))) {
+    if (cast_transpose4_ok(dtype, src, dst, dstT, R, C, s_src, s_dst, s_dstT)) {
         switch (dtype) {
             case MFVIT_BF16: MFVIT_LAUNCH(cast_transpose4_kernel<bf16>, grid, dim3(256), 0, st, src, (bf16*)dst, (bf16*)dstT, R, C, s_src, s_dst, s_dstT); break;
             case MFVIT_BF16X3: MFVIT_LAUNCH(cast_transpose4_kernel<sbf16>, grid, dim3(256), 0, st, src, (sbf16*)dst, (sbf16*)dstT, R, C, s_src, s_dst, s_dstT); break;
@@ -604,6 +768,32 @@
     return MFVIT_OK;
 }
 
+__global__ __launch_bounds__(1024) void embed_param_grads_kernel(const float* __restrict__ x, long ld, const float* __restrict__ all,
+                                                                 float* __restrict__ dcls, float* __restrict__ dpe_b, int B, int T, int N) {
+    const int n = blockIdx.x * 64 + (threadIdx.x & 63), sub = threadIdx.x >> 6;
+    __shared__ float sm[16][64];
+    float s = 0.f;
+    if (n < N) {
+#pragma unroll 4
+        for (int r = sub; r < B; r += 16) s += x[(long)r * T * ld + n];
+    }
+    sm[sub][threadIdx.x & 63] = s;
+    __syncthreads();
+    if (sub == 0 && n < N) {
+        s = 0.f;
+#pragma unroll
+        for (int i = 0; i < 16; ++i) s += sm[i][threadIdx.x];
+        dcls[n] += s;
+        if (dpe_b) dpe_b[n] = fmaf(-1.0f, 0.f + s, fmaf(1.0f, all[n], dpe_b[n]));
+    }
+}
+int embed_param_grads(const float* x, long ld, const float* all, float* dcls, float* dpe_b, int B, int T, int N, hipStream_t st) {
+    if (!x || !dcls || (dpe_b && !all) || B <= 0 || T <= 0 || N <= 0) return MFVIT_EINVAL;
+    MFVIT_LAUNCH(embed_param_grads_kernel, dim3((N + 63) / 64), dim3(1024), 0, st, x, ld, all, dcls, dpe_b, B, T, N);
+    MFVIT_CHECK_LAUNCH();
+    return MFVIT_OK;
+}
+
 __global__ __launch_bounds__(256) void batch_sum_kernel(const float* __restrict__ x, float* __restrict__ out, int B, long n) {
     const long i = blockIdx.x * 256L + threadIdx.x;
     if (i >= n) return;
diff --git a/multi-feature-vit_amd/csrc/fusion.hip b/multi-feature-vit_amd/csrc/fusion.hip
--- a/multi-feature-vit_amd/csrc/fusion.hip
+++ b/multi-feature-vit_amd/csrc/fusion.hip
@@ -896,10 +896,19 @@
                               const float* f_enh, float* ws, int B, int T, float eps_pre, hipStream_t st) {
     const int DH = D / nh;
     const float scale = 1.0f / sqrtf((float)DH);
-    for (int dir = 0; dir < ndir; ++dir) {
+    {
+        static_assert(CAST_TABLE_MAX >= 8, "two directions x (wq, wk, wv, wp)");
         const long offs[4] = {L.wq, L.wk, L.wv, L.wp};
-        for (int k = 0; k < 4; ++k)
-            FUS_TRY(cast_transpose(MFVIT_F32, params + L.ca[dir] + offs[k], nullptr, ws + W.wT + ((long)dir * 4 + k) * D * D, D, D, st));
+        CastFam fams[8];
+        int n = 0;
+        for (int dir = 0; dir < ndir && dir < 2; ++dir)
+            for (int k = 0; k < 4; ++k)
+                fams[n++] = CastFam{params + L.ca[dir] + offs[k], nullptr, ws + W.wT + ((long)dir * 4 + k) * D * D, D, D, 1, 0, 0, 0};
+        CastTable tb;
+        const unsigned own = cast_table_build(MFVIT_F32, fams, n, tb);
+        FUS_TRY(cast_transpose_table(MFVIT_F32, tb, st));
+        for (int i = 0; i < n; ++i)
+            if (own >> i & 1) FUS_TRY(cast_transpose(MFVIT_F32, fams[i].src, nullptr, fams[i].dstT, D, D, st));
     }
     MFVIT_LAUNCH(x_cls_ln_kernel<D>, dim3(B, ndir), dim3(64), 0, st, f_cxr, f_enh, params, L, eps_pre, B, T, ws + W.z0, ws + W.st0);
     MFVIT_CHECK_LAUNCH();
diff --git a/multi-feature-vit_amd/csrc/kernels.h b/multi-feature-vit_amd/csrc/kernels.h
--- a/multi-feature-vit_amd/csrc/kernels.h
+++ b/multi-feature-vit_amd/csrc/kernels.h
@@ -69,6 +69,21 @@
 int cast_transpose(int dtype, const float* src, void* dst, void* dstT, int R, int C, hipStream_t st);
 int cast_transpose_batched(int dtype, const float* src, void* dst, void* dstT, int R, int C, int nb, long s_src, long s_dst, long s_dstT,
                            hipStream_t st);
+#define CAST_TABLE_MAX 8
+struct CastFam { const float* src; void* dst; void* dstT; int R, C, nb; long s_src, s_dst, s_dstT; };
+struct CastTable { CastFam fam[CAST_TABLE_MAX]; int tile0[CAST_TABLE_MAX + 1]; int nfam; };
+__host__ __device__ inline void cast_table_locate(const CastTable& tb, int tile, int& f, int& z, int& r0, int& c0) {
+    f = 0;
+#pragma unroll
+    for (int i = 1; i < CAST_TABLE_MAX; ++i) if (i < tb.nfam && tile >= tb.tile0[i]) f = i;
+    const int tc = (tb.fam[f].C + 63) / 64, per = ((tb.fam[f].R + 63) / 64) * tc, t = tile - tb.tile0[f];
+    z = t / per;
+    r0 = (t % per) / tc * 64;
+    c0 = (t % per) % tc * 64;
+}
+unsigned cast_table_build(int dtype, const CastFam* fams, int n, CastTable& tb);
+int cast_transpose_table(int dtype, const CastTable& tb, hipStream_t st);
+int embed_param_grads(const float* x, long ld, const float* all, float* dcls, float* dpe_b, int B, int T, int N, hipStream_t st);
 int linear_small_fwd(const float* x, long ldx, const float* W, const float* b, float* y, long ldy, int M, int N, int K, int accumulate,
                      hipStream_t st);
 int linear_small_bwd(const float* dy, long lddy, const float* x, long ldx, const float* W, float* dx, long lddx, int dx_accumulate, float* dW,
diff --git a/multi-feature-vit_amd/csrc/vit.hip b/multi-feature-vit_amd/csrc/vit.hip
--- a/multi-feature-vit_amd/csrc/vit.hip
+++ b/multi-feature-vit_amd/csrc/vit.hip
@@ -412,14 +412,27 @@
     const ShadowLayout S = shadow_layout(d);
     char* sh = (char*)shadow;
     const bool hw = d.dtype != MFVIT_F32;
-    if (hw && !d.tok) MFVIT_TRY(cast_transpose(d.dtype, params + L.pe_w, sh + S.pe_w, nullptr, d.D, 768, st));
     const float* pb = params + L.blk0;
     char* sb = sh + S.blk0;
     const long ss = L.blk_stride, sd = (long)S.blk_stride;
-    MFVIT_TRY(cast_transpose_batched(d.dtype, pb + L.qkv_w, hw ? sb + S.qkv_w : nullptr, sb + S.qkv_t, 3 * d.D, d.D, d.depth, ss, sd, sd, st));
-    MFVIT_TRY(cast_transpose_batched(d.dtype, pb + L.proj_w, hw ? sb + S.proj_w : nullptr, sb + S.proj_t, d.D, d.D, d.depth, ss, sd, sd, st));
-    MFVIT_TRY(cast_transpose_batched(d.dtype, pb + L.fc1_w, hw ? sb + S.fc1_w : nullptr, sb + S.fc1_t, d.F, d.D, d.depth, ss, sd, sd, st));
-    MFVIT_TRY(cast_transpose_batched(d.dtype, pb + L.fc2_w, hw ? sb + S.fc2_w : nullptr, sb + S.fc2_t, d.D, d.F, d.depth, ss, sd, sd, st));
+    CastFam fams[5];
+    int n = 0;
+    if (hw && !d.tok) fams[n++] = CastFam{params + L.pe_w, sh + S.pe_w, nullptr, d.D, 768, 1, 0, 0, 0};
+    fams[n++] = CastFam{pb + L.qkv_w, hw ? sb + S.qkv_w : nullptr, sb + S.qkv_t, 3 * d.D, d.D, d.depth, ss, sd, sd};
+    fams[n++] = CastFam{pb + L.proj_w, hw ? sb + S.proj_w : nullptr, sb + S.proj_t, d.D, d.D, d.depth, ss, sd, sd};
+    fams[n++] = CastFam{pb + L.fc1_w, hw ? sb + S.fc1_w : nullptr, sb + S.fc1_t, d.F, d.D, d.depth, ss, sd, sd};
+    fams[n++] = CastFam{pb + L.fc2_w, hw ? sb + S.fc2_w : nullptr, sb + S.fc2_t, d.D, d.F, d.depth, ss, sd, sd};
+    static int s_table = INT_MIN;
+    unsigned own = ~0u;
+    if (env_switch("MFVIT_SHADOW_TABLE", 1, s_table) != 0) {
+        CastTable tb;
+        own = cast_table_build(d.dtype, fams, n, tb);
+        MFVIT_TRY(cast_transpose_table(d.dtype, tb, st));
+    }
+    for (int i = 0; i < n; ++i)
+        if (own >> i & 1)
+            MFVIT_TRY(cast_transpose_batched(d.dtype, fams[i].src, fams[i].dst, fams[i].dstT, fams[i].R, fams[i].C, fams[i].nb, fams[i].s_src,
+                                             fams[i].s_dst, fams[i].s_dstT, st));
     return MFVIT_OK;
 }
 
@@ -791,11 +804,8 @@
                 MFVIT_TRY(gemm_nt_tile(d.dtype, EPI_COL2IM16, p, st));
             }
             if (!wg) continue;
-            MFVIT_TRY(colsum_rows(gx, D, dparams + L.cls, d.B, d.T, 0, d.D, st));
+            MFVIT_TRY(embed_param_grads(gx, D, colscr, dparams + L.cls, cfg->stop_grad_conv1 ? nullptr : dparams + L.pe_b, d.B, d.T, d.D, st));
             if (!cfg->stop_grad_conv1) {
-                MFVIT_TRY(colsum_rows(gx, D, colscr + D, d.B, d.T, 0, d.D, st));
-                MFVIT_TRY(axpy(dparams + L.pe_b, colscr, 1.0f, d.D, st));
-                MFVIT_TRY(axpy(dparams + L.pe_b, colscr + D, -1.0f, d.D, st));
                 GemmP p = nt(pp(W.gxT, -1), D * e, ws + W.patches, 768 * e, d.Mp, d.D, 768);
                 p.orow_in = d.np; p.orow_out = d.T; p.orow_off = 1;
                 p.out0 = dparams + L.pe_w; p.ldo0 = 768;
diff --git a/multi-feature-vit_amd/mfvit/_lib.py b/multi-feature-vit_amd/mfvit/_lib.py
--- a/multi-feature-vit_amd/mfvit/_lib.py
+++ b/multi-feature-vit_amd/mfvit/_lib.py
@@ -84,7 +84,10 @@
     "mfvit_dropout_mask": (I, [F, c_uint64, c_uint32, L, P, P]),
     "mfvit_layernorm_fwd": (I, [I, P, P, I, P, P, F, P, P, I, I, P]),
     "mfvit_layernorm_bwd": (I, [I, P, P, P, P, P, P, P, P, P, P, P, I, I, P]),
+    "mfvit_layernorm_bwd_ws": (I, [I, P, P, P, P, P, P, P, P, P, P, P, P, I, I, P]),
     "mfvit_cast_transpose": (I, [I, P, P, P, I, I, P]),
+    "mfvit_embed_param_grads": (I, [P, L, P, P, P, I, I, I, P]),
+    "mfvit_cast_table_plan": (I, [I, I, POINTER(c_int64), POINTER(c_int64), POINTER(c_int64), I]),
     "mfvit_head_fwd": (I, [P, L, P, P, P, L, I, I, I, I, P]),
     "mfvit_head_bwd": (I, [P, L, P, L, P, P, L, I, P, P, I, I, I, P]),
     "mfvit_cross_entropy": (I, [P, P, P, P, P, I, I, P]),
diff --git a/multi-feature-vit_amd/mfvit/ops.py b/multi-feature-vit_amd/mfvit/ops.py
--- a/multi-feature-vit_amd/mfvit/ops.py
+++ b/multi-feature-vit_amd/mfvit/ops.py
@@ -258,6 +258,27 @@
     check(lib().mfvit_layernorm_bwd(code, ptr(dy), ptr(x), ptr(mean), ptr(rstd), ptr(gamma), ptr(dres), ptr(dx), ptr(dx_t), ptr(dgamma),
                                     ptr(dbeta), ptr(dcol), rows, N, stream()), "mfvit_layernorm_bwd")
     return dx, dx_t, dgamma, dbeta, dcol
+
+
+def layernorm_bwd_ws(dy, x, mean, rstd, gamma, dres=None, copy_dtype=None, split=False):
+    require_cuda(dy, x)
+    rows, N = x.shape
+    dx = torch.empty_like(x)
+    dx_t = torch.empty(rows, N * (2 if split else 1), device=x.device, dtype=copy_dtype) if copy_dtype is not None else None
+    dgamma = torch.zeros(N, device=x.device, dtype=torch.float32)
+    dbeta = torch.zeros_like(dgamma)
+    dcol = torch.zeros_like(dgamma)
+    colpart = torch.zeros(256, 3, N, device=x.device, dtype=torch.float32)
+    code = _code_of_dtype(copy_dtype, split)
+    check(lib().mfvit_layernorm_bwd_ws(code, ptr(dy), ptr(x), ptr(mean), ptr(rstd), ptr(gamma), ptr(dres), ptr(dx), ptr(dx_t), ptr(dgamma),
+                                       ptr(dbeta), ptr(dcol), ptr(colpart), rows, N, stream()), "mfvit_layernorm_bwd_ws")
+    return dx, dx_t, dgamma, dbeta, dcol, colpart[:min((rows + 3) // 4, 256)]
+
+
+def embed_param_grads(gx, colsum_all, dcls, dpe_b, B, T):
+    require_cuda(gx, colsum_all, dcls, dpe_b)
+    check(lib().mfvit_embed_param_grads(ptr(gx), gx.stride(0), ptr(colsum_all), ptr(dcls), ptr(dpe_b), B, T, gx.shape[1], stream()),
+          "mfvit_embed_param_grads")
 
 
 def cast_transpose(src, dtype, want_straight=True, want_transposed=True, split=False):
```

New measurement: 4969 (median of 6 runs). About the same (+0.4%).
